# alexlocher/hpmvs

Measured on AMD Instinct MI355X. Metric: refined_patches_per_sec, higher is better.
Workload: dtype f32 textures / f64 optimiser

## Files before the change

hpmvs_amd/api.py:

```python
from __future__ import annotations

import ctypes as C
import os
from dataclasses import dataclass

import numpy as np

try:
    import torch
except Exception:
    torch = None

HERE = os.path.dirname(os.path.abspath(__file__))
LIB_PATH = os.environ.get("HPMVS_LIB") or os.path.join(HERE, "libhpmvs_amd.so")
MAX_IMAGES = 256
FAST_IMAGES = 64
MAX_LEVELS = 8


class HpmvsError(RuntimeError):
    pass


class Options(C.Structure):
    _fields_ = [("MAXLEVEL", C.c_int32), ("MINLEVEL", C.c_int32), ("MAX_ANGLE", C.c_float),
                ("MIN_ANGLE", C.c_float), ("MAX_IMAGES_PER_PATCH", C.c_int32),
                ("MIN_IMAGES_PER_PATCH", C.c_int32), ("NCC_ALPHA_1", C.c_float), ("NCC_ALPHA_2", C.c_float)]


class Camera(C.Structure):
    _fields_ = [("P0", C.c_float * 12), ("center", C.c_float * 4), ("xaxis", C.c_float * 3),
                ("yaxis", C.c_float * 3), ("zaxis", C.c_float * 3), ("fsum", C.c_float), ("n_levels", C.c_int32)]


class PatchBatch(C.Structure):
    _fields_ = [("n", C.c_int32), ("max_images", C.c_int32), ("center", C.c_void_p), ("normal", C.c_void_p),
                ("scale", C.c_void_p), ("n_images", C.c_void_p), ("images", C.c_void_p), ("ok", C.c_void_p),
                ("color", C.c_void_p), ("ncc", C.c_void_p), ("fmin", C.c_void_p), ("x", C.c_void_p),
                ("result", C.c_void_p), ("nevals", C.c_void_p), ("stage", C.c_void_p), ("ngrabs", C.c_void_p)]


class LeafTable(C.Structure):
    _fields_ = [("n", C.c_int32), ("root_center", C.c_float * 3), ("root_width", C.c_float), ("cell_center", C.c_void_p),
                ("cell_width", C.c_void_p), ("patch_center", C.c_void_p), ("born", C.c_void_p), ("died", C.c_void_p)]


class OctreeIndex(C.Structure):
    _fields_ = [("root_center", C.c_float * 3), ("root_width", C.c_float), ("n_branches", C.c_int32), ("n_leaves", C.c_int32),
                ("branch_key", C.c_void_p), ("leaf_key", C.c_void_p)]


class ExtendTreeKeysStruct(C.Structure):
    _fields_ = [("skip", C.c_void_p), ("pre_inside", C.c_void_p), ("pre_key", C.c_void_p), ("border", C.c_void_p),
                ("post_key", C.c_void_p)]


class OctreeForest(C.Structure):
    _fields_ = [("n_trees", C.c_int32), ("root", C.c_void_p), ("branch_first", C.c_void_p), ("leaf_first", C.c_void_p),
                ("branch_key", C.c_void_p), ("leaf_key", C.c_void_p)]


class ProcessForestResultStruct(C.Structure):
    _fields_ = [("support", C.c_void_p), ("removed", C.c_void_p), ("split", C.c_void_p), ("children", C.c_void_p),
                ("child_key", C.c_void_p), ("n_neighbours", C.c_void_p), ("neighbour_key", C.c_void_p)]


class BorderForestResultStruct(C.Structure):
    _fields_ = [("tree", C.c_void_p), ("accepted", C.c_void_p), ("leaf_key", C.c_void_p), ("blocker", C.c_void_p)]


class OctreePartitionInfo(C.Structure):
    _fields_ = [("n_trees", C.c_int32), ("n_orphans", C.c_int32), ("n_splits", C.c_int32), ("stop", C.c_int32),
                ("histogram", C.c_int32 * 22)]


class SeedTreeInfo(C.Structure):
    _fields_ = [("root_center", C.c_float * 3), ("root_width", C.c_float), ("scale_floor", C.c_float), ("n_rows", C.c_int32),
                ("n_leaves", C.c_int32)]


EXPORTS = [
    "hpmvs_last_error", "hpmvs_device_count", "hpmvs_build_id", "hpmvs_default_options", "hpmvs_camera_from_nvm",
    "hpmvs_scene_create", "hpmvs_scene_set_view", "hpmvs_scene_set_covis", "hpmvs_scene_commit",
    "hpmvs_scene_destroy", "hpmvs_scene_get_level", "hpmvs_scene_bytes", "hpmvs_build_pyramid",
    "hpmvs_optimize_batch", "hpmvs_init_patches_batch", "hpmvs_objective_batch", "hpmvs_inccs_batch", "hpmvs_last_kernel_ms",
    "hpmvs_last_wide_patches",
    "hpmvs_expand_batch", "hpmvs_expand_directions", "hpmvs_selftest_bobyqa",
    "hpmvs_pack_records", "hpmvs_unpack_records", "hpmvs_allgather_records", "hpmvs_pack_record_tails", "hpmvs_unpack_record_tails",
    "hpmvs_scene_depth_reset", "hpmvs_scene_depth_set_level", "hpmvs_scene_depth_get_level",
    "hpmvs_set_depths_batch", "hpmvs_depth_gates_batch", "hpmvs_depth_footprints_batch", "hpmvs_depth_ops_batch", "hpmvs_level_support_batch",
    "hpmvs_host_alloc", "hpmvs_host_free", "hpmvs_last_staging",
    "hpmvs_undistort", "hpmvs_undistort_map", "hpmvs_scene_set_view_distorted",
    "hpmvs_regularize_batch", "hpmvs_filter_batch", "hpmvs_seed_tree_batch", "hpmvs_octree_locate_batch",
    "hpmvs_octree_insert_batch", "hpmvs_octree_route_batch", "hpmvs_octree_partition", "hpmvs_extend_tree_batch",
    "hpmvs_extend_forest_batch", "hpmvs_process_forest_batch", "hpmvs_border_forest_batch",
    "hpmvs_level_conflicts_batch", "hpmvs_conflicts_from_footprints", "hpmvs_level_walk_batch", "hpmvs_last_level_walk",
    "hpmvs_scene_center", "hpmvs_init_patches_sphere_batch",
    "hpmvs_jpeg_info", "hpmvs_jpeg_decode", "hpmvs_scene_set_view_jpeg", "hpmvs_jpeg_decode_timed",
    "hpmvs_jpeg_decode_ex", "hpmvs_scene_set_view_jpeg_ex", "hpmvs_jpeg_coefficients", "hpmvs_jpeg_entropy_timed",
    "hpmvs_jpeg_last_decode",
    "hpmvs_jpeg_encode_bound", "hpmvs_jpeg_encode", "hpmvs_jpeg_encode_timed", "hpmvs_scene_get_level_jpeg",
    "hpmvs_depth_colormap", "hpmvs_scene_depth_image", "hpmvs_scene_depth_jpeg",
    "hpmvs_ply_ext_batch", "hpmvs_ply_ext_timed",
]
JPEG_ENTROPY = {"auto": 0, "host": 1, "device": 2}


_lib = None


def lib():
    global _lib
    if _lib is not None:
        return _lib
    if not os.path.exists(LIB_PATH):
        raise HpmvsError(f"{LIB_PATH} is missing: run `python -c 'import __graft_entry__ as g; g.build()'` "
                         "(there is no fallback implementation)")
    L = C.CDLL(LIB_PATH)
    L.hpmvs_last_error.restype = C.c_char_p
    L.hpmvs_build_id.restype = C.c_char_p
    L.hpmvs_default_options.argtypes = [C.POINTER(Options)]
    L.hpmvs_camera_from_nvm.argtypes = [C.c_double, C.POINTER(C.c_double), C.POINTER(C.c_double), C.c_int, C.c_int,
                                        C.c_int, C.POINTER(Camera)]
    L.hpmvs_scene_create.argtypes = [C.c_int, C.c_int, C.POINTER(C.c_void_p)]
    L.hpmvs_scene_set_view.argtypes = [C.c_void_p, C.c_int, C.c_int, C.c_int, C.c_void_p, C.c_int, C.POINTER(Camera)]
    L.hpmvs_scene_set_covis.argtypes = [C.c_void_p, C.c_int, C.POINTER(C.c_int32), C.c_int]
    L.hpmvs_scene_commit.argtypes = [C.c_void_p]
    L.hpmvs_scene_destroy.argtypes = [C.c_void_p]
    L.hpmvs_scene_get_level.argtypes = [C.c_void_p, C.c_int, C.c_int, C.c_void_p, C.c_size_t, C.POINTER(C.c_int),
                                        C.POINTER(C.c_int)]
    L.hpmvs_scene_bytes.restype = C.c_size_t
    L.hpmvs_scene_bytes.argtypes = [C.c_void_p]
    L.hpmvs_build_pyramid.argtypes = [C.c_int, C.c_void_p, C.c_int, C.c_int, C.c_void_p, C.c_int]
    L.hpmvs_undistort.argtypes = [C.c_int, C.c_void_p, C.c_int, C.c_int, C.c_float, C.c_float, C.c_void_p, C.c_int]
    L.hpmvs_undistort_map.argtypes = [C.c_int, C.c_int, C.c_int, C.c_float, C.c_float, C.c_void_p]
    L.hpmvs_scene_set_view_distorted.argtypes = [C.c_void_p, C.c_int, C.c_int, C.c_int, C.c_void_p, C.c_int,
                                                 C.POINTER(Camera), C.c_float, C.c_float]
    L.hpmvs_jpeg_info.argtypes = [C.c_char_p, C.c_size_t] + [C.POINTER(C.c_int)] * 5
    L.hpmvs_jpeg_decode.argtypes = [C.c_int, C.c_char_p, C.c_size_t, C.c_void_p, C.c_size_t, C.c_int]
    L.hpmvs_jpeg_decode_timed.argtypes = [C.c_int, C.c_char_p, C.c_size_t, C.c_void_p, C.c_size_t, C.POINTER(C.c_float)]
    L.hpmvs_scene_set_view_jpeg.argtypes = [C.c_void_p, C.c_int, C.c_char_p, C.c_size_t, C.POINTER(Camera), C.c_float, C.c_float]
    L.hpmvs_jpeg_decode_ex.argtypes = [C.c_int, C.c_char_p, C.c_size_t, C.c_void_p, C.c_size_t, C.c_int, C.c_int, C.POINTER(C.c_int)]
    L.hpmvs_scene_set_view_jpeg_ex.argtypes = [C.c_void_p, C.c_int, C.c_char_p, C.c_size_t, C.POINTER(Camera), C.c_float, C.c_float,
                                               C.c_int, C.POINTER(C.c_int)]
    L.hpmvs_jpeg_coefficients.argtypes = [C.c_int, C.c_char_p, C.c_size_t, C.c_int, C.c_int, C.c_void_p, C.c_size_t,
                                          C.POINTER(C.c_int), C.POINTER(C.c_int)]
    L.hpmvs_jpeg_last_decode.argtypes = [C.POINTER(C.c_int), C.POINTER(C.c_int)]
    L.hpmvs_jpeg_entropy_timed.argtypes = [C.c_int, C.c_char_p, C.c_size_t, C.c_void_p, C.c_size_t, C.POINTER(C.c_float)]
    L.hpmvs_jpeg_encode_bound.restype = C.c_size_t
    L.hpmvs_jpeg_encode_bound.argtypes = [C.c_int, C.c_int]
    L.hpmvs_jpeg_encode.argtypes = [C.c_int, C.c_void_p, C.c_int, C.c_int, C.c_int, C.c_void_p, C.c_size_t, C.POINTER(C.c_size_t), C.c_int]
    L.hpmvs_jpeg_encode_timed.argtypes = [C.c_int, C.c_void_p, C.c_int, C.c_int, C.c_int, C.c_void_p, C.c_size_t, C.POINTER(C.c_size_t),
                                          C.POINTER(C.c_float)]
    L.hpmvs_scene_get_level_jpeg.argtypes = [C.c_void_p, C.c_int, C.c_int, C.c_int, C.c_void_p, C.c_size_t, C.POINTER(C.c_size_t)]
    L.hpmvs_optimize_batch.argtypes = [C.c_void_p, C.POINTER(Options), C.POINTER(PatchBatch), C.c_int, C.c_void_p]
    L.hpmvs_init_patches_batch.argtypes = [C.c_void_p, C.POINTER(Options), C.c_int, C.c_int, C.c_void_p, C.c_void_p,
                                           C.c_void_p, C.POINTER(PatchBatch), C.c_int, C.c_void_p]
    L.hpmvs_init_patches_sphere_batch.argtypes = [C.c_void_p, C.POINTER(Options), C.c_int, C.c_int, C.c_void_p, C.c_void_p,
                                                  C.c_void_p, C.c_void_p, C.POINTER(PatchBatch), C.c_int, C.c_void_p]
    L.hpmvs_scene_center.argtypes = [C.c_void_p, C.c_int, C.POINTER(C.c_double), C.POINTER(C.c_double), C.POINTER(C.c_int)]
    L.hpmvs_objective_batch.argtypes = [C.c_void_p, C.POINTER(Options), C.POINTER(PatchBatch), C.c_void_p,
                                        C.c_void_p, C.c_void_p, C.c_int, C.c_void_p]
    L.hpmvs_inccs_batch.argtypes = [C.c_void_p, C.POINTER(Options), C.POINTER(PatchBatch), C.c_int, C.c_int,
                                    C.c_void_p, C.c_int, C.c_void_p]
    L.hpmvs_last_kernel_ms.argtypes = [C.c_void_p, C.POINTER(C.c_float)]
    L.hpmvs_host_alloc.argtypes = [C.c_size_t]
    L.hpmvs_host_alloc.restype = C.c_void_p
    L.hpmvs_host_free.argtypes = [C.c_void_p]
    L.hpmvs_host_free.restype = None
    L.hpmvs_last_staging.argtypes = [C.c_void_p, C.POINTER(C.c_ulonglong), C.POINTER(C.c_ulonglong)]
    L.hpmvs_expand_batch.argtypes = [C.c_void_p, C.POINTER(Options), C.c_int, C.POINTER(PatchBatch), C.c_void_p,
                                     C.c_void_p, C.c_void_p, C.POINTER(PatchBatch), C.c_int, C.c_void_p]
    L.hpmvs_expand_directions.argtypes = [C.c_int, C.c_void_p]
    L.hpmvs_scene_depth_reset.argtypes = [C.c_void_p]
    L.hpmvs_scene_depth_set_level.argtypes = [C.c_void_p, C.c_int, C.c_int, C.c_void_p, C.c_int, C.c_int]
    L.hpmvs_scene_depth_get_level.argtypes = [C.c_void_p, C.c_int, C.c_int, C.c_void_p, C.c_size_t, C.POINTER(C.c_int),
                                              C.POINTER(C.c_int)]
    L.hpmvs_depth_colormap.argtypes = [C.c_void_p]
    L.hpmvs_scene_depth_image.argtypes = [C.c_void_p, C.c_int, C.c_int, C.c_void_p, C.c_size_t, C.c_int, C.POINTER(C.c_int),
                                          C.POINTER(C.c_int), C.POINTER(C.c_float)]
    L.hpmvs_scene_depth_jpeg.argtypes = [C.c_void_p, C.c_int, C.c_int, C.c_int, C.c_void_p, C.c_size_t, C.POINTER(C.c_size_t)]
    L.hpmvs_set_depths_batch.argtypes = [C.c_void_p, C.POINTER(PatchBatch), C.c_int, C.c_void_p]
    L.hpmvs_depth_footprints_batch.argtypes = [C.c_void_p, C.POINTER(PatchBatch), C.c_void_p, C.c_void_p, C.c_void_p, C.c_void_p,
                                               C.c_int, C.c_void_p]
    L.hpmvs_level_conflicts_batch.argtypes = [C.c_void_p, C.POINTER(PatchBatch), C.c_void_p, C.c_void_p, C.c_void_p, C.c_size_t,
                                              C.c_void_p, C.c_void_p, C.c_size_t, C.POINTER(C.c_uint32), C.POINTER(C.c_uint32),
                                              C.c_int, C.c_void_p]
    L.hpmvs_conflicts_from_footprints.argtypes = [C.c_int] * 5 + [C.c_void_p] * 6 + [C.c_void_p, C.c_void_p, C.c_size_t,
                                                  C.c_void_p, C.c_void_p, C.c_size_t, C.POINTER(C.c_uint32), C.POINTER(C.c_uint32),
                                                  C.c_int, C.c_void_p]
    L.hpmvs_level_walk_batch.argtypes = [C.c_void_p, C.POINTER(Options), C.POINTER(PatchBatch)] + [C.c_void_p] * 4 + [C.c_float, C.c_int] + \
        [C.c_void_p] * 4 + [C.POINTER(C.c_int32), C.c_int, C.c_void_p]
    L.hpmvs_last_level_walk.argtypes = [C.c_void_p] + [C.POINTER(C.c_int32)] * 3
    L.hpmvs_depth_gates_batch.argtypes = [C.c_void_p, C.POINTER(PatchBatch), C.c_float, C.c_int, C.c_void_p, C.c_void_p,
                                          C.c_void_p, C.c_int, C.c_void_p]
    L.hpmvs_depth_ops_batch.argtypes = [C.c_void_p, C.POINTER(PatchBatch), C.c_void_p, C.c_int, C.c_void_p]
    L.hpmvs_regularize_batch.argtypes = [C.c_void_p, C.POINTER(PatchBatch), C.c_void_p, C.c_void_p, C.c_void_p, C.POINTER(LeafTable),
                                         C.c_void_p, C.c_void_p, C.c_void_p, C.c_int, C.c_void_p]
    L.hpmvs_level_support_batch.argtypes = [C.c_void_p, C.POINTER(PatchBatch), C.c_int, C.c_void_p, C.c_int, C.c_void_p]
    L.hpmvs_filter_batch.argtypes = [C.c_void_p, C.POINTER(PatchBatch), C.c_void_p, C.c_int, C.c_void_p, C.c_void_p, C.c_int, C.c_void_p]
    L.hpmvs_seed_tree_batch.argtypes = [C.c_void_p, C.POINTER(PatchBatch), C.c_int, C.c_int, C.POINTER(SeedTreeInfo), C.c_void_p,
                                        C.c_void_p, C.c_void_p, C.c_void_p, C.c_void_p, C.c_void_p, C.c_int, C.c_void_p]
    L.hpmvs_octree_locate_batch.argtypes = [C.c_void_p, C.POINTER(OctreeIndex), C.c_int] + [C.c_void_p] * 8 + [C.c_int, C.c_void_p]
    L.hpmvs_octree_insert_batch.argtypes = [C.c_void_p, C.POINTER(OctreeIndex), C.c_int] + [C.c_void_p] * 5 + [C.c_int, C.c_void_p]
    L.hpmvs_extend_tree_batch.argtypes = [C.c_void_p, C.POINTER(Options), C.POINTER(OctreeIndex), C.POINTER(PatchBatch), C.c_float,
                                          C.POINTER(PatchBatch), C.POINTER(ExtendTreeKeysStruct), C.c_int, C.c_void_p]
    L.hpmvs_extend_forest_batch.argtypes = [C.c_void_p, C.POINTER(Options), C.POINTER(OctreeForest), C.POINTER(PatchBatch), C.c_void_p,
                                            C.c_float, C.POINTER(PatchBatch), C.POINTER(ExtendTreeKeysStruct), C.c_int, C.c_void_p]
    L.hpmvs_process_forest_batch.argtypes = [C.c_void_p, C.POINTER(Options), C.POINTER(OctreeForest), C.c_void_p, C.POINTER(PatchBatch),
                                             C.c_void_p, C.c_void_p, C.c_void_p, C.c_void_p, C.POINTER(PatchBatch),
                                             C.POINTER(ProcessForestResultStruct), C.c_int, C.c_void_p]
    L.hpmvs_border_forest_batch.argtypes = [C.c_void_p, C.POINTER(OctreeForest), C.POINTER(PatchBatch), C.c_int,
                                            C.POINTER(BorderForestResultStruct), C.c_int, C.c_void_p]
    L.hpmvs_octree_route_batch.argtypes = [C.c_void_p, C.c_int, C.c_void_p, C.c_int, C.c_void_p, C.c_void_p, C.c_int, C.c_void_p]
    L.hpmvs_octree_partition.argtypes = [C.c_void_p, C.POINTER(OctreeIndex), C.c_int, C.c_int, C.POINTER(OctreePartitionInfo)] + \
        [C.c_void_p] * 9 + [C.c_int, C.c_void_p]
    L.hpmvs_ply_ext_batch.argtypes = [C.c_int, C.POINTER(PatchBatch), C.c_void_p, C.c_int, C.c_int, C.c_void_p, C.c_size_t,
                                      C.POINTER(C.c_size_t), C.c_int, C.c_void_p]
    L.hpmvs_ply_ext_timed.argtypes = [C.c_int, C.POINTER(PatchBatch), C.c_void_p, C.c_int, C.c_int, C.c_void_p, C.c_size_t,
                                      C.POINTER(C.c_size_t), C.POINTER(C.c_float)]
    _lib = L
    return L


def _chk(rc):
    if rc != 0:
        raise HpmvsError(f"hpmvs_amd error {rc}: {lib().hpmvs_last_error().decode()}")


def build_id() -> str:
    return lib().hpmvs_build_id().decode()


def device_count() -> int:
    return lib().hpmvs_device_count()


def default_options() -> Options:
    o = Options()
    lib().hpmvs_default_options(C.byref(o))
    return o


def camera_from_nvm(f, q, c, width, height, max_level=5) -> Camera:
    cam = Camera()
    qq = (C.c_double * 4)(*[float(t) for t in q])
    cc = (C.c_double * 3)(*[float(t) for t in c])
    _chk(lib().hpmvs_camera_from_nvm(float(f), qq, cc, int(width), int(height), int(max_level), C.byref(cam)))
    return cam


def scene_center(cameras):
    cams = (Camera * max(1, len(cameras)))(*cameras)
    center, radius, valid = (C.c_double * 3)(), C.c_double(), C.c_int()
    _chk(lib().hpmvs_scene_center(cams, len(cameras), center, C.byref(radius), C.byref(valid)))
    if not valid.value:
        return None
    return np.array(center[:], dtype=np.float64), radius.value


def _ptr(a):
    if a is None:
        return None
    if isinstance(a, np.ndarray):
        return a.ctypes.data
    if isinstance(a, int):
        return a
    return a.data_ptr()


def undistort(img, f: float, k1: float, device: int = 0):
    if isinstance(img, np.ndarray):
        src = np.ascontiguousarray(img, dtype=np.uint8)
        if src.ndim != 3 or src.shape[2] != 3:
            raise HpmvsError("undistort: img must be uint8 [H, W, 3]")
        out = np.empty_like(src)
        _chk(lib().hpmvs_undistort(device, src.ctypes.data, src.shape[1], src.shape[0], float(f), float(k1),
                                   out.ctypes.data, 0))
        return out
    src = img.contiguous()
    if src.dim() != 3 or src.shape[2] != 3 or str(src.dtype) != "torch.uint8":
        raise HpmvsError("undistort: img must be uint8 [H, W, 3]")
    out = torch.empty_like(src)
    _chk(lib().hpmvs_undistort(device, src.data_ptr(), src.shape[1], src.shape[0], float(f), float(k1), out.data_ptr(), 1))
    return out


def undistort_map(w: int, h: int, f: float, k1: float, device: int = 0) -> np.ndarray:
    xy = np.empty((int(h), int(w), 2), dtype=np.float32)
    _chk(lib().hpmvs_undistort_map(device, int(w), int(h), float(f), float(k1), xy.ctypes.data))
    return xy


def jpeg_info(data):
    data = bytes(data)
    v = [C.c_int() for _ in range(5)]
    _chk(lib().hpmvs_jpeg_info(data, len(data), *[C.byref(x) for x in v]))
    return tuple(x.value for x in v)


def _jpeg_entropy(name):
    if name not in JPEG_ENTROPY:
        raise HpmvsError(f"entropy must be one of {sorted(JPEG_ENTROPY)}, not {name!r}")
    return JPEG_ENTROPY[name]


def jpeg_decode(data, device: int = 0, on_device: bool = False, entropy: str = "auto"):
    data = bytes(data)
    mode = _jpeg_entropy(entropy)
    w, h = jpeg_info(data)[:2]
    if on_device:
        out = torch.empty((h, w, 3), dtype=torch.uint8, device=f"cuda:{device}")
        ptr, nb = out.data_ptr(), out.numel()
    else:
        out = np.empty((h, w, 3), dtype=np.uint8)
        ptr, nb = out.ctypes.data, out.nbytes
    if mode == 0:
        _chk(lib().hpmvs_jpeg_decode(device, data, len(data), ptr, nb, int(on_device)))
    else:
        _chk(lib().hpmvs_jpeg_decode_ex(device, data, len(data), ptr, nb, int(on_device), mode, None))
    return out


def jpeg_coefficients(data, entropy: str = "auto", subseq_bits: int = 0, device: int = 0):
    data = bytes(data)
    w, h, comps, hs, vs = jpeg_info(data)
    mx, my = -(-w // (8 * hs)), -(-h // (8 * vs))
    out = np.empty(64 * mx * my * (hs * vs + (2 if comps == 3 else 0)), dtype=np.int16)
    used, rounds = C.c_int(), C.c_int()
    _chk(lib().hpmvs_jpeg_coefficients(device, data, len(data), _jpeg_entropy(entropy), int(subseq_bits), out.ctypes.data, out.size,
                                       C.byref(used), C.byref(rounds)))
    return out, "device" if used.value == 2 else "host", rounds.value


def jpeg_encode_bound(width: int, height: int) -> int:
    return int(lib().hpmvs_jpeg_encode_bound(int(width), int(height)))


def jpeg_encode(rgb, quality: int = 100, device: int = 0) -> bytes:
    if isinstance(rgb, np.ndarray):
        rgb = np.ascontiguousarray(rgb, dtype=np.uint8)
        ptr, on_device = rgb.ctypes.data, 0
    else:
        rgb = rgb.contiguous()
        ptr, on_device = rgb.data_ptr(), 1
    if rgb.ndim != 3 or rgb.shape[2] != 3 or (on_device and rgb.dtype != torch.uint8):
        raise HpmvsError("jpeg_encode: pixels must be uint8 [H, W, 3]")
    h, w = int(rgb.shape[0]), int(rgb.shape[1])
    out = np.empty(max(1, jpeg_encode_bound(w, h)), dtype=np.uint8)
    n = C.c_size_t(0)
    _chk(lib().hpmvs_jpeg_encode(device, ptr, w, h, int(quality), out.ctypes.data, out.nbytes, C.byref(n), on_device))
    return out[:n.value].tobytes()


class Scene:

    def __init__(self, synth_scene, device: int = 0, jpeg_entropy: str = "auto"):
        L = lib()
        jpeg_mode = _jpeg_entropy(jpeg_entropy)
        self.h = C.c_void_p()
        self.device = device
        self.n_views = synth_scene.n_views
        self.view_levels = []
        self.cameras = []
        _chk(L.hpmvs_scene_create(self.n_views, device, C.byref(self.h)))
        for i, v in enumerate(synth_scene.views):
            rgb = v.rgb
            if isinstance(rgb, (bytes, bytearray)):
                data = bytes(rgb)
                w, h = jpeg_info(data)[:2]
                cam = camera_from_nvm(v.f, v.q, v.c, w, h, synth_scene.max_level)
                self.view_levels.append(int(cam.n_levels))
                self.cameras.append(cam)
                if jpeg_mode == 0:
                    _chk(L.hpmvs_scene_set_view_jpeg(self.h, i, data, len(data), C.byref(cam), float(v.f),
                                                     float(getattr(v, "k1", 0.0))))
                else:
                    _chk(L.hpmvs_scene_set_view_jpeg_ex(self.h, i, data, len(data), C.byref(cam), float(v.f),
                                                        float(getattr(v, "k1", 0.0)), jpeg_mode, None))
                continue
            cam = camera_from_nvm(v.f, v.q, v.c, v.width, v.height, synth_scene.max_level)
            self.view_levels.append(int(cam.n_levels))
            self.cameras.append(cam)
            if isinstance(rgb, np.ndarray):
                rgb = np.ascontiguousarray(rgb, dtype=np.uint8)
                ptr, on_device = rgb.ctypes.data, 0
            else:
                rgb = rgb.contiguous()
                ptr, on_device = rgb.data_ptr(), 1
            k1 = float(getattr(v, "k1", 0.0))
            if k1 != 0.0:
                _chk(L.hpmvs_scene_set_view_distorted(self.h, i, v.width, v.height, ptr, on_device, C.byref(cam),
                                                      float(v.f), k1))
            else:
                _chk(L.hpmvs_scene_set_view(self.h, i, v.width, v.height, ptr, on_device, C.byref(cam)))
        for i, lst in enumerate(synth_scene.covis):
            arr = (C.c_int32 * max(1, len(lst)))(*lst)
            _chk(L.hpmvs_scene_set_covis(self.h, i, arr, len(lst)))
        _chk(L.hpmvs_scene_commit(self.h))

    def close(self):
        if self.h:
            lib().hpmvs_scene_destroy(self.h)
            self.h = C.c_void_p()

    def __del__(self):
        try:
            self.close()
        except Exception:
            pass

    def bytes(self) -> int:
        return lib().hpmvs_scene_bytes(self.h)

    def level(self, view: int, level: int) -> np.ndarray:
        w, h = C.c_int(), C.c_int()
        _chk(lib().hpmvs_scene_get_level(self.h, view, level, None, 0, C.byref(w), C.byref(h)))
        out = np.empty((h.value, w.value, 3), dtype=np.uint8)
        _chk(lib().hpmvs_scene_get_level(self.h, view, level, out.ctypes.data, out.nbytes, C.byref(w), C.byref(h)))
        return out

    def level_jpeg(self, view: int, level: int = 0, quality: int = 100) -> bytes:
        n = C.c_size_t(0)
        _chk(lib().hpmvs_scene_get_level_jpeg(self.h, view, level, int(quality), None, 0, C.byref(n)))
        out = np.empty(n.value, dtype=np.uint8)
        _chk(lib().hpmvs_scene_get_level_jpeg(self.h, view, level, int(quality), out.ctypes.data, out.nbytes, C.byref(n)))
        return out[:n.value].tobytes()

    def depth_image(self, view: int, level=None, with_range: bool = False):
        lv = DEPTH_COMBINED if level is None else int(level)
        w, h = C.c_int(), C.c_int()
        _chk(lib().hpmvs_scene_depth_image(self.h, view, lv, None, 0, 0, C.byref(w), C.byref(h), None))
        out = np.empty((h.value, w.value, 3), dtype=np.uint8)
        rng = (C.c_float * 2)()
        _chk(lib().hpmvs_scene_depth_image(self.h, view, lv, out.ctypes.data if out.size else None, out.nbytes, 0, C.byref(w), C.byref(h), rng))
        return (out, (np.float32(rng[0]), np.float32(rng[1]))) if with_range else out

    def depth_jpeg(self, view: int, level=None, quality: int = 100) -> bytes:
        lv = DEPTH_COMBINED if level is None else int(level)
        n = C.c_size_t(0)
        _chk(lib().hpmvs_scene_depth_jpeg(self.h, view, lv, int(quality), None, 0, C.byref(n)))
        out = np.empty(n.value, dtype=np.uint8)
        _chk(lib().hpmvs_scene_depth_jpeg(self.h, view, lv, int(quality), out.ctypes.data, out.nbytes, C.byref(n)))
        return out[:n.value].tobytes()

    def last_staging(self):
        a, b = C.c_ulonglong(), C.c_ulonglong()
        _chk(lib().hpmvs_last_staging(self.h, C.byref(a), C.byref(b)))
        return a.value, b.value

    def last_wide_patches(self) -> int:
        n = C.c_int32()
        _chk(lib().hpmvs_last_wide_patches(self.h, C.byref(n)))
        return n.value

    def last_kernel_ms(self) -> float:
        ms = C.c_float()
        _chk(lib().hpmvs_last_kernel_ms(self.h, C.byref(ms)))
        return ms.value


class Batch:

    def __init__(self, center, normal, scale, n_images, images):
        self.n = int(len(scale))
        self.max_images = int(images.shape[1])
        self.center = np.ascontiguousarray(center, dtype=np.float32).copy()
        self.normal = np.ascontiguousarray(normal, dtype=np.float32).copy()
        self.scale = np.ascontiguousarray(scale, dtype=np.float32).copy()
        self.n_images = np.ascontiguousarray(n_images, dtype=np.int32).copy()
        self.images = np.ascontiguousarray(images, dtype=np.int32).copy()
        n = self.n
        self.ok = np.zeros(n, dtype=np.uint8)
        self.color = np.zeros((n, 3), dtype=np.float32)
        self.ncc = np.zeros(n, dtype=np.float32)
        self.fmin = np.zeros(n, dtype=np.float64)
        self.x = np.zeros((n, 3), dtype=np.float64)
        self.result = np.zeros(n, dtype=np.int32)
        self.nevals = np.zeros(n, dtype=np.int32)
        self.stage = np.zeros(n, dtype=np.int32)
        self.ngrabs = np.zeros(n, dtype=np.int32)

    @classmethod
    def from_seeds(cls, seeds, idx=None):
        if idx is None:
            idx = np.arange(len(seeds.scale))
        idx = np.asarray(idx)
        return cls(seeds.center[idx], seeds.normal[idx], seeds.scale[idx], seeds.n_images[idx], seeds.images[idx])

    FIELDS = ("center", "normal", "scale", "n_images", "images", "ok", "color", "ncc", "fmin", "x", "result", "nevals",
              "stage", "ngrabs")

    def pin(self):
        import weakref
        L = lib()
        for name in self.FIELDS:
            a = getattr(self, name)
            nbytes = max(int(a.nbytes), 1)
            p = L.hpmvs_host_alloc(nbytes)
            if not p:
                raise MemoryError(f"hpmvs_host_alloc({nbytes})")
            buf = (C.c_char * nbytes).from_address(p)
            weakref.finalize(buf, L.hpmvs_host_free, p)
            na = np.frombuffer(buf, dtype=a.dtype, count=a.size).reshape(a.shape)
            na[...] = a
            setattr(self, name, na)
        return self

    def c_struct(self) -> PatchBatch:
        b = PatchBatch()
        b.n, b.max_images = self.n, self.max_images
        for name in ("center", "normal", "scale", "n_images", "images", "ok", "color", "ncc", "fmin", "x", "result",
                     "nevals", "stage", "ngrabs"):
            setattr(b, name, _ptr(getattr(self, name)))
        return b


def optimize_batch(scene: Scene, batch: Batch, options: Options | None = None) -> Batch:
    o = options or default_options()
    b = batch.c_struct()
    _chk(lib().hpmvs_optimize_batch(scene.h, C.byref(o), C.byref(b), 0, None))
    return batch


def init_patches_batch(scene: Scene, xyz, meas_off, meas_img, start_level=4, max_images=FAST_IMAGES,
                       options: Options | None = None, sphere=None) -> Batch:
    o = options or default_options()
    xyz = np.ascontiguousarray(xyz, dtype=np.float64)
    off = np.ascontiguousarray(meas_off, dtype=np.int32)
    img = np.ascontiguousarray(meas_img, dtype=np.int32)
    n = len(xyz)
    batch = Batch(np.zeros((n, 4), np.float32), np.zeros((n, 4), np.float32), np.zeros(n, np.float32),
                  np.zeros(n, np.int32), np.full((n, max_images), -1, np.int32))
    b = batch.c_struct()
    if sphere is None:
        _chk(lib().hpmvs_init_patches_batch(scene.h, C.byref(o), start_level, n, xyz.ctypes.data, off.ctypes.data,
                                            img.ctypes.data if len(img) else None, C.byref(b), 0, None))
        return batch
    sph = np.ascontiguousarray(sphere, dtype=np.float64).reshape(4)
    _chk(lib().hpmvs_init_patches_sphere_batch(scene.h, C.byref(o), start_level, n, xyz.ctypes.data, off.ctypes.data,
                                               img.ctypes.data if len(img) else None, sph.ctypes.data, C.byref(b), 0, None))
    return batch


EXPAND_EXTEND, EXPAND_BRANCH = 0, 1


def expand_directions(mode: int) -> np.ndarray:
    out = np.zeros(12, dtype=np.float32)
    n = lib().hpmvs_expand_directions(mode, out.ctypes.data)
    if n < 0:
        _chk(n)
    return out[:2 * n].reshape(n, 2)


def expand_batch(scene: Scene, mode: int, parents: Batch, cell_center, cell_width, skip=None,
                 options: Options | None = None) -> Batch:
    o = options or default_options()
    N = 6 if mode == EXPAND_EXTEND else 4
    n = parents.n
    cc = np.ascontiguousarray(cell_center, dtype=np.float32).reshape(n, 3)
    cw = np.ascontiguousarray(cell_width, dtype=np.float32).reshape(n)
    sk = None if skip is None else np.ascontiguousarray(skip, dtype=np.uint8).reshape(n * N)
    out = Batch(np.zeros((n * N, 4), np.float32), np.zeros((n * N, 4), np.float32), np.zeros(n * N, np.float32),
                np.zeros(n * N, np.int32), np.full((n * N, parents.max_images), -1, np.int32))
    pb, ob = parents.c_struct(), out.c_struct()
    _chk(lib().hpmvs_expand_batch(scene.h, C.byref(o), mode, C.byref(pb), cc.ctypes.data, cw.ctypes.data,
                                  None if sk is None else sk.ctypes.data, C.byref(ob), 0, None))
    return out


def objective_batch(scene: Scene, batch: Batch, x: np.ndarray, options: Options | None = None):
    o = options or default_options()
    b = batch.c_struct()
    x = np.ascontiguousarray(x, dtype=np.float64)
    f = np.zeros(batch.n, dtype=np.float64)
    g = np.zeros(batch.n, dtype=np.int32)
    _chk(lib().hpmvs_objective_batch(scene.h, C.byref(o), C.byref(b), x.ctypes.data, f.ctypes.data, g.ctypes.data, 0,
                                     None))
    return f, g


def inccs_batch(scene: Scene, batch: Batch, ref_idx=0, robust=0, options: Options | None = None) -> np.ndarray:
    o = options or default_options()
    b = batch.c_struct()
    out = np.zeros((batch.n, batch.max_images), dtype=np.float32)
    _chk(lib().hpmvs_inccs_batch(scene.h, C.byref(o), C.byref(b), ref_idx, robust, out.ctypes.data, 0, None))
    return out


def depth_reset(scene: Scene):
    _chk(lib().hpmvs_scene_depth_reset(scene.h))


def depth_level(scene: Scene, view: int, level: int) -> np.ndarray:
    r, c = C.c_int(), C.c_int()
    _chk(lib().hpmvs_scene_depth_get_level(scene.h, view, level, None, 0, C.byref(r), C.byref(c)))
    out = np.zeros((c.value, r.value), dtype=np.float32)
    _chk(lib().hpmvs_scene_depth_get_level(scene.h, view, level, out.ctypes.data, out.size, C.byref(r), C.byref(c)))
    return out


depth_get_level = depth_level


def depth_set_level(scene: Scene, view: int, level: int, data):
    m = np.ascontiguousarray(data, dtype=np.float32)
    if m.size:
        _chk(lib().hpmvs_scene_depth_set_level(scene.h, view, level, m.ctypes.data, m.shape[1], m.shape[0]))


DEPTH_COMBINED = -1


def depth_colormap() -> np.ndarray:
    lut = np.zeros((256, 3), dtype=np.uint8)
    _chk(lib().hpmvs_depth_colormap(lut.ctypes.data))
    return lut


def set_depths_batch(scene: Scene, batch: Batch):
    b = batch.c_struct()
    _chk(lib().hpmvs_set_depths_batch(scene.h, C.byref(b), 0, None))


def depth_ops_batch(scene: Scene, batch: Batch, subtract):
    b = batch.c_struct()
    sub = np.ascontiguousarray(subtract, dtype=np.uint8).reshape(batch.n)
    _chk(lib().hpmvs_depth_ops_batch(scene.h, C.byref(b), sub.ctypes.data, 0, None))


def level_support_batch(scene: Scene, batch: Batch, min_level=0):
    b = batch.c_struct()
    out = np.zeros(batch.n, dtype=np.int32)
    _chk(lib().hpmvs_level_support_batch(scene.h, C.byref(b), int(min_level), out.ctypes.data, 0, None))
    return out


def depth_gates_batch(scene: Scene, batch: Batch, margin=1.0, abs_int=0):
    b = batch.c_struct()
    v = np.zeros(batch.n, dtype=np.int32); k = np.zeros(batch.n, dtype=np.int32); f = np.zeros(batch.n, dtype=np.int32)
    _chk(lib().hpmvs_depth_gates_batch(scene.h, C.byref(b), float(margin), int(abs_int), v.ctypes.data, k.ctypes.data,
                                       f.ctypes.data, 0, None))
    return v, k, f


def depth_footprints_batch(scene: Scene, batch: Batch):
    b = batch.c_struct()
    n, M, V = batch.n, batch.max_images, scene.n_views
    wr = np.zeros((n, M, 4), np.int32); fr = np.zeros((n, M, 4), np.int32)
    at = np.zeros((n, M, 3), np.int32); vb = np.zeros((n, V, 3), np.int32)
    _chk(lib().hpmvs_depth_footprints_batch(scene.h, C.byref(b), wr.ctypes.data, fr.ctypes.data, at.ctypes.data, vb.ctypes.data, 0, None))
    return wr, fr, at, vb


def _conflicts(call, n):
    fo = np.zeros(n + 1, np.uint32); ao = np.zeros(n + 1, np.uint32)
    nf, na = C.c_uint32(0), C.c_uint32(0)
    fa = np.zeros(32 * n + 64, np.uint32); aa = np.zeros(32 * n + 64, np.uint32)
    rc = call(fo.ctypes.data, fa.ctypes.data, fa.size, ao.ctypes.data, aa.ctypes.data, aa.size, C.byref(nf), C.byref(na))
    if rc != 0:
        if "capacity" not in lib().hpmvs_last_error().decode():
            _chk(rc)
        fa = np.zeros(nf.value, np.uint32); aa = np.zeros(na.value, np.uint32)
        _chk(call(fo.ctypes.data, fa.ctypes.data, fa.size, ao.ctypes.data, aa.ctypes.data, aa.size, C.byref(nf), C.byref(na)))
    return fo, fa[:nf.value].copy(), ao, aa[:na.value].copy()


def level_conflicts(scene: Scene, batch: Batch, is_event=None):
    b = batch.c_struct()
    ev = None if is_event is None else np.ascontiguousarray(is_event, dtype=np.uint8).reshape(batch.n)
    evp = None if ev is None else ev.ctypes.data
    return _conflicts(lambda fo, fa, cf, ao, aa, ca, nf, na: lib().hpmvs_level_conflicts_batch(
        scene.h, C.byref(b), evp, fo, fa, cf, ao, aa, ca, nf, na, 0, None), batch.n)


def conflicts_from_footprints(n_images, writes, frees, attached, view_block, n_levels, is_event=None, device: int = 0):
    wr = np.ascontiguousarray(writes, dtype=np.int32); fr = np.ascontiguousarray(frees, dtype=np.int32)
    at = np.ascontiguousarray(attached, dtype=np.int32); vb = np.ascontiguousarray(view_block, dtype=np.int32)
    n, M, V = wr.shape[0], wr.shape[1], vb.shape[1]
    if wr.shape != (n, M, 4) or fr.shape != (n, M, 4) or at.shape != (n, M, 3) or vb.shape != (n, V, 3):
        raise ValueError("conflicts_from_footprints: the footprint arrays do not have the layouts of depth_footprints_batch")
    ni = np.ascontiguousarray(n_images, dtype=np.int32).reshape(n)
    ev = None if is_event is None else np.ascontiguousarray(is_event, dtype=np.uint8).reshape(n)
    evp = None if ev is None else ev.ctypes.data
    return _conflicts(lambda fo, fa, cf, ao, aa, ca, nf, na: lib().hpmvs_conflicts_from_footprints(
        int(device), n, M, V, int(n_levels), ni.ctypes.data, wr.ctypes.data, fr.ctypes.data, at.ctypes.data, vb.ctypes.data, evp,
        fo, fa, cf, ao, aa, ca, nf, na, 0, None), n)


WALK_EVENT, WALK_REFINED, WALK_BORDER, WALK_HAS_PRE, WALK_PRE_TAKEN, WALK_POST_TAKEN = 1, 2, 4, 8, 16, 32


def level_walk(scene: Scene, batch: Batch, flags, set, pre_key, post_key, margin=1.0, abs_int=0, options: Options | None = None,
               stage=None):
    o = options or default_options()
    n = batch.n
    b = batch.c_struct()
    fl = np.ascontiguousarray(flags, dtype=np.uint8).reshape(n)
    st = None if set is None else np.ascontiguousarray(set, dtype=np.int32).reshape(n)
    pre = np.ascontiguousarray(pre_key, dtype=np.uint64).reshape(n)
    post = np.ascontiguousarray(post_key, dtype=np.uint64).reshape(n)
    stage = np.array(batch.stage if stage is None else stage, dtype=np.int32).reshape(n)
    counts = np.full((n, 3), -1, np.int32); accepted = np.zeros(n, np.uint8); wave = np.zeros(n, np.int32)
    n_waves = C.c_int32(0)
    _chk(lib().hpmvs_level_walk_batch(scene.h, C.byref(o), C.byref(b), fl.ctypes.data, None if st is None else st.ctypes.data,
                                      pre.ctypes.data, post.ctypes.data, float(margin), int(abs_int), stage.ctypes.data,
                                      counts.ctypes.data, accepted.ctypes.data, wave.ctypes.data, C.byref(n_waves), 0, None))
    return stage, counts, accepted, wave, int(n_waves.value)


def last_level_walk(scene: Scene):
    r, m, f = C.c_int32(0), C.c_int32(0), C.c_int32(0)
    _chk(lib().hpmvs_last_level_walk(scene.h, C.byref(r), C.byref(m), C.byref(f)))
    return int(r.value), int(m.value), int(f.value)


def build_pyramid(img: np.ndarray, device: int = 0) -> np.ndarray:
    h, w, _ = img.shape
    img = np.ascontiguousarray(img, dtype=np.uint8)
    out = np.zeros((h // 2, w // 2, 3), dtype=np.uint8)
    _chk(lib().hpmvs_build_pyramid(device, img.ctypes.data, w, h, out.ctypes.data, 0))
    return out


INT32_MAX = 2**31 - 1
REGULARIZE_PROBES = 24


def regularize_batch(scene: Scene, cells: Batch, cell_width, position, expanded, root_center, root_width, leaf_center,
                     leaf_width, leaf_patch, born=None, died=None, flatness=None, neighbours: bool = True):
    n = cells.n
    L = int(len(leaf_width))
    cw = np.ascontiguousarray(cell_width, dtype=np.float32).reshape(n)
    pos = np.ascontiguousarray(position, dtype=np.int32).reshape(n)
    exp = np.ascontiguousarray(expanded).astype(np.uint8).reshape(n)
    lc = np.ascontiguousarray(leaf_center, dtype=np.float32).reshape(L, 3)
    lw = np.ascontiguousarray(leaf_width, dtype=np.float32).reshape(L)
    lp = np.ascontiguousarray(np.asarray(leaf_patch, dtype=np.float32)[:, :3]).reshape(L, 3)
    lb = np.full(L, -1, np.int32) if born is None else np.ascontiguousarray(born, dtype=np.int32).reshape(L)
    ld = np.full(L, INT32_MAX, np.int32) if died is None else np.ascontiguousarray(died, dtype=np.int32).reshape(L)
    t = LeafTable()
    t.n = L
    for k in range(3):
        t.root_center[k] = float(np.float32(root_center[k]))
    t.root_width = float(np.float32(root_width))
    t.cell_center, t.cell_width, t.patch_center = lc.ctypes.data, lw.ctypes.data, lp.ctypes.data
    t.born, t.died = lb.ctypes.data, ld.ctypes.data
    fl = np.full(n, -1.0, np.float32) if flatness is None else np.ascontiguousarray(flatness, dtype=np.float32).reshape(n).copy()
    nn = np.zeros(n, np.int32)
    nb = np.zeros((n, REGULARIZE_PROBES), np.int32) if neighbours else None
    b = cells.c_struct()
    _chk(lib().hpmvs_regularize_batch(scene.h, C.byref(b), cw.ctypes.data, pos.ctypes.data, exp.ctypes.data, C.byref(t),
                                      fl.ctypes.data, nn.ctypes.data, None if nb is None else nb.ctypes.data, 0, None))
    return fl, nn, nb


def filter_batch(scene: Scene, patches: Batch, cell_start):
# ... 315 lines not shown
```

hpmvs_amd/csrc/capi.hip:

```cpp
#include <hip/hip_runtime.h>

#include <dlfcn.h>

#include <algorithm>
#include <atomic>
#include <chrono>
#include <cmath>
#include <cstdio>
#include <cstdlib>
#include <cstring>
#include <mutex>
#include <optional>
#include <string>
#include <thread>
#include <time.h>
#include <vector>

#include "../../include/hpmvs_amd.h"
#include "capi_common.hpp"
#include "dev_types.h"
#include "launch.h"
#include "octree.hpp"
#include "ply_text.hpp"

// ... 2489 lines not shown
        if (!on_device) {
            df = nf ? (uint32_t*)c.scratch(4 * (size_t)nf) : nullptr; da = na ? (uint32_t*)c.scratch(4 * (size_t)na) : nullptr;
            if ((nf && !df) || (na && !da)) return c.error();
        }
        launch_conflicts_adjacency(pairs, nf, na, df, da, st);
        HIPCHK(hipGetLastError());
        if (!on_device) {
            HIPCHK(hipStreamSynchronize(st));
            if (nf) HIPCHK(hipMemcpy(flow_adj, df, 4 * (size_t)nf, hipMemcpyDeviceToHost));
            if (na) HIPCHK(hipMemcpy(anti_adj, da, 4 * (size_t)na, hipMemcpyDeviceToHost));
        }
    }
    const int done = c.finish();
    if (done) return done;
    if (!fits) return fail(HPMVS_ERR_ARG, who + ": capacity: the graph has " + std::to_string(nf) + " flow and " + std::to_string(na) +
                                              " anti entries (n_flow / n_anti are set; allocate and call again)");
    return HPMVS_OK;
}
static int conflicts_empty(int on_device, uint32_t* flow_off, uint32_t* anti_off, uint32_t* n_flow, uint32_t* n_anti, hipStream_t st) {
    if (on_device) {
        HIPCHK(hipMemsetAsync(flow_off, 0, 4, st));
        HIPCHK(hipMemsetAsync(anti_off, 0, 4, st));
    } else { flow_off[0] = 0; anti_off[0] = 0; }
    *n_flow = 0; *n_anti = 0;
    return HPMVS_OK;
}

int hpmvs_conflicts_from_footprints(int device, int n, int max_images, int n_views, int n_levels, const int32_t* n_images, const int32_t* writes,
                                    const int32_t* frees, const int32_t* attached, const int32_t* view_block, const uint8_t* is_event,
                                    uint32_t* flow_off, uint32_t* flow_adj, size_t cap_flow, uint32_t* anti_off, uint32_t* anti_adj,
                                    size_t cap_anti, uint32_t* n_flow, uint32_t* n_anti, int on_device, void* stream) {
    const std::string who = "conflicts_from_footprints";
    int rc = conflicts_check(who, n, max_images, n_views, n_levels, flow_off, flow_adj, cap_flow, anti_off, anti_adj, cap_anti, n_flow, n_anti);
    if (rc) return rc;
    if (n > 0 && (!n_images || !writes || !frees || !attached || !view_block)) return fail(HPMVS_ERR_ARG, who + ": a footprint array is null");
    const int count = hpmvs_device_count();
    if (count <= 0) return fail(HPMVS_ERR_NODEVICE, who + ": no HIP device visible");
    if (device < 0 || device >= count) return fail(HPMVS_ERR_ARG, who + ": no such device");
    HIPCHK(hipSetDevice(device));
    hipStream_t st = (hipStream_t)stream;
    if (n == 0) return conflicts_empty(on_device, flow_off, anti_off, n_flow, n_anti, st);
    Call c(nullptr, on_device, st);
    const size_t N = (size_t)n, M = (size_t)max_images, V = (size_t)n_views;
    conflicts::Footprints F;
    F.n = n; F.M = max_images; F.V = n_views; F.n_levels = n_levels;
    F.n_images = c.in(n_images, N);
    F.wr = c.in(writes, N * M * 4); F.fr = c.in(frees, N * M * 4); F.at = c.in(attached, N * M * 3); F.vb = c.in(view_block, N * V * 3);
    F.is_event = c.in(is_event, N);
    uint32_t* dfo = c.arr(flow_off, N + 1, Call::kCopyBack);
    uint32_t* dao = c.arr(anti_off, N + 1, Call::kCopyBack);
    if ((rc = c.begin())) return rc;
    return conflicts_call(c, who, F, on_device, dfo, flow_adj, cap_flow, dao, anti_adj, cap_anti, n_flow, n_anti, st);
}

int hpmvs_level_conflicts_batch(const hpmvs_scene* s, const hpmvs_patch_batch* b, const uint8_t* is_event, uint32_t* flow_off, uint32_t* flow_adj,
                                size_t cap_flow, uint32_t* anti_off, uint32_t* anti_adj, size_t cap_anti, uint32_t* n_flow, uint32_t* n_anti,
                                int on_device, void* stream) {
    const std::string who = "level_conflicts_batch";
    int rc = check_depth_batch(s, b, who.c_str());
    if (rc) return rc;
    int n_levels = 1;
    for (int v = 0; v < s->n_views; v++) n_levels = std::max(n_levels, (int)s->hviews[v].n_levels);
    if ((rc = conflicts_check(who, b->n, b->max_images, s->n_views, n_levels, flow_off, flow_adj, cap_flow, anti_off, anti_adj, cap_anti, n_flow, n_anti)))
        return rc;
    HIPCHK(hipSetDevice(s->device));
    hipStream_t st = (hipStream_t)stream;
    if (b->n == 0) return conflicts_empty(on_device, flow_off, anti_off, n_flow, n_anti, st);
    Call c(s, on_device, st);
    const size_t N = (size_t)b->n, M = (size_t)b->max_images, V = (size_t)s->n_views;
    const DevBatch D = c.batch(b, Call::kRead);
    const uint8_t* dev = c.in(is_event, N);
    uint32_t* dfo = c.arr(flow_off, N + 1, Call::kCopyBack);
    uint32_t* dao = c.arr(anti_off, N + 1, Call::kCopyBack);
    int32_t* fp = (int32_t*)c.scratch(4 * N * (11 * M + 3 * V));
    if (!fp) return c.error();
    if ((rc = c.begin())) return rc;
    conflicts::Footprints F;
    F.n = b->n; F.M = b->max_images; F.V = s->n_views; F.n_levels = n_levels;
    F.n_images = D.n_images; F.is_event = dev;
    int32_t *wr = fp, *fr = wr + N * M * 4, *at = fr + N * M * 4, *vb = at + N * M * 3;
    F.wr = wr; F.fr = fr; F.at = at; F.vb = vb;
    launch_depth_footprints(dev_scene(s), s->ddepth, D, wr, fr, at, vb, st);
    HIPCHK(hipGetLastError());
    return conflicts_call(c, who, F, on_device, dfo, flow_adj, cap_flow, dao, anti_adj, cap_anti, n_flow, n_anti, st);
}

static constexpr int kWalkFewDecided = 8;
static constexpr int kWalkFinishBudget = 128;
int hpmvs_level_walk_batch(hpmvs_scene* s, const hpmvs_options* o, const hpmvs_patch_batch* items, const uint8_t* flags, const int32_t* set,
                           const uint64_t* pre_key, const uint64_t* post_key, float margin, int abs_int, int32_t* stage, int32_t* counts,
                           uint8_t* accepted, int32_t* wave, int32_t* n_waves, int on_device, void* stream) {
    const std::string who = "level_walk_batch";
    if (!s || !o || !items || !n_waves) return fail(HPMVS_ERR_ARG, who + ": null scene / options / batch / n_waves");
    if (items->n < 0 || items->max_images < 1 || items->max_images > HPMVS_MAX_IMAGES) return fail(HPMVS_ERR_ARG, who + ": bad n/max_images");
    if (items->n > 0 && (!items->center || !items->normal || !items->scale || !items->n_images || !items->images))
        return fail(HPMVS_ERR_ARG, who + ": batch input arrays missing");
    if (items->n > 0 && (!flags || !pre_key || !post_key || !stage || !counts || !accepted || !wave))
        return fail(HPMVS_ERR_ARG, who + ": flags / pre_key / post_key / stage / counts / accepted / wave missing");
    if (o->MIN_IMAGES_PER_PATCH < 1) return fail(HPMVS_ERR_ARG, who + ": MIN_IMAGES_PER_PATCH must be >= 1");
    int n_levels = 1;
    for (int v = 0; v < s->n_views; v++) n_levels = std::max(n_levels, (int)s->hviews[v].n_levels);
    {
        uint32_t off = 0, total = 0;
        const int rc = conflicts_check(who, items->n, items->max_images, s->n_views, n_levels, &off, nullptr, 0, &off, nullptr, 0, &total, &total);
        if (rc) return rc;
    }
    if (!s->committed || !s->depth_pool || !s->ddepth) return fail(HPMVS_ERR_STATE, who + ": call hpmvs_scene_depth_reset first");
    if (s->depth_floats >= ((size_t)1 << 32)) return fail(HPMVS_ERR_STATE, who + ": the scene's depth maps hold 2^32 cells or more");
    *n_waves = 0;
    for (auto& w : s->last_walk) w = 0;
    if (items->n == 0) return HPMVS_OK;
    HIPCHK(hipSetDevice(s->device));
    hipStream_t st = (hipStream_t)stream;
    int rc;
    Call c(s, on_device, st);
    const int n = items->n, M = items->max_images, V = s->n_views;
    const size_t N = (size_t)n;
    const DevBatch D = c.batch(items, Call::kRead);
    const uint8_t* dflags = c.in(flags, N);
    const int32_t* dset = c.in(set, N);
    const unsigned long long *dpre = c.in((const unsigned long long*)pre_key, N), *dpost = c.in((const unsigned long long*)post_key, N);
    int32_t* dstage = c.arr(stage, N, Call::kCopyIn | Call::kCopyBack);
    int32_t* dcounts = c.arr(counts, 3 * N, Call::kCopyBack);
    uint8_t* daccepted = c.arr(accepted, N, Call::kCopyBack);
    int32_t* dwave = c.arr(wave, N, Call::kCopyBack);
    size_t need = 0;
    auto room = [&need](size_t bytes) { const size_t at = need; need += reg_align(bytes); return at; };
    const size_t a_ctl = room(64), a_state = room(N), a_ok = room(N), a_sub = room(N), a_nev = room(N), a_mark = room(4 * N), a_scan = room(4 * N),
                 a_node = room(4 * N), a_item = room(4 * N), a_slot = room(4 * N), a_rows = room(4 * N), a_gv = room(4 * N), a_gb = room(4 * N),
                 a_gf = room(4 * N), a_fpre = room(4 * N), a_fpost = room(4 * N), a_foff = room(4 * (N + 1)), a_aoff = room(4 * (N + 1)),
                 a_k0 = room(16 * N), a_k1 = room(16 * N), a_key = room(16 * N), a_v0 = room(8 * N), a_v1 = room(8 * N), a_val = room(8 * N),
                 a_s0 = room(8 * N), a_set = room(8 * N), a_p0 = room(8 * N), a_perm = room(8 * N), a_bc = room(16 * N), a_bn = room(16 * N),
                 a_bs = room(4 * N), a_bi = room(4 * N), a_bm = room(4 * N * (size_t)M);
    char* block = (char*)c.scratch(need);
    if ((rc = c.begin())) return rc;
    if (!block) return c.error() ? c.error() : fail(HPMVS_ERR_HIP, who + ": out of device memory");
    unsigned int* ctl = (unsigned int*)(block + a_ctl);
    uint8_t *state = (uint8_t*)(block + a_state), *ok = (uint8_t*)(block + a_ok), *sub = (uint8_t*)(block + a_sub), *node_event = (uint8_t*)(block + a_nev);
    uint32_t *mark = (uint32_t*)(block + a_mark), *scan = (uint32_t*)(block + a_scan);
    int32_t *node_of = (int32_t*)(block + a_node), *item_of = (int32_t*)(block + a_item), *slot_of = (int32_t*)(block + a_slot), *rows = (int32_t*)(block + a_rows);
    uint32_t *flow_off = (uint32_t*)(block + a_foff), *anti_off = (uint32_t*)(block + a_aoff);
    DevBatch B;
    memset(&B, 0, sizeof(B));
    B.max_images = M;
    B.center = (float*)(block + a_bc); B.normal = (float*)(block + a_bn); B.scale = (float*)(block + a_bs);
    B.n_images = (int32_t*)(block + a_bi); B.images = (int32_t*)(block + a_bm);
    auto temp_of = [&c](size_t bytes) { return c.scratch(bytes ? bytes : 16); };
#define WALK_PRIM(call_with_temp)                                                                        \
    do {                                                                                                 \
        void* temp = nullptr; size_t temp_bytes = 0;                                                     \
        if ((call_with_temp) != 0) return fail(HPMVS_ERR_HIP, who + ": rocPRIM size query failed");      \
        if (!(temp = temp_of(temp_bytes))) return c.error();                                             \
        if ((call_with_temp) != 0) return fail(HPMVS_ERR_HIP, who + ": rocPRIM call failed");            \
    } while (0)

    HIPCHK(hipMemsetAsync(ctl, 0, 64, st));
    launch_walk_check(n, dflags, dset, ctl + 8, st);
    unsigned int bad = 0;
    HIPCHK(hipMemcpyAsync(&bad, ctl + 8, 4, hipMemcpyDeviceToHost, st));
    HIPCHK(hipStreamSynchronize(st));
    if (bad) return fail(HPMVS_ERR_ARG, who + ": " + std::to_string(bad) + " items with a flag byte that cannot occur (an event that is refined or border, an unknown bit) or a negative set");
    launch_walk_mark(n, dflags, mark, st);
    WALK_PRIM(walk_scan(temp, &temp_bytes, mark, scan, n, st));
    launch_walk_nodes(n, dflags, mark, scan, node_of, item_of, node_event, sub, ctl + 9, st);
    unsigned int n_nodes = 0;
    HIPCHK(hipMemcpyAsync(&n_nodes, ctl + 9, 4, hipMemcpyDeviceToHost, st));
    HIPCHK(hipStreamSynchronize(st));
    if (n_nodes > (unsigned int)n) return fail(HPMVS_ERR_HIP, who + ": node count");
    uint32_t *flow_adj = nullptr, *anti_adj = nullptr;
    if (n_nodes) {
        B.n = (int)n_nodes;
        launch_walk_gather(D, item_of, (int)n_nodes, B, st);
        int32_t* fp = (int32_t*)c.scratch(4 * (size_t)n_nodes * (11 * (size_t)M + 3 * (size_t)V));
        if (!fp) return c.error();
        conflicts::Footprints F;
        F.n = (int)n_nodes; F.M = M; F.V = V; F.n_levels = n_levels; F.n_images = B.n_images; F.is_event = node_event;
        int32_t *wr = fp, *fr = wr + (size_t)n_nodes * M * 4, *at = fr + (size_t)n_nodes * M * 4, *vb = at + (size_t)n_nodes * M * 3;
        F.wr = wr; F.fr = fr; F.at = at; F.vb = vb;
        launch_depth_footprints(dev_scene(s), s->ddepth, B, wr, fr, at, vb, st);
        HIPCHK(hipGetLastError());
        const unsigned long long* pairs = nullptr;
        uint32_t nf = 0, na = 0;
        const int grc = launch_conflicts(F, [&c](size_t bytes) { return c.scratch(bytes); }, flow_off, anti_off, &pairs, &nf, &na, st);
        if (grc == kConflictsMemory) return c.error() ? c.error() : fail(HPMVS_ERR_HIP, who + ": out of device memory");
        if (grc == kConflictsTooMany)
            return fail(HPMVS_ERR_STATE, who + ": more than 2^30 conflicting (reader, writer) pairs before duplicates are dropped");
        if (grc != kConflictsOk) return fail(HPMVS_ERR_HIP, who + ": " + hipGetErrorString(hipGetLastError()));
        flow_adj = (uint32_t*)c.scratch(4 * ((size_t)nf + 1)); anti_adj = (uint32_t*)c.scratch(4 * ((size_t)na + 1));
        if (!flow_adj || !anti_adj) return c.error();
        launch_conflicts_adjacency(pairs, nf, na, flow_adj, anti_adj, st);
        HIPCHK(hipGetLastError());
    }
    unsigned long long *k0 = (unsigned long long*)(block + a_k0), *k1 = (unsigned long long*)(block + a_k1), *rec_key = (unsigned long long*)(block + a_key);
    uint32_t *v0 = (uint32_t*)(block + a_v0), *v1 = (uint32_t*)(block + a_v1), *rec_val = (uint32_t*)(block + a_val);
    uint32_t *s0 = (uint32_t*)(block + a_s0), *rec_set = (uint32_t*)(block + a_set), *p0 = (uint32_t*)(block + a_p0), *perm = (uint32_t*)(block + a_perm);
    launch_walk_records(n, dflags, dpre, dpost, k0, v0, st);
    WALK_PRIM(walk_sort_keys64(temp, &temp_bytes, k0, k1, v0, v1, 2 * n, st));
    launch_walk_record_sets(n, dflags, dset, v1, s0, p0, st);
    WALK_PRIM(walk_sort_keys32(temp, &temp_bytes, s0, rec_set, p0, perm, 2 * n, st));
    launch_walk_permute(n, perm, k1, v1, rec_key, rec_val, st);
    level_walk::Level L;
    L.n = n; L.min_images = o->MIN_IMAGES_PER_PATCH; L.flags = dflags; L.set = dset; L.pre = dpre; L.post = dpost;
    L.node_of = node_of; L.item_of = item_of; L.flow_off = flow_off; L.flow_adj = flow_adj; L.anti_off = anti_off; L.anti_adj = anti_adj;
    L.n_rec = 2u * (unsigned int)n; L.rec_set = rec_set; L.rec_key = rec_key; L.rec_val = rec_val;
    L.first_pre = (uint32_t*)(block + a_fpre); L.first_post = (uint32_t*)(block + a_fpost);
    launch_walk_first(L, (uint32_t*)(block + a_fpre), (uint32_t*)(block + a_fpost), st);
    launch_walk_init(n, state, ok, dcounts, daccepted, dwave, st);
    HIPCHK(hipGetLastError());
    WalkArrays A;
    A.state = state; A.ok = ok; A.slot_of = slot_of; A.gv = (int32_t*)(block + a_gv); A.gb = (int32_t*)(block + a_gb); A.gf = (int32_t*)(block + a_gf);
    A.n_images = D.n_images; A.stage = dstage; A.counts = dcounts; A.wave = dwave; A.accepted = daccepted;
    DevBatch Dok = D;
    Dok.ok = ok;
    const DevScene sc = dev_scene(s);
    unsigned long long *op_keys = nullptr, *op_sorted = nullptr;
    void* op_temp = nullptr;
    size_t op_temp_bytes = 0;
    int waves = 0, rounds_all = 0, rounds_most = 0, finishes = 0;
    for (int w = 1;; w++) {
        HIPCHK(hipMemsetAsync(ctl, 0, 32, st));
        launch_walk_begin(n, dflags, state, ok, rows, slot_of, ctl, st);
        unsigned int head[2] = {0, 0};
        HIPCHK(hipMemcpyAsync(head, ctl, 8, hipMemcpyDeviceToHost, st));
        HIPCHK(hipStreamSynchronize(st));
        const unsigned int pending = head[0], gated = head[1];
        if (!pending) break;
        if (w > n || pending > (unsigned int)n || gated > pending) return fail(HPMVS_ERR_STATE, who + ": the waves do not end (a bug: the first pending item of a wave always decides)");
        waves = w;
        if (gated) {
            B.n = (int)gated;
            launch_walk_gather(D, rows, (int)gated, B, st);
            launch_depth_gates(sc, s->ddepth, B, margin, abs_int, A.gv, A.gb, A.gf, st);
        }
        unsigned int tail[3] = {0, 0, 0};
        int rounds = 0;
        for (unsigned int decided = 0; decided < pending;) {
            launch_walk_round(L, A, w, ctl, st);
            HIPCHK(hipMemcpyAsync(tail, ctl + 2, 12, hipMemcpyDeviceToHost, st));
            HIPCHK(hipStreamSynchronize(st));
            rounds++;
            if (tail[0] <= decided || tail[0] > pending) return fail(HPMVS_ERR_STATE, who + ": a round decided nothing (a bug: the first undecided item always decides)");
            const bool few = tail[0] - decided < (unsigned int)kWalkFewDecided;
            decided = tail[0];
            if (few && decided < pending && pending - decided <= (unsigned int)kWalkFinishBudget) {
                launch_walk_finish(L, A, w, kWalkFinishBudget, ctl, st);
                HIPCHK(hipMemcpyAsync(tail, ctl + 2, 12, hipMemcpyDeviceToHost, st));
                HIPCHK(hipStreamSynchronize(st));
                finishes++;
                if (tail[0] <= decided || tail[0] > pending) return fail(HPMVS_ERR_STATE, who + ": the in-order pass decided nothing (a bug)");
                decided = tail[0];
            }
        }
        HIPCHK(hipGetLastError());
        rounds_all += rounds; rounds_most = std::max(rounds_most, rounds);
        if (tail[1] && !tail[2]) launch_set_depths(sc, s->ddepth, Dok, st);
        else if (tail[1]) {
            const size_t cap = N * (size_t)M;
            if (!op_keys) {
                op_keys = (unsigned long long*)c.scratch(8 * cap); op_sorted = (unsigned long long*)c.scratch(8 * cap);
                if (!op_keys || !op_sorted) return c.error();
            }
            HIPCHK(hipMemsetAsync(ctl + 10, 0, 4, st));
            launch_depth_ops_keys(sc, s->ddepth, s->depth_pool, Dok, op_keys, ctl + 10, st);
            unsigned int count = 0;
            HIPCHK(hipMemcpyAsync(&count, ctl + 10, 4, hipMemcpyDeviceToHost, st));
            HIPCHK(hipStreamSynchronize(st));
            if (count > cap) return fail(HPMVS_ERR_HIP, who + ": depth-op key count");
            if (count) {
                size_t bytes = 0;
                if (depth_ops_sort(nullptr, &bytes, op_keys, op_sorted, count, st) != 0) return fail(HPMVS_ERR_HIP, who + ": rocPRIM size query failed");
                if (bytes > op_temp_bytes || !op_temp) {
                    if (!(op_temp = temp_of(bytes))) return c.error();
                    op_temp_bytes = bytes;
                }
                if (depth_ops_sort(op_temp, &bytes, op_keys, op_sorted, count, st) != 0) return fail(HPMVS_ERR_HIP, who + ": rocPRIM sort failed");
                launch_depth_ops_apply(sc, s->ddepth, s->depth_pool, Dok, sub, op_sorted, count, st);
            }
        }
        HIPCHK(hipGetLastError());
    }
#undef WALK_PRIM
    *n_waves = waves;
    s->last_walk[0] = rounds_all; s->last_walk[1] = rounds_most; s->last_walk[2] = finishes;
    return c.finish();
}
int hpmvs_last_level_walk(const hpmvs_scene* s, int32_t* rounds, int32_t* most_rounds, int32_t* in_order_passes) {
    if (!s) return fail(HPMVS_ERR_ARG, "last_level_walk: null scene");
    if (rounds) *rounds = s->last_walk[0];
    if (most_rounds) *most_rounds = s->last_walk[1];
    if (in_order_passes) *in_order_passes = s->last_walk[2];
    return HPMVS_OK;
}

int hpmvs_last_wide_patches(const hpmvs_scene* s, int32_t* n) {
    if (!s || !n) return fail(HPMVS_ERR_ARG, "last_wide_patches: null argument");
    *n = 0;
    if (!s->last_ws) return HPMVS_OK;
    HIPCHK(hipSetDevice(s->device));
    HIPCHK(hipDeviceSynchronize());
    HIPCHK(hipMemcpy(n, s->last_ws + 241, sizeof(int32_t), hipMemcpyDeviceToHost));
    return HPMVS_OK;
}

int hpmvs_debug_counters(const hpmvs_scene* s, unsigned long long* out4) {
    if (!s || !out4) return fail(HPMVS_ERR_ARG, "debug_counters: null argument");
    HIPCHK(hipSetDevice(s->device));
    { const int rcq = service_quiesce(s); if (rcq) return rcq; }
    HIPCHK(hipDeviceSynchronize());
    if (!s->last_queue) return fail(HPMVS_ERR_STATE, "debug_counters: no launch yet");
    HIPCHK(hipMemcpy(out4, (char*)s->last_queue + 16, 544, hipMemcpyDeviceToHost));
    return HPMVS_OK;
}

int hpmvs_last_staging(const hpmvs_scene* s, unsigned long long* staged_bytes, unsigned long long* in_place_bytes) {
    if (!s || !staged_bytes || !in_place_bytes) return fail(HPMVS_ERR_ARG, "last_staging: null argument");
    *staged_bytes = s->last_staged_bytes; *in_place_bytes = s->last_mapped_bytes;
    return HPMVS_OK;
}

void* hpmvs_host_alloc(size_t bytes) {
    void* p = nullptr;
    if (bytes == 0 || hipHostMalloc(&p, bytes, hipHostMallocDefault) != hipSuccess) { (void)hipGetLastError(); return nullptr; }
    return p;
}
void hpmvs_host_free(void* p) {
    if (p && hipHostFree(p) != hipSuccess) (void)hipGetLastError();
}

int hpmvs_last_kernel_ms(const hpmvs_scene* s, float* ms) {
    if (!s || !ms) return fail(HPMVS_ERR_ARG, "last_kernel_ms: null argument");
    if (!s->timed) return fail(HPMVS_ERR_STATE, "last_kernel_ms: no optimize launch yet");
    HIPCHK(hipSetDevice(s->device));
    HIPCHK(hipEventSynchronize(s->ev1));
    HIPCHK(hipEventElapsedTime(ms, s->ev0, s->ev1));
    return HPMVS_OK;
}

}
```

hpmvs_amd/csrc/kernel_optimize.hip:

```cpp
#include <hip/hip_runtime.h>
#include <atomic>

#include "prof.h"
#define BQ_STATE_LDS 1
#define BQ_STATE_LDS_EXTERN 1
#ifndef BQ_P
#define BQ_P 29
#endif
#define BQ_SLOTS BQ_P
#ifndef HPMVS_STATIC_SLOTS
#define HPMVS_STATIC_SLOTS (!HPMVS_COLD_GLOBAL)
#endif
#ifndef HPMVS_STATIC_MAX_PER_WG
#define HPMVS_STATIC_MAX_PER_WG(W_, kS_) ((W_) * (kS_))
#endif
#ifndef HPMVS_SPREAD_SOLO
#define HPMVS_SPREAD_SOLO 1
#endif
#ifndef HPMVS_COLD_GLOBAL
#define HPMVS_COLD_GLOBAL 0
#endif
#if HPMVS_COLD_GLOBAL
#define BQ_COLD_GLOBAL 1
#ifndef BQ_COLD_LO
#define BQ_COLD_LO 77
#endif
#ifndef BQ_COLD_HI
#define BQ_COLD_HI 138
#endif
#define HPMVS_STATE_ND (164 - (BQ_COLD_HI - BQ_COLD_LO))
#else
#define HPMVS_STATE_ND 164
#endif
#define HPMVS_STATE_NI 13
#define HPMVS_REGION_BYTES (HPMVS_STATE_ND * 8 * BQ_P + HPMVS_STATE_NI * 4 * BQ_P)
#define HPMVS_REGION_KIB ((HPMVS_REGION_BYTES + 1023) / 1024)
#define HPMVS_REGION_16 (HPMVS_REGION_KIB * 64)
#ifndef HPMVS_WG_WAVES
#define HPMVS_WG_WAVES 8
#endif
#ifndef HPMVS_WG_REGIONS
#if HPMVS_COLD_GLOBAL
#define HPMVS_WG_REGIONS 6
#else
#define HPMVS_WG_REGIONS 4
#endif
#endif
#ifdef HPMVS_VARIANT_SUFFIX
#define HPMVS_CAT2(a, b) a##b
#define HPMVS_CAT(a, b) HPMVS_CAT2(a, b)
#define HPMVS_V(name) HPMVS_CAT(name, HPMVS_VARIANT_SUFFIX)
#define HPMVS_VK(name) HPMVS_CAT(name, HPMVS_VARIANT_SUFFIX)
#else
#define HPMVS_VK(name) name
#define HPMVS_V(name) name##_std
#endif
extern __shared__ uint4 hpmvs_dyn[];
#define bq_lds_d ((double*)hpmvs_dyn)
#define bq_lds_i ((int*)((char*)hpmvs_dyn + HPMVS_STATE_ND * 8 * BQ_P))
#include "bobyqa3.hpp"
#include "launch.h"
#include "photometric.hpp"
#include "pipeline.hpp"

namespace hpmvs {

static_assert(BQ_ND_LDS == HPMVS_STATE_ND && BQ_NI == HPMVS_STATE_NI, "state region sized for another layout");

namespace {

constexpr int kP = BQ_P;
constexpr int kRow = 64;
constexpr size_t kCounterBytes = 1024;
constexpr int kPark16 = HPMVS_REGION_16;

#ifndef HPMVS_PARK_AUX
#define HPMVS_PARK_AUX 0
#endif
#ifndef HPMVS_PROXY
#define HPMVS_PROXY 0
#endif
constexpr int kAuxDoubles = 64;
constexpr int kAuxVal = 18;
constexpr int kAuxGrabs = 25;
constexpr int kAuxCtx = 64;
constexpr int kMaxExtra = 7;
typedef __attribute__((address_space(1))) double gdouble;
typedef __attribute__((address_space(1))) float gfloat;
__device__ __forceinline__ void page_in(const uint4* __restrict__ park, uint4* hpmvs_region) {
    const char* g = (const char*)(park + lane_id());
#pragma unroll
    for (int c4 = 0; c4 < HPMVS_REGION_KIB; c4 += 4) {
        asm volatile("" : "+v"(g));
        auto lds = (__attribute__((address_space(3))) void*)(hpmvs_region + c4 * 64);
        auto src = (const __attribute__((address_space(1))) void*)g;
        __builtin_amdgcn_global_load_lds(src, lds, 16, 0, HPMVS_PARK_AUX);
        if (c4 + 1 < HPMVS_REGION_KIB) __builtin_amdgcn_global_load_lds(src, lds, 16, 1024, HPMVS_PARK_AUX);
        if (c4 + 2 < HPMVS_REGION_KIB) __builtin_amdgcn_global_load_lds(src, lds, 16, 2048, HPMVS_PARK_AUX);
        if (c4 + 3 < HPMVS_REGION_KIB) __builtin_amdgcn_global_load_lds(src, lds, 16, 3072, HPMVS_PARK_AUX);
        g += 4096;
    }
    asm volatile("s_waitcnt vmcnt(0)" ::: "memory");
}
#ifndef HPMVS_PARK_NT_STORE
#define HPMVS_PARK_NT_STORE 0
#endif
#if HPMVS_PARK_NT_STORE
#define HPMVS_PARK_ST(dst, v) __builtin_nontemporal_store((v), &(dst))
#else
#define HPMVS_PARK_ST(dst, v) (dst) = (v)
#endif
__device__ __attribute__((noinline)) void page_out(uint4* __restrict__ park, int region_index) {
    typedef unsigned int u4 __attribute__((ext_vector_type(4)));
    typedef __attribute__((address_space(1))) u4 gu4;
    const int lane = lane_id();
    const u4* region = (const u4*)(hpmvs_dyn + region_index * HPMVS_REGION_16);
    gu4* out = (gu4*)(unsigned long long)park;
    int c = 0;
#pragma unroll
    for (; c + 8 <= HPMVS_REGION_KIB; c += 8) {
        const u4 v0 = region[(c + 0) * 64 + lane], v1 = region[(c + 1) * 64 + lane], v2 = region[(c + 2) * 64 + lane],
                    v3 = region[(c + 3) * 64 + lane], v4 = region[(c + 4) * 64 + lane], v5 = region[(c + 5) * 64 + lane],
                    v6 = region[(c + 6) * 64 + lane], v7 = region[(c + 7) * 64 + lane];
        __builtin_amdgcn_sched_barrier(0);
        HPMVS_PARK_ST(out[(c + 0) * 64 + lane], v0); HPMVS_PARK_ST(out[(c + 1) * 64 + lane], v1); HPMVS_PARK_ST(out[(c + 2) * 64 + lane], v2); HPMVS_PARK_ST(out[(c + 3) * 64 + lane], v3);
        HPMVS_PARK_ST(out[(c + 4) * 64 + lane], v4); HPMVS_PARK_ST(out[(c + 5) * 64 + lane], v5); HPMVS_PARK_ST(out[(c + 6) * 64 + lane], v6); HPMVS_PARK_ST(out[(c + 7) * 64 + lane], v7);
        __builtin_amdgcn_sched_barrier(0);
    }
#pragma unroll
    for (; c < HPMVS_REGION_KIB; c++) { const u4 v = region[c * 64 + lane]; HPMVS_PARK_ST(out[c * 64 + lane], v); }
}

}

__device__ __forceinline__ unsigned long long ld_host64(const unsigned long long* p) {
    return __hip_atomic_load(p, __ATOMIC_RELAXED, __HIP_MEMORY_SCOPE_SYSTEM);
}

#ifndef HPMVS_WAVES_PER_EU
#define HPMVS_WAVES_PER_EU 2
#endif
#ifndef HPMVS_BQ_PRIO
#define HPMVS_BQ_PRIO 3
#endif
#ifndef HPMVS_LOCK_SLEEP
#define HPMVS_LOCK_SLEEP 8
#endif
#ifndef HPMVS_A_PRIO
#define HPMVS_A_PRIO 2
#endif
template <bool SERVICE, int W, int R>
__device__ __forceinline__ void optimize_body(DevScene sc, DevOptions o, DevBatch b, int32_t* queue) {
    const int lane = lane_id();
    const int wv = (int)(threadIdx.x >> 6);
    int* const hpmvs_lock = (int*)(hpmvs_dyn + R * HPMVS_REGION_16);
    const int n_wgs = (int)gridDim.x;
    const int gw = wv * n_wgs + (int)blockIdx.x;
    uint16_t* lists = (uint16_t*)((char*)queue + kCounterBytes) + (size_t)gw * kP * kRow;
    uint16_t* row = &lists[(lane < kP ? lane : 0) * kRow];
    uint4* park = (uint4*)((char*)queue + kCounterBytes + (size_t)W * n_wgs * kP * kRow * sizeof(uint16_t)) + (size_t)gw * kPark16;
#if HPMVS_COLD_GLOBAL
    char* cold = (char*)queue + kCounterBytes + (size_t)W * n_wgs * kP * kRow * sizeof(uint16_t) + (size_t)W * n_wgs * kPark16 * 16 +
                 (size_t)W * n_wgs * kP * kRow * sizeof(float) + (size_t)gw * BQ_NCOLD * kP * sizeof(double);
    {
        const unsigned long long a = (unsigned long long)cold;
        const unsigned lo = (unsigned)__builtin_amdgcn_readfirstlane((int)(a & 0xffffffffull)), hi = (unsigned)__builtin_amdgcn_readfirstlane((int)(a >> 32));
        cold = (char*)(((unsigned long long)hi << 32) | lo);
    }
#endif
    const GlobalRows erows{(float*)((char*)queue + kCounterBytes + (size_t)W * n_wgs * kP * kRow * sizeof(uint16_t) +
                                    (size_t)W * n_wgs * kPark16 * 16) + (size_t)gw * kP * kRow, kRow};
    constexpr bool kProxy = HPMVS_PROXY == 2 || (HPMVS_PROXY == 1 && SERVICE);
    gdouble* const auxw = (gdouble*)(unsigned long long)((char*)queue + kCounterBytes + (size_t)W * n_wgs * kP * kRow * sizeof(uint16_t) +
                          (size_t)W * n_wgs * kPark16 * 16 + (size_t)W * n_wgs * kP * kRow * sizeof(float) +
                          (size_t)W * n_wgs * (size_t)(HPMVS_COLD_GLOBAL ? (164 - HPMVS_STATE_ND) : 0) * kP * sizeof(double)) +
                          (size_t)gw * kP * kAuxDoubles;
    gdouble* const aux = auxw + (lane < kP ? lane : 0) * kAuxDoubles;
    int pre_nf = 0;
    bool pre_ctx = false;
    int extra = 0;
    int px_owner = -1;
    int px_k = 0;

    constexpr bool service = SERVICE;
    const int per_wg = (b.n + n_wgs - 1) / n_wgs;
    int quota = per_wg - wv * kP;
    quota = quota < 0 ? 0 : (quota < kP ? quota : kP);
#if HPMVS_SPREAD_SOLO
    if (4 * per_wg <= 3 * R * kP) {
        const int a = per_wg < R ? per_wg : R;
        quota = wv < a ? per_wg / a + (wv < per_wg % a ? 1 : 0) : 0;
    }
#endif
#if HPMVS_STATIC_SLOTS
    constexpr bool can_static = !SERVICE && (W % R == 0) && (W / R > 1);
    constexpr int kS = kP / (W / R > 0 ? W / R : 1);
    bool stat = false;
    if (can_static && per_wg <= HPMVS_STATIC_MAX_PER_WG(W, kS)) {
        stat = true;
        const int a = per_wg < W ? per_wg : W;
        quota = wv < a ? per_wg / a + (wv < per_wg % a ? 1 : 0) : 0;
    }
#endif
    if (service) quota = wv == 0 ? (b.svc_lanes < kP ? b.svc_lanes : kP) : 0;
    if (threadIdx.x <= R) hpmvs_lock[threadIdx.x] = 0;
    __syncthreads();
    if (quota == 0) {
        if (lane == 0) atomicOr(&hpmvs_lock[R], 1 << wv);
        return;
    }
    __builtin_amdgcn_s_setprio(HPMVS_A_PRIO);
    bool held = false, solo = false;
    int reg = 0;
    bool parked = false;
    int stage = (lane < quota) ? S_FETCH : S_IDLE;
    int idx = -1, nimg = 0, ii = 0, refindex = -1, ngrabs = 0, fail_stage = 0, nl_result = 0;
    float c0[3] = {0, 0, 0}, n0[3] = {0, 0, 0};
    float c[3] = {0, 0, 0}, n[3] = {0, 0, 1};
    float scale = 1.0f, refbest = 0.0f;
    OptFields F;
    Bobyqa3 B;
    B.slot = lane < kP ? lane : 0;
    B.slot_i = B.slot;
#if HPMVS_STATIC_SLOTS
    if (stat) {
        reg = wv / (W / R);
        const int sl = (lane < kS ? lane : 0) + (wv % (W / R)) * kS;
        B.slot = sl + reg * (HPMVS_REGION_16 * 2);
        B.slot_i = sl + reg * (HPMVS_REGION_16 * 4);
        held = true; solo = true;
    }
#endif
#if HPMVS_COLD_GLOBAL
    B.coff = (unsigned)B.slot * 8u;
    B.coldp = cold;
    B.cold = __builtin_amdgcn_make_buffer_rsrc(cold, 0, BQ_NCOLD * BQ_CSTRIDE * 8, 0x00020000);
#endif
    float ax[3] = {0, 0, 0}, ay[3] = {0, 0, 0}, az[3] = {0, 0, 1};
    int op = OP_NONE, req_ref = 0, req_robust = 0;
    float req_thr = 0.0f;
    double res_f = 0.0;
    unsigned long long res_mask = 0ull;
    float res_sum = 0.0f;
    const double lbv[3] = {-HUGE_VAL, -23.99999, -23.99999};
    const double ubv[3] = {HUGE_VAL, 23.99999, 23.99999};

#ifdef HPMVS_PROFILE_PHASES
    long long tA = 0, tB = 0, nrounds = 0, nreq = 0, t0 = clock64();
    s_prof[lane] = 0ull;
    __syncthreads();
#endif
    int res_n = 0, res_fail = 0;
    float res_rgb[3] = {0, 0, 0};
    int svc_n = 0, svc_closed = 0;
    uint32_t* srec = service ? b.svc_stage + ((size_t)gw * kP + (lane < kP ? lane : 0)) * kSvcOutDwords : nullptr;
    int fin_idx = 0;
    bool fin_pending = false;
    for (;;) {
        bool yield = false;
        if (service) {
            if (gw == 0 && lane == 0) {
                const int closed = __hip_atomic_load(&b.svc_ctrl[1], __ATOMIC_RELAXED, __HIP_MEMORY_SCOPE_SYSTEM);
                asm volatile("s_waitcnt vmcnt(0)" ::: "memory");
                const int n_pub = __hip_atomic_load(&b.svc_ctrl[0], __ATOMIC_RELAXED, __HIP_MEMORY_SCOPE_SYSTEM);
                __hip_atomic_store(&queue[200], n_pub, __ATOMIC_RELAXED, __HIP_MEMORY_SCOPE_AGENT);
                asm volatile("s_waitcnt vmcnt(0)" ::: "memory");
                __hip_atomic_store(&queue[201], closed, __ATOMIC_RELAXED, __HIP_MEMORY_SCOPE_AGENT);
            }
            int cl = 0, np = 0;
            if (lane == 0) {
                cl = __hip_atomic_load(&queue[201], __ATOMIC_RELAXED, __HIP_MEMORY_SCOPE_AGENT);
                asm volatile("s_waitcnt vmcnt(0)" ::: "memory");
                np = __hip_atomic_load(&queue[200], __ATOMIC_RELAXED, __HIP_MEMORY_SCOPE_AGENT);
            }
            svc_closed = bcast_i(cl, 0);
            svc_n = bcast_i(np, 0);
        }
        while (op == OP_NONE && stage != S_IDLE && !yield) {
            bool finish_fail = false, finish_ok = false;
            switch (stage) {
            case S_FETCH:
                idx = atomicAdd(queue, 1);
                if (idx >= b.n) { stage = S_IDLE; break; }
                if (service) { stage = S_WAIT; break; }
                [[fallthrough]];
            case S_WAIT: {
                if (service && stage == S_WAIT) {
                    if (idx >= svc_n) {
                        if (svc_closed) stage = S_IDLE; else yield = true;
                        break;
                    }
                }
                bool bad_id = false;
                if (service) {
                    const unsigned long long* in = b.svc_in + (size_t)idx * (kSvcInDwords / 2);
                    const unsigned long long w0 = ld_host64(in), w1 = ld_host64(in + 1), w2 = ld_host64(in + 2), w3 = ld_host64(in + 3);
                    c0[0] = __uint_as_float((unsigned)w0); c0[1] = __uint_as_float((unsigned)(w0 >> 32));
                    c0[2] = __uint_as_float((unsigned)w1); scale = __uint_as_float((unsigned)(w1 >> 32));
                    n0[0] = __uint_as_float((unsigned)w2); n0[1] = __uint_as_float((unsigned)(w2 >> 32));
                    n0[2] = __uint_as_float((unsigned)w3); nimg = (int)(unsigned)(w3 >> 32);
                    for (int k = 0; k < 3; k++) { c[k] = c0[k]; n[k] = n0[k]; }
                    ngrabs = 0; nl_result = 0;
                    srec[3] = 0;
                    for (int k = 20; k < 28; k++) srec[k] = 0;
                    if (nimg < 0) { fail_stage = -nimg; nimg = 0; finish_fail = true; break; }
                    if (nimg > kMaxImages || nimg > b.max_images) { fail_stage = 100; finish_fail = true; break; }
                    for (int k = 0; k < nimg; k += 2) {
                        const unsigned long long w = ld_host64(in + 4 + k / 2);
                        const int id0 = (int)(unsigned)w, id1 = (int)(unsigned)(w >> 32);
                        bad_id |= (id0 < 0 || id0 >= sc.n_views);
                        row[k] = (uint16_t)id0;
                        if (k + 1 < nimg) { bad_id |= (id1 < 0 || id1 >= sc.n_views); row[k + 1] = (uint16_t)id1; }
                    }
                } else {
                    for (int k = 0; k < 3; k++) { c0[k] = b.center[4 * idx + k]; n0[k] = b.normal[4 * idx + k]; c[k] = c0[k]; n[k] = n0[k]; }
                    scale = b.scale[idx];
                    nimg = b.n_images[idx];
                    ngrabs = 0; nl_result = 0;
                    if (b.fmin) b.fmin[idx] = 0.0;
                    if (b.x) for (int k = 0; k < 3; k++) b.x[3 * idx + k] = 0.0;
                    if (b.nevals) b.nevals[idx] = 0;
                    if (nimg < 0) { fail_stage = -nimg; nimg = 0; finish_fail = true; break; }
                    if (nimg > kMaxImages || nimg > b.max_images) { fail_stage = 100; finish_fail = true; break; }
                    for (int k = 0; k < nimg; k++) {
                        const int id = b.images[(size_t)idx * b.max_images + k];
                        bad_id |= (id < 0 || id >= sc.n_views);
                        row[k] = (uint16_t)id;
                    }
                }
                if (bad_id) { fail_stage = 101; finish_fail = true; break; }
                op = OPL_ADD;
                stage = S_ADD1;
                break;
            }
            case S_ADD1: {
                nimg = res_n;
                if (nimg < 0) { fail_stage = 100; finish_fail = true; break; }
                if (nimg < o.MIN_IMAGES_PER_PATCH) { fail_stage = 1; finish_fail = true; break; }
                op = OP_INCC; req_ref = 0; req_robust = 0; req_thr = o.NCC_ALPHA_1;
                stage = S_F1;
                break;
            }
            case S_F1:
                op = OPL_F1;
                stage = S_F1B;
                break;
            case S_F1B: {
                nimg = res_n;
                if (res_fail) { fail_stage = res_fail; finish_fail = true; break; }
                set_optimization_fields(sc.views[row[0]], c, F);
                op = OPQ_START;
                stage = S_BQ;
                break;
            }
            case S_BQ:
                op = OPQ_STEP;
                break;
            case S_BQFAIL:
                fail_stage = 4; finish_fail = true;
                break;
            case S_ADD2: {
                nimg = res_n;
                if (nimg < 0) { fail_stage = 100; finish_fail = true; break; }
                if (nimg < o.MIN_IMAGES_PER_PATCH) { fail_stage = 5; finish_fail = true; break; }
                op = OP_INCC; req_ref = 0; req_robust = 0; req_thr = o.NCC_ALPHA_2;
                stage = S_F2;
                break;
            }
            case S_F2:
                op = OPL_F2;
                stage = S_F2B;
                break;
            case S_F2B: {
                nimg = res_n;
                if (res_fail) { fail_stage = res_fail; finish_fail = true; break; }
                ii = 0; refindex = -1; refbest = 3.402823466e+38f;
                op = OP_REFSUM; req_ref = 0; req_robust = 1;
                stage = S_RS;
                if (kProxy) {
                    gfloat* ctx = (gfloat*)aux + kAuxCtx;
                    ctx[0] = scale; ctx[1] = __int_as_float(nimg);
                    for (int k = 0; k < 3; k++) { ctx[2 + k] = c[k]; ctx[5 + k] = n[k]; }
                }
                break;
            }
            case S_RS: {
                if (res_sum < refbest) { refbest = res_sum; refindex = ii; }
                ii++;
                if (kProxy) {
                    for (int k = 0; k < extra; k++) {
                        const float sx = (float)aux[kAuxVal + k];
                        ngrabs += (int)aux[kAuxGrabs + k];
                        if (sx < refbest) { refbest = sx; refindex = ii; }
                        ii++;
                    }
                    extra = 0;
                }
                if (ii < nimg) { op = OP_REFSUM; req_ref = ii; req_robust = 1; break; }
                if (refindex > 0) {
                    const uint16_t t = row[0];
                    row[0] = row[refindex];
                    row[refindex] = t;
                }
                op = OP_INCC; req_ref = 0; req_robust = 0; req_thr = o.NCC_ALPHA_2;
                stage = S_F3;
                break;
            }
            case S_F3:
                op = OPL_F3;
                stage = S_F3B;
                break;
            case S_F3B: {
                nimg = res_n;
                if (res_fail) { fail_stage = res_fail; finish_fail = true; break; }
                finish_ok = true;
                break;
            }
            default: stage = S_IDLE; break;
            }
            if (finish_ok || finish_fail) {
                if (service) {
                    srec[0] = finish_ok ? 1u : 0u; srec[1] = (unsigned)(finish_ok ? 0 : fail_stage); srec[2] = (unsigned)nl_result;
                    srec[4] = (unsigned)ngrabs; srec[5] = (unsigned)(finish_ok ? nimg : 0);
                    if (finish_ok) {
                        for (int k = 0; k < 3; k++) { srec[8 + k] = __float_as_uint(c[k]); srec[12 + k] = __float_as_uint(n[k]); srec[16 + k] = __float_as_uint(res_rgb[k]); }
                        srec[11] = __float_as_uint(1.0f); srec[15] = __float_as_uint(0.0f);
                        srec[19] = __float_as_uint(1.4f);
                        for (int k = 0; k < nimg && k < b.max_images; k++) srec[32 + k] = row[k];
                    }
                    fin_idx = idx; fin_pending = true; yield = true;
                } else {
                    b.ok[idx] = finish_ok ? 1 : (fail_stage == 100 ? 2 : 0);
                    if (finish_ok) {
                        for (int k = 0; k < 3; k++) { b.center[4 * idx + k] = c[k]; b.normal[4 * idx + k] = n[k]; }
                        b.center[4 * idx + 3] = 1.0f;
                        b.normal[4 * idx + 3] = 0.0f;
                        b.n_images[idx] = nimg;
                        for (int k = 0; k < nimg && k < b.max_images; k++) b.images[(size_t)idx * b.max_images + k] = row[k];
                        if (b.color) { b.color[3 * idx] = res_rgb[0]; b.color[3 * idx + 1] = res_rgb[1]; b.color[3 * idx + 2] = res_rgb[2]; }
                        if (b.ncc) b.ncc[idx] = 1.4f;
                    }
                    if (b.stage) b.stage[idx] = finish_ok ? 0 : fail_stage;
                    if (b.result) b.result[idx] = nl_result;
                    if (b.ngrabs) b.ngrabs[idx] = ngrabs;
                }
                stage = S_FETCH;
            }
        }
        if (service) {
            const unsigned long long fm = __ballot(fin_pending);
            if (fm) {
                asm volatile("s_waitcnt vmcnt(0)" ::: "memory");
                for (unsigned long long t = fm; t; t &= t - 1ull) {
                    const int p = __ffsll((long long)t) - 1;
                    const int pidx = bcast_i(fin_idx, p);
                    const uint32_t* src = b.svc_stage + ((size_t)gw * kP + p) * kSvcOutDwords;
                    uint32_t* dst = b.svc_out + (size_t)pidx * kSvcOutDwords;
                    const uint32_t v0 = __hip_atomic_load(src + lane, __ATOMIC_RELAXED, __HIP_MEMORY_SCOPE_AGENT);
                    const uint32_t v1 = lane < kSvcOutDwords - 64 ? __hip_atomic_load(src + 64 + lane, __ATOMIC_RELAXED, __HIP_MEMORY_SCOPE_AGENT) : 0u;
                    __hip_atomic_store(dst + lane, v0, __ATOMIC_RELAXED, __HIP_MEMORY_SCOPE_SYSTEM);
                    if (lane < kSvcOutDwords - 64) __hip_atomic_store(dst + 64 + lane, v1, __ATOMIC_RELAXED, __HIP_MEMORY_SCOPE_SYSTEM);
                }
                asm volatile("s_waitcnt vmcnt(0)" ::: "memory");
                if (fin_pending) __hip_atomic_store(&b.svc_done[fin_idx], 1, __ATOMIC_RELAXED, __HIP_MEMORY_SCOPE_SYSTEM);
                fin_pending = false;
            }
        }
        {
            wave_lds_sync();
            const unsigned long long lm = __ballot(op >= OPL_ADD && op <= OPL_F3);
            if (lm) {
                BQ_PROF_BEGIN(tls_);
                for (unsigned long long t = lm; t; t &= t - 1ull) {
                    const int p = __ffsll((long long)t) - 1;
                    const int kind = bcast_i(op, p);
                    uint16_t* prow = lists + p * kRow;
                    const int pn = bcast_i(nimg, p);
                    const U3 pc{bcast_f(c[0], p), bcast_f(c[1], p), bcast_f(c[2], p)};
                    const U3 pnrm{bcast_f(n[0], p), bcast_f(n[1], p), bcast_f(n[2], p)};
                    const float pscale = bcast_f(scale, p);
                    const unsigned long long pmask = bcast_u64(res_mask, p);
                    ListResult r;
                    r.nimg = 0; r.fail = 0; r.rgb = U3{0.0f, 0.0f, 0.0f};
                    const ListEnv le = list_env(sc, o);
                    if (kind == OPL_ADD) r.nimg = coop_add_images(le, prow, pn, pc, pnrm, pscale);
                    else if (kind == OPL_F1) r = coop_list_f1(le, prow, pn, pmask, pc, pnrm, pscale);
                    else if (kind == OPL_F2) r = coop_list_f2(le, prow, pn, pmask, pc, pnrm);
                    else { LevelThr lt; for (int k = 0; k < kMaxLevels; k++) lt.t[k] = sc.lvl_thr[k]; r = coop_list_f3(sc.views, lt, o.MIN_IMAGES_PER_PATCH, prow, pn, pmask, pc, pscale, b.max_images, service || b.color != nullptr); }
                    if (lane == p) {
                        res_n = r.nimg; res_fail = r.fail;
                        res_rgb[0] = r.rgb.x; res_rgb[1] = r.rgb.y; res_rgb[2] = r.rgb.z;
                        op = OP_NONE;
                    }
                }
                wave_lds_sync();
                BQ_PROF_END(tls_, 24);
                continue;
            }
        }
        if (__any(op >= OPQ_START)) {
            const bool mine = op >= OPQ_START;
            double x0[3] = {0, 0, 0}, dx[3] = {1, 1, 1};
            if (op == OPQ_START) {
                parameters_from_center_norm(F, o, n, lbv, ubv, x0);
                bq_default_step(x0, lbv, ubv, dx);
            }
            if (!held) {
                BQ_PROF_BEGIN(tpg_);
                int got = 0;
                if (lane == 0) {
                    int r = R > 1 ? wv % R : 0;
                    for (;;) {
                        if (atomicCAS(&hpmvs_lock[r], 0, 1 + wv) == 0) break;
                        r = r + 1 == R ? 0 : r + 1;
                        if (r == (R > 1 ? wv % R : 0)) __builtin_amdgcn_s_sleep(HPMVS_LOCK_SLEEP);
                    }
                    got = r;
                }
                reg = __builtin_amdgcn_readfirstlane(got);
                __builtin_amdgcn_fence(__ATOMIC_ACQUIRE, "workgroup");
                __builtin_amdgcn_wave_barrier();
                BQ_PROF_END(tpg_, 25);
                B.slot = (lane < kP ? lane : 0) + reg * (HPMVS_REGION_16 * 2);
                B.slot_i = (lane < kP ? lane : 0) + reg * (HPMVS_REGION_16 * 4);
                BQ_PROF_BEGIN(tpi_);
                if (parked) page_in(park, hpmvs_dyn + reg * HPMVS_REGION_16);
                BQ_PROF_END(tpi_, 27);
                held = true;
                solo = W - __popc((unsigned)hpmvs_lock[R] & ((1u << W) - 1u)) <= R;
            }
#if HPMVS_BQ_PRIO
            __builtin_amdgcn_s_setprio(HPMVS_BQ_PRIO);
#endif
            int ret = BQ_DONE;
#ifdef HPMVS_HOLD_DELAY
            for (int dly = 0; dly < HPMVS_HOLD_DELAY; dly++) __builtin_amdgcn_s_sleep(127);
#endif
            if (kProxy) {
                if (op == OPQ_START) {
                    ret = bq_start(B, x0, lbv, ubv, dx, 1.e-7, 1000, (double*)(unsigned long long)aux);
                    pre_nf = ret == BQ_CONTINUE ? 1 : 0; pre_ctx = false;
                }
                const bool pre = op == OPQ_STEP && pre_nf > 0;
                bool stepping = op == OPQ_STEP;
                double fcur = res_f;
                int kx = 0;
                for (;;) {
                    if (stepping) { ret = bq_step(B, fcur); pre_nf += pre ? 1 : 0; }
                    stepping = pre && kx < extra && ret == BQ_CONTINUE;
                    if (!__any(stepping)) break;
                    if (stepping) { fcur = (double)aux[kAuxVal + kx]; ngrabs += (int)aux[kAuxGrabs + kx]; kx++; }
                }
                if (pre) { if (pre_nf > 7 || ret != BQ_CONTINUE) pre_nf = 0; extra = 0; }
            } else {
                if (op == OPQ_START) ret = bq_start(B, x0, lbv, ubv, dx, 1.e-7, 1000);
                if (op == OPQ_STEP) ret = bq_step(B, res_f);
            }
            double xe[3] = {0, 0, 0};
            if (mine) {
                for (int k = 0; k < 3; k++) xe[k] = BQA(xeval, k);
                if (ret != BQ_CONTINUE) {
                    nl_result = BQN(rc);
                    if (service) {
                        const unsigned long long mf = (unsigned long long)__double_as_longlong((double)BQS(minf));
                        srec[3] = (unsigned)BQN(nevals);
                        srec[20] = (unsigned)mf; srec[21] = (unsigned)(mf >> 32);
                        for (int k = 0; k < 3; k++) {
                            const unsigned long long xv = (unsigned long long)__double_as_longlong(xe[k]);
                            srec[22 + 2 * k] = (unsigned)xv; srec[23 + 2 * k] = (unsigned)(xv >> 32);
                        }
                    } else {
                        if (b.fmin) b.fmin[idx] = BQS(minf);
                        if (b.x) for (int k = 0; k < 3; k++) b.x[3 * idx + k] = xe[k];
                        if (b.nevals) b.nevals[idx] = BQN(nevals);
                    }
                }
            }
            if (!solo) {
                BQ_PROF_BEGIN(tpo_);
                page_out(park, reg);
                parked = true;
                __builtin_amdgcn_fence(__ATOMIC_RELEASE, "workgroup");
                __builtin_amdgcn_wave_barrier();
                if (lane == 0) atomicExch(&hpmvs_lock[reg], 0);
                held = false;
                BQ_PROF_END(tpo_, 26);
            }
#if HPMVS_BQ_PRIO
            __builtin_amdgcn_s_setprio(HPMVS_A_PRIO);
#endif
            {
                const bool cont = mine && ret == BQ_CONTINUE;
                const bool failed = mine && !cont && (op == OPQ_START || !(nl_result >= 1 && nl_result <= 4));
                const bool done = mine && !cont && !failed;
                int nset = (cont || done) ? 1 : 0;
                const int pfirst = pre_nf;
                if (kProxy) {
                    const bool anyfree = __any(!mine && op == OP_NONE && lane < kP && (stage == S_IDLE || (service && stage == S_WAIT)));
                    if (anyfree && cont && pre_nf >= 1 && pre_nf <= 6 && !pre_ctx) { nset = 8 - pre_nf; pre_ctx = true; }
                }
                for (int k = 0; __any(k < nset); k++) {
                    if (k < nset) {
                        double xk[3] = {xe[0], xe[1], xe[2]};
                        float ck[3], nk[3];
                        if (kProxy && k > 0) for (int i3 = 0; i3 < 3; i3++) xk[i3] = aux[3 * (pfirst + k - 2) + i3];
                        set_center_norm(F, o, xk, ck, nk);
                        if (k == 0) { for (int i3 = 0; i3 < 3; i3++) { c[i3] = ck[i3]; n[i3] = nk[i3]; } }
                        else if (kProxy) {
                            gfloat* ctx = (gfloat*)aux + kAuxCtx + 8 + 6 * (pfirst + k - 2);
                            for (int i3 = 0; i3 < 3; i3++) { ctx[i3] = ck[i3]; ctx[3 + i3] = nk[i3]; }
                            gfloat* c0 = (gfloat*)aux + kAuxCtx;
                            c0[0] = scale; c0[1] = __int_as_float(nimg);
                        }
                    }
                }
                if (cont) op = OP_OBJ;
                else if (failed) { op = OP_NONE; stage = S_BQFAIL; }
                else if (done) { op = OPL_ADD; stage = S_ADD2; }
            }
            if (__any((op == OP_NONE && stage != S_IDLE) || (op >= OPL_ADD && op <= OPL_F3))) continue;
        }
        const uint16_t* brow = row;
        if (kProxy) {
            unsigned long long freem = __ballot(op == OP_NONE && lane < kP && (stage == S_IDLE || (service && stage == S_WAIT)) && !fin_pending);
            int want = 0;
            if (op == OP_OBJ && pre_ctx && pre_nf >= 1 && pre_nf <= 6) want = 7 - pre_nf;
            else if (op == OP_REFSUM && stage == S_RS) want = nimg - 1 - req_ref;
            want = want > kMaxExtra ? kMaxExtra : want;
            unsigned long long own = freem ? __ballot(want > 0) : 0ull;
            if (own) {
                for (; own && freem; own &= own - 1ull) {
                    const int p = __ffsll((long long)own) - 1;
                    const int w = bcast_i(want, p);
                    int cnt = 0;
                    for (; cnt < w && freem; cnt++, freem &= freem - 1ull)
                        if (lane == __ffsll((long long)freem) - 1) { px_owner = p; px_k = cnt; }
                    if (lane == p) extra = cnt;
                }
                const int src = px_owner >= 0 ? px_owner : lane;
                const int o_op = shfl_i(op, src), o_ref = shfl_i(req_ref, src), o_pre = shfl_i(pre_nf, src);
                if (px_owner >= 0) {
                    brow = lists + px_owner * kRow;
                    const gfloat* ctx = (const gfloat*)(auxw + px_owner * kAuxDoubles) + kAuxCtx;
                    scale = ctx[0]; nimg = __float_as_int(ctx[1]);
                    const gfloat* cn = (o_op == OP_OBJ) ? ctx + 8 + 6 * (o_pre - 1 + px_k) : ctx + 2;
                    for (int k = 0; k < 3; k++) { c[k] = cn[k]; n[k] = cn[3 + k]; }
                    if (o_op == OP_OBJ) op = OP_OBJ;
                    else { op = OP_REFSUM; req_ref = o_ref + 1 + px_k; req_robust = 1; }
                }
            }
        }
        BQ_PROF_BEGIN(tax_);
        if (op != OP_NONE) {
            const DevView& RV = sc.views[brow[op == OP_OBJ ? 0 : req_ref]];
            calc_patch_axes(RV.xaxis, RV.yaxis, n, scale, ax, ay, az);
        }
        BQ_PROF_END(tax_, 17);
        wave_lds_sync();
        unsigned long long pending = __ballot(op != OP_NONE);
#ifdef HPMVS_PROFILE_PHASES
        { const long long t1 = clock64(); tA += t1 - t0; t0 = t1; nrounds++; nreq += __popcll(pending); }
#endif
        if (pending == 0ull) {
            if (service && (__any(stage != S_IDLE) || (gw == 0 && !svc_closed))) {
                if (gw == 0) __builtin_amdgcn_s_sleep(32);
                else { __builtin_amdgcn_s_sleep(127); __builtin_amdgcn_s_sleep(127); __builtin_amdgcn_s_sleep(127); }
                continue;
            }
            if (lane == 0) atomicOr(&hpmvs_lock[R], 1 << wv);
            break;
        }
        {
            PackedReq q;
            q.obj_mode = (op == OP_OBJ) ? 1 : 0;
            q.ref = req_ref; q.robust = req_robust; q.nimg = nimg; q.thr = req_thr;
            q.scale = scale;
            for (int k = 0; k < 3; k++) { q.c[k] = c[k]; q.zax[k] = (op == OP_OBJ) ? az[k] : n[k]; q.px[k] = ax[k]; q.py[k] = ay[k]; }
            PackedRes r;
            r.obj = 2.0; r.keep = 0ull; r.incc_sum = 0.0f; r.ngrabs = 0;
            __builtin_amdgcn_s_setprio(0);
            wave_eval_rows<false>(sc, o, brow, pending, q, r, erows);
            __builtin_amdgcn_s_setprio(HPMVS_A_PRIO);
            if (op != OP_NONE) {
                res_f = r.obj;
                res_mask = r.keep;
                res_sum = r.incc_sum;
                ngrabs += r.ngrabs;
                op = OP_NONE;
            }
            if (kProxy) {
                const unsigned long long pm = __ballot(px_owner >= 0);
                if (pm) {
                    for (unsigned long long t = pm; t; t &= t - 1ull) {
                        const int fl = __ffsll((long long)t) - 1;
                        const int p = bcast_i(px_owner, fl), k = bcast_i(px_k, fl), g = bcast_i(r.ngrabs, fl), kind = bcast_i(q.obj_mode, fl);
                        const double vf = bcast_d(res_f, fl);
                        const float vs = bcast_f(res_sum, fl);
                        if (lane == p) { aux[kAuxVal + k] = kind ? vf : (double)vs; aux[kAuxGrabs + k] = (double)g; }
                    }
                    asm volatile("s_waitcnt vmcnt(0)" ::: "memory");
                    px_owner = -1;
                }
            }
        }
        wave_lds_sync();
#ifdef HPMVS_PROFILE_PHASES
        { const long long t1 = clock64(); tB += t1 - t0; t0 = t1; }
#endif
    }
#ifdef HPMVS_PROFILE_PHASES
    unsigned long long* dbg = (unsigned long long*)(queue + 4);
    if (lane == 0) {
        atomicAdd(&dbg[0], (unsigned long long)tA);
        atomicAdd(&dbg[1], (unsigned long long)tB);
        atomicAdd(&dbg[2], (unsigned long long)nrounds);
        atomicAdd(&dbg[3], (unsigned long long)nreq);
    }
    __syncthreads();
    if (threadIdx.x == 0)
        for (int k = 0; k < 64; k++) atomicAdd(&dbg[4 + k], s_prof[k]);
#endif
}

__global__ void __launch_bounds__(64 * HPMVS_WG_WAVES, HPMVS_WAVES_PER_EU) HPMVS_VK(optimize_kernel)(DevScene sc, DevOptions o, DevBatch b, int32_t* queue) {
    optimize_body<false, HPMVS_WG_WAVES, HPMVS_WG_REGIONS>(sc, o, b, queue);
}
#ifndef HPMVS_VARIANT_SUFFIX
__global__ void __launch_bounds__(128, HPMVS_WAVES_PER_EU) optimize_service_kernel(DevScene sc, DevOptions o, DevBatch b, int32_t* queue) {
    optimize_body<true, 2, 1>(sc, o, b, queue);
}
#endif

static size_t lds_bytes(int regions) { return (size_t)regions * HPMVS_REGION_16 * 16 + (size_t)(regions + 1) * sizeof(int); }

static int max_workgroups(int n_cus, int waves, int regions) {
    int lds_per_wg = (int)lds_bytes(regions);
#ifdef HPMVS_PROFILE_PHASES
    lds_per_wg += 64 * 8;
#endif
    lds_per_wg = (lds_per_wg + 511) & ~511;
    int per_cu = (160 * 1024) / lds_per_wg;
    if (per_cu > 4 * HPMVS_WAVES_PER_EU / waves) per_cu = 4 * HPMVS_WAVES_PER_EU / waves;
    return n_cus * per_cu;
}

size_t HPMVS_V(optimize_workspace_bytes)(int n_cus) {
    const size_t waves = (size_t)HPMVS_WG_WAVES * max_workgroups(n_cus, HPMVS_WG_WAVES, HPMVS_WG_REGIONS);
    return kCounterBytes + waves * kP * kRow * sizeof(uint16_t) + waves * (size_t)kPark16 * 16 + waves * kP * kRow * sizeof(float) +
           waves * (size_t)(HPMVS_COLD_GLOBAL ? (164 - HPMVS_STATE_ND) : 0) * kP * sizeof(double) +
           (HPMVS_PROXY == 2 ? waves * kP * kAuxDoubles * sizeof(double) : 0);
}

#ifndef HPMVS_VARIANT_SUFFIX
size_t optimize_workspace_bytes_for(int wgs) {
    return kCounterBytes + (size_t)2 * wgs * kP * kRow * sizeof(uint16_t) + (size_t)2 * wgs * (size_t)kPark16 * 16 +
           (size_t)2 * wgs * kP * kRow * sizeof(float) + (size_t)2 * wgs * (size_t)(HPMVS_COLD_GLOBAL ? (164 - HPMVS_STATE_ND) : 0) * kP * sizeof(double) +
           (HPMVS_PROXY ? (size_t)2 * wgs * kP * kAuxDoubles * sizeof(double) : 0);
}
size_t optimize_stage_bytes_for(int wgs) { return (size_t)2 * wgs * kP * kSvcOutDwords * sizeof(uint32_t); }
void launch_optimize_service(const DevScene& sc, const DevOptions& o, const DevBatch& b, int32_t* workspace, int wgs,
                             hipStream_t st) {
    hipLaunchKernelGGL(optimize_service_kernel, dim3(wgs), dim3(128), lds_bytes(1), st, sc, o, b, workspace);
}
#endif

void HPMVS_V(launch_optimize)(const DevScene& sc, const DevOptions& o, const DevBatch& b, int32_t* workspace, int n_cus,
                     hipStream_t st) {
    if (b.n <= 0) return;
    int wgs = b.n;
    const int cap = max_workgroups(n_cus, HPMVS_WG_WAVES, HPMVS_WG_REGIONS);
    if (wgs > cap) wgs = cap;
    static std::atomic<unsigned long long> attr_done{0ull};
    int dev = 0;
    if (hipGetDevice(&dev) == hipSuccess && dev >= 0 && dev < 64 && !((attr_done.load(std::memory_order_relaxed) >> dev) & 1ull)) {
        (void)hipFuncSetAttribute((const void*)HPMVS_VK(optimize_kernel), hipFuncAttributeMaxDynamicSharedMemorySize, (int)lds_bytes(HPMVS_WG_REGIONS));
        attr_done.fetch_or(1ull << dev, std::memory_order_relaxed);
    }
    hipLaunchKernelGGL(HPMVS_VK(optimize_kernel), dim3(wgs), dim3(64 * HPMVS_WG_WAVES), lds_bytes(HPMVS_WG_REGIONS), st, sc, o, b, workspace);
}

}
```

hpmvs_amd/csrc/photometric.hpp:

```cpp
#pragma once
#include <hip/hip_runtime.h>

#include "cr_acos.hpp"
#include "dev_types.h"

#include "prof.h"
#if defined(HPMVS_PROFILE_PHASES) && defined(__HIP_DEVICE_COMPILE__)
#define PH_T(v) const long long v = clock64()
#define PH_ADD(v0, v1, i) do { if (__lane_id() == 0) { atomicAdd(&s_prof[2 * (i)], (unsigned long long)((v1) - (v0))); atomicAdd(&s_prof[2 * (i) + 1], 1ull); } } while (0)
#else
#define PH_T(v) do { } while (0)
#define PH_ADD(v0, v1, i) do { } while (0)
#endif

namespace hpmvs {


__device__ __forceinline__ int lane_id() { return (int)__lane_id(); }

__device__ __forceinline__ float bcast_f(float v, int src_lane) {
    return __int_as_float(__builtin_amdgcn_readlane(__float_as_int(v), src_lane));
}
__device__ __forceinline__ int bcast_i(int v, int src_lane) { return __builtin_amdgcn_readlane(v, src_lane); }
__device__ __forceinline__ double bcast_d(double v, int src_lane) {
    const long long b = __double_as_longlong(v);
    const int lo = __builtin_amdgcn_readlane((int)(b & 0xffffffffll), src_lane);
    const int hi = __builtin_amdgcn_readlane((int)(b >> 32), src_lane);
    return __longlong_as_double(((long long)hi << 32) | (unsigned int)lo);
}
__device__ __forceinline__ const uint8_t* bcast_p(const uint8_t* p, int src_lane) {
    const unsigned long long b = (unsigned long long)p;
    const unsigned int lo = (unsigned int)__builtin_amdgcn_readlane((int)(b & 0xffffffffull), src_lane);
    const unsigned int hi = (unsigned int)__builtin_amdgcn_readlane((int)(b >> 32), src_lane);
    return (const uint8_t*)(((unsigned long long)hi << 32) | lo);
}

__device__ __forceinline__ int cvt_i32_x86(float v) { return (v >= -2147483648.0f && v < 2147483648.0f) ? (int)v : (int)0x80000000; }
__device__ __forceinline__ int cvt_i32_x86(double v) { return (v > -2147483649.0 && v < 2147483648.0) ? (int)v : (int)0x80000000; }


__device__ __forceinline__ float dot3f(const float* a, const float* b) { return (a[0] * b[0] + a[1] * b[1]) + a[2] * b[2]; }
__device__ __forceinline__ void cross3f(const float* a, const float* b, float* r) {
    const float r0 = a[1] * b[2] - a[2] * b[1];
    const float r1 = a[2] * b[0] - a[0] * b[2];
    const float r2 = a[0] * b[1] - a[1] * b[0];
    r[0] = r0; r[1] = r1; r[2] = r2;
}
__device__ __forceinline__ void normalized3f(const float* a, float* r) {
    const float n2 = dot3f(a, a);
    if (n2 > 0.0f) { const float n = sqrtf(n2); r[0] = a[0] / n; r[1] = a[1] / n; r[2] = a[2] / n; }
    else { r[0] = a[0]; r[1] = a[1]; r[2] = a[2]; }
}

__device__ __forceinline__ void calc_patch_axes(const float* cam_xaxis, const float* cam_yaxis, const float* n,
                                                float scale, float* px, float* py, float* pz) {
    float t[3], x[3], y[3];
    normalized3f(n, pz);
    cross3f(pz, cam_xaxis, t); normalized3f(t, y);
    cross3f(y, pz, t); normalized3f(t, x);
    for (int k = 0; k < 3; k++) { x[k] *= scale; y[k] *= scale; }
    float yn[3], yan[3];
    normalized3f(y, yn); normalized3f(cam_yaxis, yan);
    const float fs = dot3f(yn, yan);
    for (int k = 0; k < 3; k++) { px[k] = x[k]; py[k] = y[k] * fs; }
}

__device__ __forceinline__ void project0(const float* P, float X0, float X1, float X2, float& u, float& v) {
    const float r0 = ((P[0] * X0 + P[1] * X1) + P[2] * X2) + P[3];
    const float r1 = ((P[4] * X0 + P[5] * X1) + P[6] * X2) + P[7];
    const float r2 = ((P[8] * X0 + P[9] * X1) + P[10] * X2) + P[11];
    const float lo = -2147483648.0f, hi = 2147483648.0f;
    const float uu = fmaxf(lo, fminf(hi, r0 / r2)), vv = fmaxf(lo, fminf(hi, r1 / r2));
    const bool behind = r2 <= 0.0f;
    u = behind ? -65535.0f : uu;
    v = behind ? -65535.0f : vv;
}

__device__ __forceinline__ int level_clamped(const DevScene& sc, float scale, float fsum, float fz, int max_level) {
    const double r = (double)(scale * fsum) / (2.0 * (double)fz);
    int lvl = 0;
#pragma unroll
    for (int k = 0; k < kMaxLevels - 1; k++)
        if (k < max_level && r >= sc.lvl_thr[k]) lvl++;
    return lvl;
}

struct Prep {
    int ok;
    float tlx, tly;
    float dxx, dxy;
    float dyx, dyy;
    const uint8_t* pix;
    int W;
};

constexpr int kGrabLevels = 5;
struct ViewRegs { float P[12]; float cx, cy, cz, fsum; int w0, h0; const uint8_t* pix0; const DevView* vp; };
__device__ __forceinline__ ViewRegs load_view(const DevView& V) {
    ViewRegs r;
#pragma unroll
    for (int k = 0; k < 12; k++) r.P[k] = V.P0[k];
    r.cx = V.center[0]; r.cy = V.center[1]; r.cz = V.center[2];
    r.fsum = V.fsum; r.w0 = V.w[0]; r.h0 = V.h[0];
    r.pix0 = V.pix[0];
    r.vp = &V;
    return r;
}
__device__ __forceinline__ Prep prep_from_view(const DevScene& sc, const ViewRegs& V, const DevOptions& o, const float* c, float scale,
                                               const float* pxa, const float* pya, const float* zax) {
    Prep r;
    const float d0 = V.cx - c[0], d1 = V.cy - c[1], d2 = V.cz - c[2];
    const float n2 = (d0 * d0 + d1 * d1) + d2 * d2;
    const float nn = sqrtf(n2);
    const float g_unit = ((d0 / nn) * zax[0] + (d1 / nn) * zax[1]) + (d2 / nn) * zax[2];
    const float g_raw = (d0 * zax[0] + d1 * zax[1]) + d2 * zax[2];
    const float g = (n2 > 0.0f) ? g_unit : g_raw;
    const bool angle_ok = !((double)g < o.cos_max_d);
    const int lvl = level_clamped(sc, scale, V.fsum, nn, o.MAXLEVEL - 1);
    {
        unsigned ofs = 0u;
#pragma unroll
        for (int k = 0; k < kGrabLevels - 1; k++) {
            const unsigned nb = (3u * (unsigned)(V.w0 >> k) * (unsigned)(V.h0 >> k) + 16u + 255u) & ~255u;
            ofs += (k < lvl) ? nb : 0u;
        }
        r.pix = (lvl < kGrabLevels) ? V.pix0 + ofs : V.vp->pix[lvl];
    }
    float cu, cv, xu, xv, yu, yv;
    project0(V.P, c[0], c[1], c[2], cu, cv);
    project0(V.P, c[0] + pxa[0], c[1] + pxa[1], c[2] + pxa[2], xu, xv);
    project0(V.P, c[0] + pya[0], c[1] + pya[1], c[2] + pya[2], yu, yv);
    const float s = __int_as_float((127 - lvl) << 23);
    cu *= s; cv *= s;
    const float dxx = xu * s - cu, dxy = xv * s - cv;
    const float dyx = yu * s - cu, dyy = yv * s - cv;
    const float hs = 3.5f;
    const float tlx = (cu - hs * dxx) - hs * dyx, tly = (cv - hs * dxy) - hs * dyy;
    const float trx = (cu + hs * dxx) - hs * dyx, try_ = (cv + hs * dxy) - hs * dyy;
    const float blx = (cu - hs * dxx) + hs * dyx, bly = (cv - hs * dxy) + hs * dyy;
    const float brx = (cu + hs * dxx) + hs * dyx, bry = (cv + hs * dxy) + hs * dyy;
    const float mnx = fminf(fminf(fminf(tlx, trx), blx), brx), mny = fminf(fminf(fminf(tly, try_), bly), bry);
    const float mxx = fmaxf(fmaxf(fmaxf(tlx, trx), blx), brx), mxy = fmaxf(fmaxf(fmaxf(tly, try_), bly), bry);
    const int W = V.w0 >> lvl, H = V.h0 >> lvl;
    const float m = 3.0f;
    const bool box_ok = !(mnx < m || mny < m || mxx >= (float)(W - 3) || mxy >= (float)(H - 3));
    r.ok = (angle_ok && box_ok) ? 1 : 0;
    r.tlx = tlx; r.tly = tly; r.dxx = dxx; r.dxy = dxy; r.dyx = dyx; r.dyy = dyy;
    r.W = W;
    return r;
}

__device__ __forceinline__ uint2 load8(const uint8_t* p) {
    typedef __attribute__((address_space(1))) const uint8_t gbyte;
    gbyte* g = (gbyte*)(unsigned long long)p;
    uint2 v;
    __builtin_memcpy(&v, g, 8);
    return v;
}

__device__ __forceinline__ double recip64(float w) { return 1.0 / (double)w; }
__device__ __forceinline__ float div_by(float a, double inv_w) { return (float)((double)a * inv_w); }

__device__ __forceinline__ float robustincc(float rhs) { return rhs / (1 + 3 * rhs); }

struct PackedReq {
    int obj_mode;
    int ref, robust, nimg;
    float thr;
    float c[3], zax[3], scale, px[3], py[3];
};
struct PackedRes {
    double obj;
    unsigned long long keep;
    float incc_sum;
    int ngrabs;
};

__device__ __forceinline__ void wave_lds_sync() {
    __builtin_amdgcn_fence(__ATOMIC_RELEASE, "wavefront");
    __builtin_amdgcn_wave_barrier();
    __builtin_amdgcn_fence(__ATOMIC_ACQUIRE, "wavefront");
}

__device__ __forceinline__ float shfl_f(float v, int src_lane) {
    return __int_as_float(__builtin_amdgcn_ds_bpermute(src_lane << 2, __float_as_int(v)));
}
__device__ __forceinline__ int shfl_i(int v, int src_lane) { return __builtin_amdgcn_ds_bpermute(src_lane << 2, v); }
__device__ __forceinline__ unsigned long long bcast_u64(unsigned long long v, int src_lane) {
    const unsigned int lo = (unsigned int)__builtin_amdgcn_readlane((int)(v & 0xffffffffull), src_lane);
    const unsigned int hi = (unsigned int)__builtin_amdgcn_readlane((int)(v >> 32), src_lane);
    return ((unsigned long long)hi << 32) | lo;
}

struct Taps { uint2 a, b; float f00, f01, f10, f11; };

__device__ __forceinline__ void texel(const Taps& t, float& r, float& g, float& b) {
    r = (float)(t.a.x & 0xff) * t.f00 + (float)(t.b.x & 0xff) * t.f01;
    g = (float)((t.a.x >> 8) & 0xff) * t.f00 + (float)((t.b.x >> 8) & 0xff) * t.f01;
    b = (float)((t.a.x >> 16) & 0xff) * t.f00 + (float)((t.b.x >> 16) & 0xff) * t.f01;
    r += (float)(t.a.x >> 24) * t.f10 + (float)(t.b.x >> 24) * t.f11;
    g += (float)(t.a.y & 0xff) * t.f10 + (float)(t.b.y & 0xff) * t.f11;
    b += (float)((t.a.y >> 8) & 0xff) * t.f10 + (float)((t.b.y >> 8) & 0xff) * t.f11;
}

typedef float v2f __attribute__((ext_vector_type(2)));
__device__ __forceinline__ void texel_pair(uint2 aA, uint2 bA, float wxA, float wyA, uint2 aB, uint2 bB, float wxB, float wyB,
                                           float* outA, float* outB) {
    const v2f dx1 = {wxA, wxB}, dy1 = {wyA, wyB};
    const v2f one = {1.0f, 1.0f};
    const v2f dx0 = one - dx1, dy0 = one - dy1;
    const v2f f00 = dx0 * dy0, f01 = dx0 * dy1, f10 = dx1 * dy0, f11 = dx1 * dy1;
#define HPMVS_B(v, sh) (float)(((v) >> (sh)) & 0xffu)
    const v2f r00 = {HPMVS_B(aA.x, 0), HPMVS_B(aB.x, 0)}, r01 = {HPMVS_B(bA.x, 0), HPMVS_B(bB.x, 0)};
    const v2f g00 = {HPMVS_B(aA.x, 8), HPMVS_B(aB.x, 8)}, g01 = {HPMVS_B(bA.x, 8), HPMVS_B(bB.x, 8)};
    const v2f b00 = {HPMVS_B(aA.x, 16), HPMVS_B(aB.x, 16)}, b01 = {HPMVS_B(bA.x, 16), HPMVS_B(bB.x, 16)};
    const v2f r10 = {(float)(aA.x >> 24), (float)(aB.x >> 24)}, r11 = {(float)(bA.x >> 24), (float)(bB.x >> 24)};
    const v2f g10 = {HPMVS_B(aA.y, 0), HPMVS_B(aB.y, 0)}, g11 = {HPMVS_B(bA.y, 0), HPMVS_B(bB.y, 0)};
    const v2f b10 = {HPMVS_B(aA.y, 8), HPMVS_B(aB.y, 8)}, b11 = {HPMVS_B(bA.y, 8), HPMVS_B(bB.y, 8)};
#undef HPMVS_B
    const v2f r = (r00 * f00 + r01 * f01) + (r10 * f10 + r11 * f11);
    const v2f g = (g00 * f00 + g01 * f01) + (g10 * f10 + g11 * f11);
    const v2f b = (b00 * f00 + b01 * f01) + (b10 * f10 + b11 * f11);
    outA[0] = r.x; outA[1] = g.x; outA[2] = b.x;
    outB[0] = r.y; outB[1] = g.y; outB[2] = b.y;
}

constexpr int kGroups = 9;
#ifndef HPMVS_JOB_SETS
#define HPMVS_JOB_SETS 2
#endif
constexpr int kJobSets = HPMVS_JOB_SETS;
constexpr int kRowVals = 3 * kTex;
constexpr int kFinChunk = 8;

__device__ __forceinline__ float lane_prev(float v) {
    return __int_as_float(__builtin_amdgcn_update_dpp(0, __float_as_int(v), 0x138, 0xf, 0xf, true));
}

template <int N>
__device__ __forceinline__ float row_chain(const float (&v)[N]) {
    float out = 0.0f;
#pragma unroll
    for (int s = 0; s < kTex; s++) {
        float a = (s == 0) ? 0.0f : lane_prev(out);
#pragma unroll
        for (int i = 0; i < N; i++) a += v[i];
        out = a;
    }
    return out;
}

template <int N>
__device__ __forceinline__ void row_chain_pair(const float (&va)[N], const float (&vb)[N], float& outa, float& outb) {
    v2f out = {0.0f, 0.0f};
#pragma unroll
    for (int s = 0; s < kTex; s++) {
        v2f a;
        if (s == 0) { a.x = 0.0f; a.y = 0.0f; }
        else { a.x = lane_prev(out.x); a.y = lane_prev(out.y); }
#pragma unroll
        for (int i = 0; i < N; i++) { const v2f t = {va[i], vb[i]}; a = a + t; }
        out = a;
    }
    outa = out.x; outb = out.y;
}

#ifndef HPMVS_FAST_SUMS
#define HPMVS_FAST_SUMS 0
#endif
#ifndef HPMVS_SPLIT_PREP
#define HPMVS_SPLIT_PREP 1
#endif
#ifndef HPMVS_SINGLE_FAST
#define HPMVS_SINGLE_FAST 1
#endif
#ifndef HPMVS_TAKE_OVER
#define HPMVS_TAKE_OVER 1
#endif
template <int N>
__device__ __forceinline__ float window_sum(const float (&v)[N]) {
#if HPMVS_FAST_SUMS
    float a = v[0];
#pragma unroll
    for (int i = 1; i < N; i++) a += v[i];
    float out = a;
#pragma unroll
    for (int s = 1; s < kTex; s++) out = lane_prev(out) + a;
    return out;
#else
    return row_chain<N>(v);
#endif
}
__device__ __forceinline__ void mean_chains(const float (&vr)[kTex], const float (&vg)[kTex], const float (&vb)[kTex],
                                            float& s0, float& s1, float& s2) {
#if HPMVS_FAST_SUMS
    s0 = window_sum<kTex>(vr); s1 = window_sum<kTex>(vg); s2 = window_sum<kTex>(vb);
#else
    row_chain_pair<kTex>(vr, vg, s0, s1);
    s2 = row_chain<kTex>(vb);
#endif
}

#ifndef HPMVS_SCAN_BATCHES
#define HPMVS_SCAN_BATCHES 1
#endif
__device__ __forceinline__ int wave_scan_add(int v) {
    v += __builtin_amdgcn_update_dpp(0, v, 0x111, 0xf, 0xf, true);
    v += __builtin_amdgcn_update_dpp(0, v, 0x112, 0xf, 0xf, true);
    v += __builtin_amdgcn_update_dpp(0, v, 0x114, 0xf, 0xf, true);
    v += __builtin_amdgcn_update_dpp(0, v, 0x118, 0xf, 0xf, true);
    v += __builtin_amdgcn_update_dpp(0, v, 0x142, 0xa, 0xf, false);
    v += __builtin_amdgcn_update_dpp(0, v, 0x143, 0xc, 0xf, false);
    return v;
}

__device__ __forceinline__ int wave_max_i32(int v) {
#pragma unroll
    for (int d = 1; d < 64; d <<= 1) { const int o = __shfl_xor(v, d, 64); v = o > v ? o : v; }
    return v;
}

struct GlobalRows {
    float* base; int stride;
    typedef __attribute__((address_space(1))) float gfloat;
    __device__ __forceinline__ void store(int p, int k, float v) const { ((gfloat*)(unsigned long long)(base + (size_t)p * stride))[k] = v; }
    __device__ __forceinline__ float load(int p, int k) const { return ((const gfloat*)(unsigned long long)(base + (size_t)p * stride))[k]; }
};
struct LdsRows {
    float* base; int stride;
    typedef __attribute__((address_space(3))) float lfloat;
    __device__ __forceinline__ void store(int p, int k, float v) const { ((lfloat*)base)[p * stride + k] = v; }
    __device__ __forceinline__ float load(int p, int k) const { return ((const lfloat*)base)[p * stride + k]; }
};

template <bool WRITE_INCCS, typename ListT, typename Rows>
__device__ __forceinline__ void wave_eval_rows(const DevScene& sc, const DevOptions& o, const ListT* list,
                                               unsigned long long pending, const PackedReq& q, PackedRes& out,
                                               const Rows rows) {
    const int lane = lane_id();
    const int grp = lane / kTex;
    const int yy = lane - grp * kTex;
    const bool glane = grp < kGroups;
    const int last = glane ? grp * kTex + (kTex - 1) : lane;
    const int gl0 = lane - yy;
    const int q_refsel = q.obj_mode ? 0 : q.ref;
    const int q_userob = (q.obj_mode || q.robust) ? 1 : 0;
    const unsigned long long listbits = (unsigned long long)list;
    const int list_lo = (int)(listbits & 0xffffffffull), list_hi = (int)(listbits >> 32);

    unsigned long long rem = pending;
    while (rem) {
#if HPMVS_SCAN_BATCHES
        const bool inrem = (rem >> lane) & 1ull;
        const int mynp = inrem ? q.nimg : 0;
        const int incl = wave_scan_add(mynp);
        const int excl = incl - mynp;
        const int j_rem = bcast_i(incl, 63);
        const int n_batches = (j_rem + 64 * kJobSets - 1) / (64 * kJobSets);
        const int j_target = n_batches > 1 ? (j_rem + n_batches - 1) / n_batches : 64 * kJobSets;
        const int first = __ffsll((long long)rem) - 1;
        const unsigned long long stop = __ballot(inrem && lane != first && (incl > 64 * kJobSets || excl >= j_target));
        const unsigned long long batch = stop ? (rem & ((1ull << (__ffsll((long long)stop) - 1)) - 1ull)) : rem;
        const int lastb = 63 - __clzll(batch);
        const int J = bcast_i(incl, lastb);
        rem &= ~batch;
        PH_T(t1);
        const int myoff = excl;
        int jp[kJobSets], ji[kJobSets];
        {
            int lo[kJobSets];
#pragma unroll
            for (int k = 0; k < kJobSets; k++) lo[k] = 0;
#pragma unroll
            for (int step = 32; step >= 1; step >>= 1) {
                int v[kJobSets];
#pragma unroll
                for (int k = 0; k < kJobSets; k++) v[k] = shfl_i(incl, lo[k] + step - 1);
#pragma unroll
                for (int k = 0; k < kJobSets; k++) lo[k] += (v[k] <= lane + 64 * k) ? step : 0;
            }
#pragma unroll
            for (int k = 0; k < kJobSets; k++) {
                const int j = lane + 64 * k;
                const int e = shfl_i(excl, lo[k] & 63);
                const bool has = j < J;
                jp[k] = has ? lo[k] : -1;
                ji[k] = has ? j - e : 0;
            }
        }
#else
        int j_rem = 0;
        for (unsigned long long t = rem; t; t &= t - 1ull) j_rem += bcast_i(q.nimg, __ffsll((long long)t) - 1);
        const int n_batches = (j_rem + 64 * kJobSets - 1) / (64 * kJobSets);
        const int j_target = n_batches > 1 ? (j_rem + n_batches - 1) / n_batches : 64 * kJobSets;
        unsigned long long batch = 0ull;
        int J = 0;
        for (unsigned long long t = rem; t; t &= t - 1ull) {
            const int p = __ffsll((long long)t) - 1;
            const int np = bcast_i(q.nimg, p);
            if (batch && (J + np > 64 * kJobSets || J >= j_target)) break;
            batch |= 1ull << p;
            J += np;
        }
        rem &= ~batch;
        PH_T(t1);
        int myoff = 0;
        int jp[kJobSets], ji[kJobSets];
#pragma unroll
        for (int k = 0; k < kJobSets; k++) { jp[k] = -1; ji[k] = 0; }
        {
            int off = 0;
            for (unsigned long long t = batch; t; t &= t - 1ull) {
                const int p = __ffsll((long long)t) - 1;
                const int np = bcast_i(q.nimg, p);
                if (lane == p) myoff = off;
#pragma unroll
                for (int k = 0; k < kJobSets; k++) {
                    const int j = lane + 64 * k;
                    if (j >= off && j < off + np) { jp[k] = p; ji[k] = j - off; }
                }
                off += np;
            }
        }
#endif
        Prep PS[kJobSets];
        unsigned long long okS[kJobSets];
        int pix_lo[kJobSets], pix_hi[kJobSets];
        {
            float jc[kJobSets][3], jz[kJobSets][3], jx[kJobSets][3], jy[kJobSets][3], jscale[kJobSets];
            int jid[kJobSets];
#pragma unroll
            for (int k = 0; k < kJobSets; k++) {
                jid[k] = 0; jscale[k] = 1.0f;
                for (int a3 = 0; a3 < 3; a3++) { jc[k][a3] = 0.0f; jz[k][a3] = 0.0f; jx[k][a3] = 0.0f; jy[k][a3] = 0.0f; }
                if (J > 64 * k) {
                    const int src = jp[k] >= 0 ? jp[k] : 0;
#pragma unroll
                    for (int a3 = 0; a3 < 3; a3++) {
                        jc[k][a3] = shfl_f(q.c[a3], src); jz[k][a3] = shfl_f(q.zax[a3], src);
                        jx[k][a3] = shfl_f(q.px[a3], src); jy[k][a3] = shfl_f(q.py[a3], src);
                    }
                    jscale[k] = shfl_f(q.scale, src);
                    const unsigned long long lb = ((unsigned long long)(unsigned int)shfl_i(list_hi, src) << 32) |
                                                  (unsigned long long)(unsigned int)shfl_i(list_lo, src);
                    if (jp[k] >= 0) jid[k] = (int)((const ListT*)lb)[ji[k]];
                }
            }
            ViewRegs VR[kJobSets];
#pragma unroll
            for (int k = 0; k < kJobSets; k++) {
                VR[k] = ViewRegs{};
                if (k == 0 || J > 64) VR[k] = load_view(sc.views[jid[k]]);
            }
#if HPMVS_SPLIT_PREP == 2
#pragma unroll
            for (int k = 0; k < kJobSets; k++) {
                PS[k] = Prep{};
                if (k == 0 || J > 64) PS[k] = prep_from_view(sc, VR[k], o, jc[k], jscale[k], jx[k], jy[k], jz[k]);
            }
#else
            if (kJobSets == 1 || !HPMVS_SPLIT_PREP || J > 64) {
#pragma unroll
                for (int k = 0; k < kJobSets; k++) PS[k] = prep_from_view(sc, VR[k], o, jc[k], jscale[k], jx[k], jy[k], jz[k]);
            } else {
                PS[0] = prep_from_view(sc, VR[0], o, jc[0], jscale[0], jx[0], jy[0], jz[0]);
#pragma unroll
                for (int k = 1; k < kJobSets; k++) PS[k] = Prep{};
            }
#endif
#pragma unroll
            for (int k = 0; k < kJobSets; k++) {
                PS[k].ok = (J > 64 * k && jp[k] >= 0) ? PS[k].ok : 0;
                okS[k] = __ballot(PS[k].ok != 0);
                const unsigned long long pb = (unsigned long long)PS[k].pix;
                pix_lo[k] = (int)(pb & 0xffffffffull); pix_hi[k] = (int)(pb >> 32);
            }
        }

        const bool inbatch = (batch >> lane) & 1ull;
        unsigned long long myok = 0ull;
        if (inbatch) {
            unsigned long long lo = 0ull;
            const int w = myoff >> 6, sh = myoff & 63;
#pragma unroll
            for (int k = 0; k < kJobSets; k++) {
                if (k == w) lo |= okS[k] >> sh;
                if (k == w + 1 && sh > 0) lo |= okS[k] << (64 - sh);
            }
            myok = (q.nimg >= 64) ? lo : (lo & ((1ull << q.nimg) - 1ull));
        }
        const bool refok = inbatch && q.nimg > 0 && ((myok >> q_refsel) & 1ull);
        unsigned long long todo = __ballot(refok);
        const int mylen = __popcll(myok);
        const unsigned long long len6 = __ballot(mylen >= 6), len4 = __ballot(mylen >= 4);
#if defined(HPMVS_PROFILE_PHASES) && defined(__HIP_DEVICE_COMPILE__)
        {
            int mx = 0, tot = 0, longreq = 0;
            for (unsigned long long t = todo; t; t &= t - 1ull) {
                const int pp = __ffsll((long long)t) - 1;
                const int l = bcast_i(mylen, pp);
                mx = l > mx ? l : mx; tot += l;
                longreq += (l > 8 && !bcast_i(q.obj_mode, pp)) ? 1 : 0;
            }
            if (lane == 0) {
                atomicAdd(&s_prof[60], (unsigned long long)mx); atomicAdd(&s_prof[61], (unsigned long long)((tot + kGroups - 1) / kGroups));
                atomicAdd(&s_prof[62], 1ull); atomicAdd(&s_prof[63], (unsigned long long)longreq);
            }
        }
#endif
        PH_T(t2);
        PH_ADD(t1, t2, 13);

        int g_req = -1, g_off = 0, g_ref = 0, g_userob = 0, g_cur = 0;
        bool g_isref = false;
        unsigned long long g_ok = 0ull;
        float refn[kRowVals];
#pragma unroll
        for (int i = 0; i < kRowVals; i++) refn[i] = 0.0f;

        bool single = HPMVS_SINGLE_FAST && __popcll(todo) == 1;
        for (;;) {
            PH_T(t3);
            int rsrc = lane;
            bool moved = false;
            {
                unsigned long long idle = __ballot(glane && yy == 0 && g_req < 0);
                while (todo && idle) {
                    const unsigned long long c6 = todo & len6, c4 = todo & len4;
                    const int p = __ffsll((long long)(c6 ? c6 : (c4 ? c4 : todo))) - 1;
                    todo &= ~(1ull << p);
                    const int gl = __ffsll((long long)idle) - 1;
                    idle &= idle - 1ull;
                    const int r_off = bcast_i(myoff, p), r_ref = bcast_i(q_refsel, p), r_rob = bcast_i(q_userob, p);
                    const unsigned long long r_ok = bcast_u64(myok, p);
                    if (gl0 == gl) {
                        g_req = p; g_off = r_off; g_ref = r_ref; g_userob = r_rob;
                        g_ok = r_ok & ~(1ull << r_ref);
                        g_cur = r_ref; g_isref = true;
                    }
                }
                if (single) {
                    single = false;
                    const unsigned long long nonref = bcast_u64(g_ok, 0);
                    const int n_other = __popcll(nonref);
                    const int nh = n_other < kGroups - 1 ? n_other : kGroups - 1;
                    if (nh > 0) {
                        const int r_req = bcast_i(g_req, 0), r_off = bcast_i(g_off, 0), r_ref = bcast_i(g_ref, 0), r_rob = bcast_i(g_userob, 0);
                        unsigned long long mine = nonref, rest = nonref;
#pragma unroll
                        for (int i = 1; i < kGroups; i++) {
                            if (i < grp) mine &= mine - 1ull;
                            if (i <= nh) rest &= rest - 1ull;
                        }
                        if (grp == 0) g_ok = rest;
                        else if (glane && grp <= nh) {
                            g_req = r_req; g_off = r_off; g_ref = r_ref; g_userob = r_rob;
                            g_cur = __ffsll((long long)mine) - 1; g_ok = 0ull; g_isref = false; rsrc = yy;
                        }
                        moved = true;
                        idle = 0ull;
                    }
                }
                while (HPMVS_TAKE_OVER && idle) {
                    const int left = (glane && g_req >= 0) ? __popcll(g_ok) : 0;
                    int best = 0, n_best = 0;
                    unsigned long long vmask = 0ull;
#pragma unroll
                    for (int g = 0; g < kGroups; g++) {
                        const int l = bcast_i(left, g * kTex);
                        if (l > best) { best = l; n_best = 0; vmask = 0ull; }
                        if (l == best && l > 0) { n_best++; vmask |= 1ull << (g * kTex); }
                    }
                    if (best < 1 || __popcll(idle) < n_best) break;
                    for (unsigned long long t = vmask; t; t &= t - 1ull) {
                        const int vl = __ffsll((long long)t) - 1;
                        const int tl = __ffsll((long long)idle) - 1;
                        idle &= idle - 1ull;
                        const int take = (best + 1) / 2;
                        unsigned long long hi = bcast_u64(g_ok, vl);
                        for (int i = 0; i < best - take; i++) hi &= hi - 1ull;
                        const int r_req = bcast_i(g_req, vl), r_off = bcast_i(g_off, vl), r_ref = bcast_i(g_ref, vl), r_rob = bcast_i(g_userob, vl);
                        const int r_src = bcast_i(rsrc, vl);
                        if (gl0 == vl) g_ok &= ~hi;
                        if (gl0 == tl && glane) {
                            g_req = r_req; g_off = r_off; g_ref = r_ref; g_userob = r_rob;
                            g_cur = __ffsll((long long)hi) - 1; g_ok = hi & (hi - 1ull); g_isref = false; rsrc = r_src + yy;
                        }
                    }
                    moved = true;
                }
            }
            const bool act = glane && g_req >= 0;
            if (!__any(act)) break;

            float tlx, tly, dxx, dxy, dyx, dyy;
            const uint8_t* pix;
            int W;
            {
                const int j = g_off + g_cur;
                const int src = j & 63, set = j >> 6;
                tlx = shfl_f(PS[0].tlx, src); tly = shfl_f(PS[0].tly, src);
                dxx = shfl_f(PS[0].dxx, src); dxy = shfl_f(PS[0].dxy, src);
                dyx = shfl_f(PS[0].dyx, src); dyy = shfl_f(PS[0].dyy, src);
                W = shfl_i(PS[0].W, src);
                int plo = shfl_i(pix_lo[0], src), phi = shfl_i(pix_hi[0], src);
#pragma unroll
                for (int k = 1; k < kJobSets; k++) {
                    if (J > 64 * k) {
                        const bool sb = set == k;
                        const float b0 = shfl_f(PS[k].tlx, src), b1 = shfl_f(PS[k].tly, src), b2 = shfl_f(PS[k].dxx, src),
                                    b3 = shfl_f(PS[k].dxy, src), b4 = shfl_f(PS[k].dyx, src), b5 = shfl_f(PS[k].dyy, src);
                        const int b6 = shfl_i(PS[k].W, src), b7 = shfl_i(pix_lo[k], src), b8 = shfl_i(pix_hi[k], src);
                        tlx = sb ? b0 : tlx; tly = sb ? b1 : tly; dxx = sb ? b2 : dxx; dxy = sb ? b3 : dxy;
                        dyx = sb ? b4 : dyx; dyy = sb ? b5 : dyy; W = sb ? b6 : W; plo = sb ? b7 : plo; phi = sb ? b8 : phi;
                    }
                }
                pix = (const uint8_t*)(((unsigned long long)(unsigned int)phi << 32) | (unsigned long long)(unsigned int)plo);
            }

            float t[kRowVals];
            {
                float x = tlx, y = tly;
#pragma unroll
                for (int k = 0; k < kTex - 1; k++) { const float m = (k < yy) ? 1.0f : 0.0f; x = __builtin_fmaf(m, dyx, x); y = __builtin_fmaf(m, dyy, y); }
                uint2 ta[kTex], tb[kTex];
                float wx[kTex], wy[kTex];
                int toff[kTex];
#pragma unroll
                for (int xx = 0; xx < kTex; xx++) {
                    const int lx = (int)x, ly = (int)y;
                    wx[xx] = x - (float)lx; wy[xx] = y - (float)ly;
                    toff[xx] = 3 * (ly * W + lx);
                    ta[xx] = make_uint2(0u, 0u); tb[xx] = make_uint2(0u, 0u);
                    x += dxx; y += dxy;
                }
                if (act) {
#pragma unroll
                    for (int xx = 0; xx < kTex; xx++) {
                        const uint8_t* p0 = pix + toff[xx];
                        ta[xx] = load8(p0);
                        tb[xx] = load8(p0 + 3 * W);
                    }
                }
#pragma unroll
                for (int xx = 0; xx + 1 < kTex; xx += 2)
                    texel_pair(ta[xx], tb[xx], wx[xx], wy[xx], ta[xx + 1], tb[xx + 1], wx[xx + 1], wy[xx + 1], &t[3 * xx], &t[3 * xx + 3]);
                {
                    const int xx = kTex - 1;
                    Taps tp;
                    tp.a = ta[xx]; tp.b = tb[xx];
                    const float dx1 = wx[xx], dx0 = 1.0f - dx1;
                    const float dy1 = wy[xx], dy0 = 1.0f - dy1;
                    tp.f00 = dx0 * dy0; tp.f01 = dx0 * dy1; tp.f10 = dx1 * dy0; tp.f11 = dx1 * dy1;
                    texel(tp, t[3 * xx], t[3 * xx + 1], t[3 * xx + 2]);
                }
            }
            PH_T(t4);
            PH_ADD(t3, t4, 14);

            float a0, a1, a2;
            {
                float vr[kTex], vg[kTex], vb[kTex];
#pragma unroll
                for (int xx = 0; xx < kTex; xx++) { vr[xx] = t[3 * xx]; vg[xx] = t[3 * xx + 1]; vb[xx] = t[3 * xx + 2]; }
                float s0, s1, s2;
                mean_chains(vr, vg, vb, s0, s1, s2);
                a0 = div_by(shfl_f(s0, last), 1.0 / 49.0);
                a1 = div_by(shfl_f(s1, last), 1.0 / 49.0);
                a2 = div_by(shfl_f(s2, last), 1.0 / 49.0);
            }
            double iv;
            {
                float sq[kTex];
#pragma unroll
                for (int xx = 0; xx < kTex; xx++) {
                    const float f0 = a0 - t[3 * xx], f1 = a1 - t[3 * xx + 1], f2 = a2 - t[3 * xx + 2];
                    sq[xx] = f0 * f0 + f1 * f1 + f2 * f2;
                }
                float v2 = sqrtf(div_by(shfl_f(window_sum<kTex>(sq), last), 1.0 / 147.0));
                if (v2 == 0.0f) v2 = 1.0f;
                iv = recip64(v2);
            }
            PH_T(t5);
            PH_ADD(t4, t5, 15);
#pragma unroll
            for (int xx = 0; xx < kTex; xx++) {
                t[3 * xx] = div_by(t[3 * xx] - a0, iv);
                t[3 * xx + 1] = div_by(t[3 * xx + 1] - a1, iv);
                t[3 * xx + 2] = div_by(t[3 * xx + 2] - a2, iv);
            }
            float raw = 0.0f, rob = 0.0f;
#pragma unroll
            for (int i = 0; i < kRowVals; i++) refn[i] = g_isref ? t[i] : refn[i];
            if (moved) {
#pragma unroll
                for (int i = 0; i < kRowVals; i++) refn[i] = shfl_f(refn[i], rsrc);
            }
            PH_T(t6);
            PH_ADD(t5, t6, 20);
            if (__any(act && !g_isref)) {
                float pr[kRowVals];
#pragma unroll
                for (int i = 0; i < kRowVals; i++) pr[i] = refn[i] * t[i];
                raw = 1.0f - div_by(shfl_f(window_sum<kRowVals>(pr), last), 1.0 / 147.0);
                rob = robustincc(raw);
            }
            PH_T(t7);
            PH_ADD(t6, t7, 21);

            if (act) {
                if (!g_isref && yy == 0) rows.store(g_req, g_cur, g_userob ? rob : raw);
                if (g_ok) { g_cur = __ffsll((long long)g_ok) - 1; g_ok &= g_ok - 1ull; g_isref = false; }
                else g_req = -1;
            }
            PH_T(t8);
            PH_ADD(t7, t8, 22);
        }

        PH_T(t9);
        asm volatile("s_waitcnt vmcnt(0) lgkmcnt(0)" ::: "memory");
        __builtin_amdgcn_wave_barrier();
        if (inbatch && !refok) {
            if (q.obj_mode) out.obj = 2.0;
            else {
                float s = 0.0f;
                for (int k = 0; k < q.nimg; k++) s += 2.0f;
                out.keep = 0ull;
                out.incc_sum = s;
            }
        }
        {
            const bool fin = inbatch && refok;
            const float thr1 = 1.0f - q.thr;
            double val = 0.0;
            int nok = 0;
            float s = 0.0f;
            unsigned long long keep = 0ull;
            const int kmax = rows.stride - 1;
            for (int k0 = 0; __any(fin && k0 < q.nimg); k0 += kFinChunk) {
                float e[kFinChunk];
#pragma unroll
                for (int j = 0; j < kFinChunk; j++) e[j] = 2.0f;
                if (fin && k0 < q.nimg) {
#pragma unroll
                    for (int j = 0; j < kFinChunk; j++) { const int kk = k0 + j < kmax ? k0 + j : kmax; e[j] = rows.load(lane, kk); }
                }
#pragma unroll
                for (int j = 0; j < kFinChunk; j++) {
                    const int k = k0 + j;
                    const bool in = fin && k < q.nimg;
                    const bool okk = (myok >> (k & 63)) & 1ull;
                    const bool isref = k == q_refsel;
                    const unsigned long long bit = 1ull << (k & 63);
                    const bool add_o = in && okk && !isref;
                    val += add_o ? (double)e[j] : 0.0;
                    nok += add_o ? 1 : 0;
                    const float v = okk ? e[j] : 2.0f;
                    s += (in && !isref) ? v : 0.0f;
                    const bool kp = in && (isref ? (0.0f < thr1) : (v < thr1));
                    keep |= kp ? bit : 0ull;
                }
            }
            if (fin) {
                out.ngrabs += mylen;
                if (q.obj_mode) out.obj = (nok < o.MIN_IMAGES_PER_PATCH - 1) ? 2.0 : val / (double)nok;
                else {
                    out.keep = WRITE_INCCS ? myok : keep;
                    out.incc_sum = s;
                    if (WRITE_INCCS) rows.store(lane, q_refsel, 0.0f);
                }
            }
        }
        PH_T(t10);
        PH_ADD(t9, t10, 16);
    }
}



struct OptFields {
    float refCenter[3];
    float refRay[3];
    float imgX[3], imgY[3], imgZ[3];
};

__device__ __forceinline__ void set_optimization_fields(const DevView& V0, const float* c, OptFields& F) {
    normalized3f(V0.xaxis, F.imgX);
    normalized3f(V0.yaxis, F.imgY);
    normalized3f(V0.zaxis, F.imgZ);
    F.refCenter[0] = c[0]; F.refCenter[1] = c[1]; F.refCenter[2] = c[2];
    const float d[3] = {c[0] - V0.center[0], c[1] - V0.center[1], c[2] - V0.center[2]};
    normalized3f(d, F.refRay);
}

__device__ __forceinline__ void sincos_halfpi(double a, double& s, double& c) {
    const double z = a * a;
    double ps = -1.0 / 51090942171709440000.0;
    ps = ps * z + 1.0 / 121645100408832000.0;
    ps = ps * z - 1.0 / 355687428096000.0;
    ps = ps * z + 1.0 / 1307674368000.0;
    ps = ps * z - 1.0 / 6227020800.0;
    ps = ps * z + 1.0 / 39916800.0;
    ps = ps * z - 1.0 / 362880.0;
    ps = ps * z + 1.0 / 5040.0;
    ps = ps * z - 1.0 / 120.0;
    ps = ps * z + 1.0 / 6.0;
    s = a - a * z * ps;
    double pc = 1.0 / 1124000727777607680000.0;
    pc = pc * z - 1.0 / 2432902008176640000.0;
    pc = pc * z + 1.0 / 6402373705728000.0;
    pc = pc * z - 1.0 / 20922789888000.0;
    pc = pc * z + 1.0 / 87178291200.0;
    pc = pc * z - 1.0 / 479001600.0;
    pc = pc * z + 1.0 / 3628800.0;
    pc = pc * z - 1.0 / 40320.0;
    pc = pc * z + 1.0 / 720.0;
    pc = pc * z - 1.0 / 24.0;
    pc = pc * z + 0.5;
    c = 1.0 - z * pc;
}

__device__ __forceinline__ void set_center_norm(const OptFields& F, const DevOptions& o, const double* x, float* c,
                                                float* n) {
    const float x0 = (float)x[0];
    for (int k = 0; k < 3; k++) c[k] = F.refCenter[k] + (x0 * F.refRay[k]) * 1.0f;
    const float angle1 = (float)(x[1] * (double)o.angle_scale);
    const float angle2 = (float)(x[2] * (double)o.angle_scale);
    double s1, c1, s2, c2;
    sincos_halfpi((double)angle1, s1, c1);
    sincos_halfpi((double)angle2, s2, c2);
    const float fx = (float)(s1 * c2);
    const float fy = (float)s2;
    const float fz = (float)(-c1 * c2);
    for (int k = 0; k < 3; k++) n[k] = (F.imgX[k] * fx + F.imgY[k] * fy) + F.imgZ[k] * fz;
}

__device__ __forceinline__ float asinf_glibc(float x) {
    const float one = 1.0f, pio2_hi = 1.57079637050628662109375f, pio2_lo = -4.37113900018624283e-8f,
                pio4_hi = 0.785398185253143310546875f;
    const float p0 = 1.666675248e-1f, p1 = 7.495297643e-2f, p2 = 4.547037598e-2f, p3 = 2.417951451e-2f,
                p4 = 4.216630880e-2f;
    const int hx = __float_as_int(x);
    const int ix = hx & 0x7fffffff;
    if (ix == 0x3f800000) return x * pio2_hi + x * pio2_lo;
    if (ix > 0x3f800000) return (x - x) / (x - x);
    if (ix < 0x3f000000) {
        if (ix < 0x32000000) return x;
        const float t = x * x;
        const float w = t * (p0 + t * (p1 + t * (p2 + t * (p3 + t * p4))));
        return x + x * w;
    }
    float w = one - fabsf(x);
    float t = w * 0.5f;
    float p = t * (p0 + t * (p1 + t * (p2 + t * (p3 + t * p4))));
    const float s = sqrtf(t);
    if (ix >= 0x3F79999A) {
        t = pio2_hi - (2.0f * (s + s * p) - pio2_lo);
    } else {
        w = __int_as_float(__float_as_int(s) & 0xfffff000);
        const float c = (t - w * w) / (s + w);
        const float r = p;
        p = 2.0f * s * r - (pio2_lo - 2.0f * c);
        const float q = pio4_hi - 2.0f * w;
        t = pio4_hi - (p - q);
    }
    return hx > 0 ? t : -t;
}

__device__ __forceinline__ void parameters_from_center_norm(const OptFields& F, const DevOptions& o, const float* n,
                                                            const double* lb, const double* ub, double* x) {
    x[0] = 0.0;
    const float fx = dot3f(F.imgX, n), fy = dot3f(F.imgY, n), fz = dot3f(F.imgZ, n);
    x[2] = (double)asinf_glibc(fy);
    double t = (x[2] < 1.0) ? x[2] : 1.0;
    t = (-1.0 < t) ? t : -1.0;
    const float cosb = (float)cos(t);
    if (cosb == 0.0f) x[1] = 0.0;
    else {
        const double sina = (double)(fx / cosb);
        const double cosa = (double)(-fz / cosb);
        double u = (-1.0 < cosa) ? cosa : -1.0;
        u = (u < 1.0) ? u : 1.0;
        x[1] = cra::acos_cr(u, acos(u));
        if (sina < 0.0) x[1] = -x[1];
    }
    x[1] /= (double)o.angle_scale;
    x[2] /= (double)o.angle_scale;
    for (int k = 0; k < 3; k++) {
        const double v = (lb[k] < x[k]) ? x[k] : lb[k];
        x[k] = (v < ub[k]) ? v : ub[k];
    }
}


}
```

hpmvs_amd/csrc/pipeline.hpp:

```cpp
#pragma once
#include <hip/hip_runtime.h>

#include "dev_types.h"
#include "photometric.hpp"

namespace hpmvs {

namespace {

enum Op { OP_NONE = 0, OP_OBJ = 1, OP_INCC = 2, OP_REFSUM = 3,
          OPL_ADD = 4, OPL_F1 = 5, OPL_F2 = 6, OPL_F3 = 7,
          OPQ_START = 8, OPQ_STEP = 9 };
enum Stage {
    S_FETCH = 0, S_WAIT, S_ADD1, S_F1, S_F1B, S_BQ, S_BQFAIL, S_ADD2, S_F2, S_F2B, S_RS, S_F3, S_F3B, S_IDLE
};

struct U3 { float x, y, z; };

struct LevelThr { double t[kMaxLevels]; };
struct ListEnv {
    const DevView* views; const int32_t* covis_off; const int32_t* covis;
    float cos_max_f, sort_thr, MAX_ANGLE, MIN_ANGLE;
    int32_t MAXLEVEL, MINLEVEL, MIN_IMAGES_PER_PATCH;
};
__device__ __forceinline__ ListEnv list_env(const DevScene& sc, const DevOptions& o) {
    return ListEnv{sc.views, sc.covis_off, sc.covis, o.cos_max_f, o.sort_thr, o.MAX_ANGLE, o.MIN_ANGLE, o.MAXLEVEL, o.MINLEVEL, o.MIN_IMAGES_PER_PATCH};
}

__device__ __forceinline__ void ray_to_cam(const DevView& V, const float* c, float* ray) {
    const float d[3] = {V.center[0] - c[0], V.center[1] - c[1], V.center[2] - c[2]};
    normalized3f(d, ray);
}

__device__ __forceinline__ unsigned long long lanes_below(int lane) { return (1ull << lane) - 1ull; }

__device__ __forceinline__ int compact_list(int& id, unsigned long long keep) {
    const int lane = lane_id();
    int nid = -1, m = 0;
    for (unsigned long long t = keep; t; t &= t - 1ull, m++) {
        const int v = bcast_i(id, __ffsll((long long)t) - 1);
        if (lane == m) nid = v;
    }
    id = nid;
    return m;
}

__device__ __forceinline__ float wave_min_f32(float v) {
#define HPMVS_MIN_DPP(ctrl, rows) v = fminf(v, __int_as_float(__builtin_amdgcn_update_dpp(__float_as_int(v), __float_as_int(v), ctrl, rows, 0xf, false)))
    HPMVS_MIN_DPP(0x111, 0xf);
    HPMVS_MIN_DPP(0x112, 0xf);
    HPMVS_MIN_DPP(0x114, 0xf);
    HPMVS_MIN_DPP(0x118, 0xf);
    HPMVS_MIN_DPP(0x142, 0xa);
    HPMVS_MIN_DPP(0x143, 0xc);
#undef HPMVS_MIN_DPP
    return bcast_f(v, 63);
}

template <class OP>
__device__ __forceinline__ bool add_images_test(const DevView& V, const OP& o, const float* c, const float* n, float scale) {
    float ray[3];
    ray_to_cam(V, c, ray);
    if (dot3f(ray, n) < o.cos_max_f) return false;
    const float dd[3] = {c[0] - V.center[0], c[1] - V.center[1], c[2] - V.center[2]};
    const float fz = sqrtf(dot3f(dd, dd));
    const float lv = (float)log2((double)(scale * V.fsum) / (2.0 * (double)fz));
    const int il = cvt_i32_x86(roundf(lv));
    if (il < o.MINLEVEL || il >= o.MAXLEVEL - 2) return false;
    float P[12];
    for (int k = 0; k < 12; k++) P[k] = V.P0[k];
    float u, v;
    project0(P, c[0], c[1], c[2], u, v);
    const float s = __int_as_float((127 - il) << 23);
    u *= s; v *= s;
    if (u < 0.0f || (float)(V.w[il] - 1) <= u || v < 0.0f || (float)(V.h[il] - 1) <= v) return false;
    return true;
}

__device__ __noinline__ int coop_add_images(ListEnv sc, uint16_t* row, int nimg, U3 c_, U3 n_, float scale) {
    if (nimg <= 0) return 0;
    const int lane = lane_id();
    const float c[3] = {c_.x, c_.y, c_.z}, n[3] = {n_.x, n_.y, n_.z};
    const int id = (lane < nimg) ? (int)row[lane] : -1;
    const int ref = bcast_i(id, 0);
    const int existing = nimg;
    const int beg = sc.covis_off[ref], end = sc.covis_off[ref + 1];
    for (int base = beg; base < end; base += 64) {
        const int ci = base + lane;
        const bool valid = ci < end;
        const int cv = valid ? sc.covis[ci] : -2;
        bool found = false;
        for (int k = 0; k < existing; k++) found |= (bcast_i(id, k) == cv);
        bool pass = false;
        if (valid && !found) pass = add_images_test(sc.views[cv], sc, c, n, scale);
        const unsigned long long m = __ballot(pass);
        const int cnt = __popcll(m);
        if (nimg + cnt > kMaxImages) return -1;
        if (pass) row[nimg + __popcll(m & lanes_below(lane))] = (uint16_t)cv;
        nimg += cnt;
    }
    return nimg;
}

template <class SC, class OP>
__device__ __forceinline__ int coop_sort_images(const SC& sc, const OP& o, int& id, int nimg, const float* c,
                                                const float* n, float scale) {
    const int lane = lane_id();
    bool cand = false;
    float w = 0.0f, ray[3] = {0.0f, 0.0f, 0.0f};
    if (nimg > 0) {
        const DevView& V0 = sc.views[bcast_i(id, 0)];
        const float dd[3] = {c[0] - V0.center[0], c[1] - V0.center[1], c[2] - V0.center[2]};
        const float fz0 = sqrtf(dot3f(dd, dd));
        int refLevel = cvt_i32_x86(roundf((float)log2((double)(scale * V0.fsum) / (2.0 * (double)fz0))));
        refLevel = refLevel < o.MAXLEVEL - 1 ? refLevel : o.MAXLEVEL - 1;
        refLevel = refLevel > 0 ? refLevel : 0;
        float nn[3];
        normalized3f(n, nn);
        if (lane < nimg) {
            const DevView& V = sc.views[id];
            ray_to_cam(V, c, ray);
            const float cosa = dot3f(ray, nn);
            if (cosa > 0.0f) {
                cand = true;
                const float e[3] = {c[0] - V.center[0], c[1] - V.center[1], c[2] - V.center[2]};
                const float fz = sqrtf(dot3f(e, e));
                const float sc_ = (V.fsum == 0.0f) ? 1.0f : (float)(2.0 * (double)fz * (double)(1 << refLevel) / (double)V.fsum);
                w = sc_ / cosa;
            }
        }
    }
    unsigned long long alive = __ballot(cand);
    if (__popcll(alive) < 2) { id = -1; return 0; }
    if (lane == __ffsll((long long)alive) - 1) w = 0.0f;
    const float thr = o.sort_thr;
    int out = 0, nid = -1;
    while (alive) {
        const bool mine = (alive >> lane) & 1ull;
        const float mn = wave_min_f32(mine ? w : __int_as_float(0x7f800000));
        const unsigned long long eq = __ballot(mine && w == mn);
        const int best = __ffsll((long long)(eq ? eq : alive)) - 1;
        const int bid = bcast_i(id, best);
        if (lane == out) nid = bid;
        out++;
        const float rb[3] = {bcast_f(ray[0], best), bcast_f(ray[1], best), bcast_f(ray[2], best)};
        alive &= ~(1ull << best);
        if ((alive >> lane) & 1ull) {
            const float ftmp = fminf(thr, fmaxf(thr / 2.0f, 1.0f - dot3f(rb, ray)));
            w = w * (thr / ftmp);
        }
    }
    id = nid;
    return out;
}

template <class SC, class OP>
__device__ __forceinline__ bool coop_assure_image_angles(const SC& sc, const OP& o, int id, int nimg, const float* c) {
    const int lane = lane_id();
    float rj[3] = {0.0f, 0.0f, 0.0f};
    if (lane < nimg) ray_to_cam(sc.views[id], c, rj);
    for (int ii = 0; ii < nimg - 1; ii++) {
        const float ri[3] = {bcast_f(rj[0], ii), bcast_f(rj[1], ii), bcast_f(rj[2], ii)};
        bool hit = false;
        if (lane > ii && lane < nimg) {
            const float a = acosf(dot3f(ri, rj));
            hit = a < o.MAX_ANGLE && a > o.MIN_ANGLE;
        }
        if (__any(hit)) return true;
    }
    return false;
}

template <class SC, class OP>
__device__ __forceinline__ int coop_filter_images_by_angle(const SC& sc, const OP& o, int& id, int nimg,
                                                           const float* c, const float* n) {
    bool keep = false;
    if (lane_id() < nimg) {
        float ray[3];
        ray_to_cam(sc.views[id], c, ray);
        keep = dot3f(ray, n) > o.cos_max_f;
    }
    return compact_list(id, __ballot(keep));
}

__device__ __forceinline__ void colour_at(const DevScene& sc, const DevView& V, const float* c, float scale, float* rgb) {
    const float dd[3] = {c[0] - V.center[0], c[1] - V.center[1], c[2] - V.center[2]};
    const float fz = sqrtf(dot3f(dd, dd));
    const int lvl = level_clamped(sc, scale, V.fsum, fz, V.n_levels - 1);
    float P[12];
    for (int k = 0; k < 12; k++) P[k] = V.P0[k];
    float x, y;
    project0(P, c[0], c[1], c[2], x, y);
    const float s = __int_as_float((127 - lvl) << 23);
    x *= s; y *= s;
    const int W = V.w[lvl];
    const int lx = (int)x, ly = (int)y;
    const uint8_t* p0 = V.pix[lvl] + 3 * (ly * W + lx);
    const uint8_t* p1 = p0 + 3 * W;
    const float dx1 = x - (float)lx, dx0 = 1.0f - dx1;
    const float dy1 = y - (float)ly, dy0 = 1.0f - dy1;
    const float f00 = dx0 * dy0, f01 = dx0 * dy1, f10 = dx1 * dy0, f11 = dx1 * dy1;
    for (int ch = 0; ch < 3; ch++) {
        float v = (float)p0[ch] * f00 + (float)p1[ch] * f01;
        v += (float)p0[3 + ch] * f10 + (float)p1[3 + ch] * f11;
        rgb[ch] = v;
    }
}

__device__ __forceinline__ U3 coop_patch_colour(const DevScene& sc, int id, int nimg, const float* c, float scale) {
    const int lane = lane_id();
    float rgb[3] = {0.0f, 0.0f, 0.0f}, norm = 0.0f;
    if (lane < nimg) {
        colour_at(sc, sc.views[id], c, scale, rgb);
        norm = sqrtf(dot3f(rgb, rgb));
    }
    int rank = 0;
    for (int j = 0; j < nimg; j++) {
        const float nj = bcast_f(norm, j);
        rank += (nj < norm) || (nj == norm && j < lane);
    }
    const int want = nimg / 2;
    const unsigned long long mm = __ballot(lane < nimg && rank == want), m0 = __ballot(lane < nimg && rank == 0);
    const int med = mm ? __ffsll((long long)mm) - 1 : 0, mn = m0 ? __ffsll((long long)m0) - 1 : 0;
    const int pick = (bcast_f(norm, med) > 250.0f) ? mn : med;
    return U3{bcast_f(rgb[0], pick), bcast_f(rgb[1], pick), bcast_f(rgb[2], pick)};
}

struct ListResult { int nimg; int fail; U3 rgb; };

__device__ __forceinline__ void store_list(uint16_t* row, int id, int nimg) {
    if (lane_id() < nimg) row[lane_id()] = (uint16_t)id;
}

__device__ __noinline__ ListResult coop_list_f1(ListEnv sc, uint16_t* row, int nimg, unsigned long long keep,
                                               U3 c_, U3 n_, float scale) {
    const ListEnv& o = sc;
    const int lane = lane_id();
    const float c[3] = {c_.x, c_.y, c_.z}, n[3] = {n_.x, n_.y, n_.z};
    ListResult r;
    r.fail = 0; r.rgb = U3{0.0f, 0.0f, 0.0f};
    int id = (lane < nimg) ? (int)row[lane] : -1;
    const unsigned long long all = nimg >= 64 ? ~0ull : ((1ull << nimg) - 1ull);
    nimg = compact_list(id, (keep | 1ull) & all);
    r.nimg = nimg;
    if (nimg < o.MIN_IMAGES_PER_PATCH) { r.fail = 2; return r; }
    nimg = coop_sort_images(sc, o, id, nimg, c, n, scale);
    r.nimg = nimg;
    if (!coop_assure_image_angles(sc, o, id, nimg, c)) { r.fail = 3; return r; }
    if (nimg < o.MIN_IMAGES_PER_PATCH) { r.fail = 4; return r; }
    store_list(row, id, nimg);
    return r;
}

__device__ __noinline__ ListResult coop_list_f2(ListEnv sc, uint16_t* row, int nimg, unsigned long long keep,
                                               U3 c_, U3 n_) {
    const ListEnv& o = sc;
    const int lane = lane_id();
    const float c[3] = {c_.x, c_.y, c_.z}, n[3] = {n_.x, n_.y, n_.z};
    ListResult r;
    r.fail = 0; r.rgb = U3{0.0f, 0.0f, 0.0f};
    int id = (lane < nimg) ? (int)row[lane] : -1;
    const unsigned long long all = nimg >= 64 ? ~0ull : ((1ull << nimg) - 1ull);
    nimg = compact_list(id, (keep | 1ull) & all);
    r.nimg = nimg;
    if (nimg < o.MIN_IMAGES_PER_PATCH) { r.fail = 6; return r; }
    nimg = coop_filter_images_by_angle(sc, o, id, nimg, c, n);
    r.nimg = nimg;
    if (nimg < o.MIN_IMAGES_PER_PATCH) { r.fail = 7; return r; }
    if (!coop_assure_image_angles(sc, o, id, nimg, c)) { r.fail = 8; return r; }
    store_list(row, id, nimg);
    return r;
}

__device__ __noinline__ ListResult coop_list_f3(const DevView* views, LevelThr lt, int min_images, uint16_t* row, int nimg, unsigned long long keep,
                                               U3 c_, float scale, int max_images, int want_colour) {
    DevScene sc;
    sc.views = views; sc.covis_off = nullptr; sc.covis = nullptr; sc.n_views = 0;
    for (int k = 0; k < kMaxLevels; k++) sc.lvl_thr[k] = lt.t[k];
    const int lane = lane_id();
    const float c[3] = {c_.x, c_.y, c_.z};
    ListResult r;
    r.fail = 0; r.rgb = U3{0.0f, 0.0f, 0.0f};
    int id = (lane < nimg) ? (int)row[lane] : -1;
    const unsigned long long all = nimg >= 64 ? ~0ull : ((1ull << nimg) - 1ull);
    nimg = compact_list(id, (keep | 1ull) & all);
    r.nimg = nimg;
    if (nimg < min_images) { r.fail = 9; return r; }
    if (nimg > max_images) { r.fail = 100; return r; }
    store_list(row, id, nimg);
    if (want_colour) r.rgb = coop_patch_colour(sc, id, nimg, c, scale);
    return r;
}

}

}
```

include/hpmvs_amd.h:

```cpp
#ifndef HPMVS_AMD_H
#define HPMVS_AMD_H

#include <stddef.h>
#include <stdint.h>

#ifdef __cplusplus
extern "C" {
#endif

#define HPMVS_OK 0
#define HPMVS_ERR_HIP (-1)
#define HPMVS_ERR_ARG (-2)
#define HPMVS_ERR_STATE (-3)
#define HPMVS_ERR_NODEVICE (-4)
#define HPMVS_ERR_UNSUPPORTED (-5)

#define HPMVS_MAX_LEVELS 8
#define HPMVS_MAX_IMAGES 256
#define HPMVS_FAST_IMAGES 64
#define HPMVS_RECORD_IMAGES 64

typedef struct hpmvs_scene hpmvs_scene;

typedef struct {
    int32_t MAXLEVEL;
    int32_t MINLEVEL;
    float MAX_ANGLE;
    float MIN_ANGLE;
    int32_t MAX_IMAGES_PER_PATCH;
    int32_t MIN_IMAGES_PER_PATCH;
    float NCC_ALPHA_1;
    float NCC_ALPHA_2;
} hpmvs_options;

typedef struct {
    float P0[12];
    float center[4];
    float xaxis[3];
    float yaxis[3];
    float zaxis[3];
    float fsum;
    int32_t n_levels;
} hpmvs_camera;

typedef struct {
    int32_t n;
    int32_t max_images;
    float *center;
    float *normal;
    float *scale;
    int32_t *n_images;
    int32_t *images;
    uint8_t *ok;
    float *color;
    float *ncc;
    double *fmin;
    double *x;
    int32_t *result;
    int32_t *nevals;
    int32_t *stage;
    int32_t *ngrabs;
} hpmvs_patch_batch;

const char *hpmvs_last_error(void);
int hpmvs_device_count(void);
const char *hpmvs_build_id(void);
void hpmvs_default_options(hpmvs_options *o);

int hpmvs_camera_from_nvm(double f, const double q_wxyz[4], const double c[3], int width, int height,
                          int max_level, hpmvs_camera *out);

int hpmvs_scene_center(const hpmvs_camera *cams, int n, double center[3], double *radius, int *valid);

int hpmvs_scene_create(int n_views, int device, hpmvs_scene **out);
int hpmvs_scene_set_view(hpmvs_scene *s, int view, int width, int height, const uint8_t *rgb_l0,
                         int rgb_on_device, const hpmvs_camera *cam);
int hpmvs_scene_set_covis(hpmvs_scene *s, int view, const int32_t *ids, int n);
int hpmvs_scene_commit(hpmvs_scene *s);
int hpmvs_scene_destroy(hpmvs_scene *s);
int hpmvs_scene_get_level(const hpmvs_scene *s, int view, int level, uint8_t *host_out, size_t cap,
                          int *w, int *h);
size_t hpmvs_scene_bytes(const hpmvs_scene *s);

int hpmvs_build_pyramid(int device, const uint8_t *src, int w, int h, uint8_t *dst, int on_device);

int hpmvs_undistort(int device, const uint8_t *src, int w, int h, float f, float k1, uint8_t *dst, int on_device);
int hpmvs_undistort_map(int device, int w, int h, float f, float k1, float *xy);
int hpmvs_scene_set_view_distorted(hpmvs_scene *s, int view, int width, int height, const uint8_t *rgb_raw,
                                   int rgb_on_device, const hpmvs_camera *cam, float f, float k1);

int hpmvs_jpeg_info(const uint8_t *bytes, size_t n, int *width, int *height, int *components, int *h_samp, int *v_samp);
int hpmvs_jpeg_decode(int device, const uint8_t *bytes, size_t n, uint8_t *rgb, size_t cap, int rgb_on_device);
int hpmvs_jpeg_decode_timed(int device, const uint8_t *bytes, size_t n, uint8_t *rgb_device, size_t cap, float *ms);
int hpmvs_jpeg_last_decode(int *used, int *rounds);
int hpmvs_jpeg_entropy_timed(int device, const uint8_t *bytes, size_t n, uint8_t *rgb_device, size_t cap, float *ms);
int hpmvs_scene_set_view_jpeg(hpmvs_scene *s, int view, const uint8_t *bytes, size_t n, const hpmvs_camera *cam, float f,
                              float k1);
enum { HPMVS_JPEG_ENTROPY_AUTO = 0, HPMVS_JPEG_ENTROPY_HOST = 1, HPMVS_JPEG_ENTROPY_DEVICE = 2 };
#define HPMVS_JPEG_AUTO_MIN_SCAN_BYTES 445155
int hpmvs_jpeg_decode_ex(int device, const uint8_t *bytes, size_t n, uint8_t *rgb, size_t cap, int rgb_on_device, int entropy,
                         int *used);
int hpmvs_scene_set_view_jpeg_ex(hpmvs_scene *s, int view, const uint8_t *bytes, size_t n, const hpmvs_camera *cam, float f,
                                 float k1, int entropy, int *used);
int hpmvs_jpeg_coefficients(int device, const uint8_t *bytes, size_t n, int entropy, int subseq_bits, int16_t *coef, size_t cap,
                            int *used, int *rounds);

size_t hpmvs_jpeg_encode_bound(int width, int height);
int hpmvs_jpeg_encode(int device, const uint8_t *rgb, int width, int height, int quality, uint8_t *out, size_t cap, size_t *n,
                      int rgb_on_device);
int hpmvs_scene_get_level_jpeg(const hpmvs_scene *s, int view, int level, int quality, uint8_t *out, size_t cap, size_t *n);
int hpmvs_jpeg_encode_timed(int device, const uint8_t *rgb_device, int width, int height, int quality, uint8_t *out, size_t cap,
                            size_t *n, float *ms);

#define HPMVS_DEPTH_COMBINED (-1)
int hpmvs_depth_colormap(uint8_t lut[768]);
int hpmvs_scene_depth_image(const hpmvs_scene *s, int view, int level, uint8_t *rgb, size_t cap, int rgb_on_device, int *width,
                            int *height, float range[2]);
int hpmvs_scene_depth_jpeg(const hpmvs_scene *s, int view, int level, int quality, uint8_t *out, size_t cap, size_t *n);

int hpmvs_optimize_batch(const hpmvs_scene *s, const hpmvs_options *o, hpmvs_patch_batch *b,
                         int on_device, void *stream);

int hpmvs_init_patches_batch(const hpmvs_scene *s, const hpmvs_options *o, int start_level, int n_points,
                             const double *xyz, const int32_t *meas_off, const int32_t *meas_img,
                             hpmvs_patch_batch *b, int on_device, void *stream);
int hpmvs_init_patches_sphere_batch(const hpmvs_scene *s, const hpmvs_options *o, int start_level, int n_points,
                                    const double *xyz, const int32_t *meas_off, const int32_t *meas_img,
                                    const double sphere[4], hpmvs_patch_batch *b, int on_device, void *stream);

#define HPMVS_EXPAND_EXTEND 0
#define HPMVS_EXPAND_BRANCH 1
int hpmvs_expand_batch(const hpmvs_scene *s, const hpmvs_options *o, int mode, const hpmvs_patch_batch *parents,
                       const float *cell_center, const float *cell_width, const uint8_t *skip,
                       hpmvs_patch_batch *out, int on_device, void *stream);
int hpmvs_expand_directions(int mode, float *dxdy);

int hpmvs_objective_batch(const hpmvs_scene *s, const hpmvs_options *o, const hpmvs_patch_batch *b,
                          const double *x, double *f_out, int32_t *ngrabs_out, int on_device,
                          void *stream);

int hpmvs_inccs_batch(const hpmvs_scene *s, const hpmvs_options *o, const hpmvs_patch_batch *b,
                      int ref_idx, int robust, float *out, int on_device, void *stream);

int hpmvs_scene_depth_reset(hpmvs_scene *s);
int hpmvs_scene_depth_set_level(hpmvs_scene *s, int view, int level, const float *data, int rows, int cols);
int hpmvs_scene_depth_get_level(const hpmvs_scene *s, int view, int level, float *data, size_t capacity, int *rows, int *cols);
int hpmvs_set_depths_batch(hpmvs_scene *s, const hpmvs_patch_batch *b, int on_device, void *stream);
int hpmvs_depth_gates_batch(const hpmvs_scene *s, const hpmvs_patch_batch *b, float margin, int abs_int,
                            int32_t *n_visible, int32_t *n_blocking, int32_t *n_free, int on_device, void *stream);
int hpmvs_depth_ops_batch(hpmvs_scene *s, const hpmvs_patch_batch *b, const uint8_t *subtract, int on_device, void *stream);
int hpmvs_level_support_batch(const hpmvs_scene *s, const hpmvs_patch_batch *b, int min_level, int32_t *support, int on_device, void *stream);
int hpmvs_depth_footprints_batch(const hpmvs_scene *s, const hpmvs_patch_batch *b, int32_t *writes, int32_t *frees,
                                 int32_t *attached, int32_t *view_block, int on_device, void *stream);
int hpmvs_level_conflicts_batch(const hpmvs_scene *s, const hpmvs_patch_batch *b, const uint8_t *is_event, uint32_t *flow_off,
                                uint32_t *flow_adj, size_t cap_flow, uint32_t *anti_off, uint32_t *anti_adj, size_t cap_anti,
                                uint32_t *n_flow, uint32_t *n_anti, int on_device, void *stream);
int hpmvs_conflicts_from_footprints(int device, int n, int max_images, int n_views, int n_levels, const int32_t *n_images,
                                    const int32_t *writes, const int32_t *frees, const int32_t *attached, const int32_t *view_block,
                                    const uint8_t *is_event, uint32_t *flow_off, uint32_t *flow_adj, size_t cap_flow,
                                    uint32_t *anti_off, uint32_t *anti_adj, size_t cap_anti, uint32_t *n_flow, uint32_t *n_anti,
                                    int on_device, void *stream);
#define HPMVS_WALK_EVENT 1
#define HPMVS_WALK_REFINED 2
#define HPMVS_WALK_BORDER 4
#define HPMVS_WALK_HAS_PRE 8
#define HPMVS_WALK_PRE_TAKEN 16
#define HPMVS_WALK_POST_TAKEN 32
int hpmvs_level_walk_batch(hpmvs_scene *s, const hpmvs_options *o, const hpmvs_patch_batch *items, const uint8_t *flags,
                           const int32_t *set, const uint64_t *pre_key, const uint64_t *post_key, float margin, int abs_int,
                           int32_t *stage, int32_t *counts, uint8_t *accepted, int32_t *wave, int32_t *n_waves, int on_device,
                           void *stream);
int hpmvs_last_level_walk(const hpmvs_scene *s, int32_t *rounds, int32_t *most_rounds, int32_t *in_order_passes);

#define HPMVS_MAX_TREE_DEPTH 21
#define HPMVS_REGULARIZE_PROBES 24
typedef struct {
    int32_t n;
    float root_center[3];
    float root_width;
    const float *cell_center;
    const float *cell_width;
    const float *patch_center;
    const int32_t *born;
    const int32_t *died;
} hpmvs_leaf_table;
int hpmvs_regularize_batch(const hpmvs_scene *s, const hpmvs_patch_batch *cells, const float *cell_width, const int32_t *position,
                           const uint8_t *expanded, const hpmvs_leaf_table *leaves, float *flatness, int32_t *n_neighbours,
                           int32_t *neighbour_leaf, int on_device, void *stream);

int hpmvs_filter_batch(const hpmvs_scene *s, const hpmvs_patch_batch *patches, const int32_t *cell_start, int n_cells, float *dist,
                       int32_t *keep, int on_device, void *stream);

typedef struct {
    float root_center[3];
    float root_width;
    float scale_floor;
    int32_t n_rows;
    int32_t n_leaves;
} hpmvs_seed_tree_info;
int hpmvs_seed_tree_batch(hpmvs_scene *s, hpmvs_patch_batch *b, int patch_init_maxlevel, int set_depths,
                          hpmvs_seed_tree_info *info, int32_t *rows , int32_t *cell_start ,
                          float *cell_center , float *cell_width , int32_t *cell_level ,
                          float *patch_center , int on_device, void *stream);

typedef struct {
    float root_center[3];
    float root_width;
    int32_t n_branches;
    int32_t n_leaves;
    const uint64_t *branch_key;
    const uint64_t *leaf_key;
} hpmvs_octree_index;
int hpmvs_octree_locate_batch(const hpmvs_scene *s, const hpmvs_octree_index *t, int n, const float *points ,
                              const float *add_width , uint8_t *inside , uint64_t *leaf_key ,
                              int32_t *leaf_index , float *leaf_width , float *leaf_center ,
                              uint64_t *target_key , int on_device, void *stream);

typedef struct {
    uint8_t  *skip;
    uint8_t  *pre_inside;
    uint64_t *pre_key;
    uint8_t  *border;
    uint64_t *post_key;
} hpmvs_extend_tree_keys;
int hpmvs_extend_tree_batch(const hpmvs_scene *s, const hpmvs_options *o, const hpmvs_octree_index *t,
                            const hpmvs_patch_batch *parents, float width, hpmvs_patch_batch *out,
                            const hpmvs_extend_tree_keys *keys, int on_device, void *stream);

typedef struct {
    int32_t n_trees;
    const float    *root;
    const int32_t  *branch_first;
    const int32_t  *leaf_first;
    const uint64_t *branch_key;
    const uint64_t *leaf_key;
} hpmvs_octree_forest;
int hpmvs_extend_forest_batch(const hpmvs_scene *s, const hpmvs_options *o, const hpmvs_octree_forest *f,
                              const hpmvs_patch_batch *parents, const int32_t *parent_tree ,
                              float width, hpmvs_patch_batch *out, const hpmvs_extend_tree_keys *keys, int on_device, void *stream);

typedef struct {
    int32_t  *support;
    uint8_t  *removed;
    uint8_t  *split;
    uint8_t  *children;
    uint64_t *child_key;
    int32_t  *n_neighbours;
    uint64_t *neighbour_key;
} hpmvs_process_forest_result;
int hpmvs_process_forest_batch(hpmvs_scene *s, const hpmvs_options *o, const hpmvs_octree_forest *f, const float *leaf_patch_center,
                               const hpmvs_patch_batch *cells, const int32_t *cell_tree, const uint64_t *cell_key, float *flatness,
                               const uint8_t *final_level, hpmvs_patch_batch *out, const hpmvs_process_forest_result *res,
                               int on_device, void *stream);

int hpmvs_octree_insert_batch(const hpmvs_scene *s, const hpmvs_octree_index *t, int n, const float *points ,
                              const float *add_width , uint8_t *accepted , uint64_t *leaf_key ,
                              int32_t *blocker , int on_device, void *stream);
int hpmvs_octree_route_batch(const hpmvs_scene *s, int n_trees, const float *roots , int n,
                             const float *points , int32_t *tree , int on_device, void *stream);

typedef struct {
    int32_t  *tree;
    uint8_t  *accepted;
    uint64_t *leaf_key;
    int32_t  *blocker;
} hpmvs_border_forest_result;
int hpmvs_border_forest_batch(hpmvs_scene *s, const hpmvs_octree_forest *f, const hpmvs_patch_batch *border,
                              int set_depths, const hpmvs_border_forest_result *res, int on_device, void *stream);

#define HPMVS_MAX_SUBTREES 4096
typedef struct {
    int32_t n_trees;
    int32_t n_orphans;
    int32_t n_splits;
    int32_t stop;
    int32_t histogram[HPMVS_MAX_TREE_DEPTH + 1];
} hpmvs_octree_partition_info;
int hpmvs_octree_partition(const hpmvs_scene *s, const hpmvs_octree_index *t, int min_trees, int min_split_leaves,
                           hpmvs_octree_partition_info *info,
                           uint64_t *root_key      ,  float *root_cell ,
                           int32_t *tree_first     ,  int32_t *tree_leaves ,
                           int32_t *leaf_order     ,
                           int32_t *leaf_tree      ,   uint64_t *leaf_sub_key   ,
                           int32_t *branch_tree    , uint64_t *branch_sub_key ,
                           int on_device, void *stream);

void *hpmvs_host_alloc(size_t bytes);
void hpmvs_host_free(void *p);
int hpmvs_last_staging(const hpmvs_scene *s, unsigned long long *staged_bytes, unsigned long long *in_place_bytes);

int hpmvs_last_kernel_ms(const hpmvs_scene *s, float *ms);
int hpmvs_last_wide_patches(const hpmvs_scene *s, int32_t *n);

typedef struct hpmvs_record {
    float center[4];
    float normal[4];
    float color[3];
    float scale;
    double fmin;
    uint8_t ok;
    uint8_t pad0;
    uint16_t n_images;
    uint8_t pad1[4];
    uint16_t images[HPMVS_RECORD_IMAGES];
} hpmvs_record;
typedef struct hpmvs_record_tail {
    int32_t patch;
    uint16_t count;
    uint16_t pad;
    uint16_t images[HPMVS_MAX_IMAGES - HPMVS_RECORD_IMAGES];
} hpmvs_record_tail;
int hpmvs_pack_record_tails(const hpmvs_patch_batch *b, hpmvs_record_tail *tails, int32_t cap, int32_t *n_tails, void *stream);
int hpmvs_unpack_record_tails(const hpmvs_record_tail *tails, int32_t n_tails, int32_t patch_offset, hpmvs_patch_batch *b, void *stream);
int hpmvs_pack_records(const hpmvs_patch_batch *b, hpmvs_record *records, void *stream);
int hpmvs_unpack_records(const hpmvs_record *records, int n, hpmvs_patch_batch *b, void *stream);
int hpmvs_allgather_records(void *nccl_comm, const hpmvs_record *send, size_t count, hpmvs_record *recv, void *stream);

#define HPMVS_PLY_BINARY 1
#define HPMVS_PLY_NORMAL 2
#define HPMVS_PLY_SCALE 4
#define HPMVS_PLY_VISIBILITY 8
int hpmvs_ply_ext_batch(int device, const hpmvs_patch_batch *b, const int32_t *order, int n_rows, int flags,
                        uint8_t *out, size_t cap, size_t *n, int on_device, void *stream);
int hpmvs_ply_ext_timed(int device, const hpmvs_patch_batch *b, const int32_t *order, int n_rows, int flags,
                        uint8_t *out, size_t cap, size_t *n, float *ms );

int hpmvs_selftest_bobyqa(int device, int n, const int32_t *kind, const double *params, const double *x0,
                          const double *lb, const double *ub, int maxeval, double *xfinal, double *minf,
                          int32_t *result, int32_t *nevals, int32_t *rescue_calls, double *trace, int trace_cap);

#ifdef __cplusplus
}
#endif
#endif
```

Before: 5.175 million.

## Reuse per-image NCC values to skip reference refinement and final INCC pass

Adds a reference-reuse path, on by default. The per-image INCC values from the filter stage are kept in an extra per-wave results row. Candidate 0's reference sum is then computed from these saved values instead of being re-evaluated, and the best reference's row is snapshotted during the reference search so the closing filter pass can derive its keep mask without another INCC objective call. This removes one photometric evaluation per patch, and usually the final INCC pass too. In exchange it doubles the results-row workspace, adds global-memory row copies on every new best reference, and adds atomic debug counters in the hot loop.

```diff
diff --git a/hpmvs_amd/api.py b/hpmvs_amd/api.py
--- a/hpmvs_amd/api.py
+++ b/hpmvs_amd/api.py
@@ -84,7 +84,7 @@
     "hpmvs_scene_create", "hpmvs_scene_set_view", "hpmvs_scene_set_covis", "hpmvs_scene_commit",
     "hpmvs_scene_destroy", "hpmvs_scene_get_level", "hpmvs_scene_bytes", "hpmvs_build_pyramid",
     "hpmvs_optimize_batch", "hpmvs_init_patches_batch", "hpmvs_objective_batch", "hpmvs_inccs_batch", "hpmvs_last_kernel_ms",
-    "hpmvs_last_wide_patches",
+    "hpmvs_last_wide_patches", "hpmvs_last_ref_reuse",
     "hpmvs_expand_batch", "hpmvs_expand_directions", "hpmvs_selftest_bobyqa",
     "hpmvs_pack_records", "hpmvs_unpack_records", "hpmvs_allgather_records", "hpmvs_pack_record_tails", "hpmvs_unpack_record_tails",
     "hpmvs_scene_depth_reset", "hpmvs_scene_depth_set_level", "hpmvs_scene_depth_get_level",
@@ -164,6 +164,8 @@
     L.hpmvs_inccs_batch.argtypes = [C.c_void_p, C.POINTER(Options), C.POINTER(PatchBatch), C.c_int, C.c_int,
                                     C.c_void_p, C.c_int, C.c_void_p]
     L.hpmvs_last_kernel_ms.argtypes = [C.c_void_p, C.POINTER(C.c_float)]
+    if hasattr(L, "hpmvs_last_ref_reuse"):
+        L.hpmvs_last_ref_reuse.argtypes = [C.c_void_p, C.POINTER(C.c_int32)]
     L.hpmvs_host_alloc.argtypes = [C.c_size_t]
     L.hpmvs_host_alloc.restype = C.c_void_p
     L.hpmvs_host_free.argtypes = [C.c_void_p]
@@ -454,6 +456,13 @@
         _chk(lib().hpmvs_last_wide_patches(self.h, C.byref(n)))
         return n.value
 
+    REF_REUSE_COUNTERS = ("cand0_from_f2", "cand0_posted", "closing_same_ref", "closing_new_ref", "closing_removed")
+
+    def last_ref_reuse(self) -> dict:
+        out = (C.c_int32 * 5)()
+        _chk(lib().hpmvs_last_ref_reuse(self.h, out))
+        return dict(zip(self.REF_REUSE_COUNTERS, (int(v) for v in out)))
+
     def last_kernel_ms(self) -> float:
         ms = C.c_float()
         _chk(lib().hpmvs_last_kernel_ms(self.h, C.byref(ms)))
diff --git a/hpmvs_amd/csrc/capi.hip b/hpmvs_amd/csrc/capi.hip
--- a/hpmvs_amd/csrc/capi.hip
+++ b/hpmvs_amd/csrc/capi.hip
@@ -2815,6 +2815,16 @@
     return HPMVS_OK;
 }
 
+int hpmvs_last_ref_reuse(const hpmvs_scene* s, int32_t* out5) {
+    if (!s || !out5) return fail(HPMVS_ERR_ARG, "last_ref_reuse: null argument");
+    for (int k = 0; k < 5; k++) out5[k] = 0;
+    if (!s->last_ws) return HPMVS_OK;
+    HIPCHK(hipSetDevice(s->device));
+    HIPCHK(hipDeviceSynchronize());
+    HIPCHK(hipMemcpy(out5, s->last_ws + 208, 5 * sizeof(int32_t), hipMemcpyDeviceToHost));
+    return HPMVS_OK;
+}
+
 int hpmvs_debug_counters(const hpmvs_scene* s, unsigned long long* out4) {
     if (!s || !out4) return fail(HPMVS_ERR_ARG, "debug_counters: null argument");
     HIPCHK(hipSetDevice(s->device));
diff --git a/hpmvs_amd/csrc/kernel_optimize.hip b/hpmvs_amd/csrc/kernel_optimize.hip
--- a/hpmvs_amd/csrc/kernel_optimize.hip
+++ b/hpmvs_amd/csrc/kernel_optimize.hip
@@ -73,6 +73,8 @@
 constexpr int kRow = 64;
 constexpr size_t kCounterBytes = 1024;
 constexpr int kPark16 = HPMVS_REGION_16;
+constexpr int kResRows = HPMVS_REF_REUSE ? 2 : 1;
+constexpr int kReuseCounters = 208;
 
 #ifndef HPMVS_PARK_AUX
 #define HPMVS_PARK_AUX 0
@@ -161,7 +163,7 @@
     uint4* park = (uint4*)((char*)queue + kCounterBytes + (size_t)W * n_wgs * kP * kRow * sizeof(uint16_t)) + (size_t)gw * kPark16;
 #if HPMVS_COLD_GLOBAL
     char* cold = (char*)queue + kCounterBytes + (size_t)W * n_wgs * kP * kRow * sizeof(uint16_t) + (size_t)W * n_wgs * kPark16 * 16 +
-                 (size_t)W * n_wgs * kP * kRow * sizeof(float) + (size_t)gw * BQ_NCOLD * kP * sizeof(double);
+                 (size_t)W * n_wgs * kResRows * kP * kRow * sizeof(float) + (size_t)gw * BQ_NCOLD * kP * sizeof(double);
     {
         const unsigned long long a = (unsigned long long)cold;
         const unsigned lo = (unsigned)__builtin_amdgcn_readfirstlane((int)(a & 0xffffffffull)), hi = (unsigned)__builtin_amdgcn_readfirstlane((int)(a >> 32));
@@ -169,10 +171,11 @@
     }
 #endif
     const GlobalRows erows{(float*)((char*)queue + kCounterBytes + (size_t)W * n_wgs * kP * kRow * sizeof(uint16_t) +
-                                    (size_t)W * n_wgs * kPark16 * 16) + (size_t)gw * kP * kRow, kRow};
+                                    (size_t)W * n_wgs * kPark16 * 16) + (size_t)gw * kResRows * kP * kRow, kRow};
     constexpr bool kProxy = HPMVS_PROXY == 2 || (HPMVS_PROXY == 1 && SERVICE);
+    constexpr bool kReuse = HPMVS_REF_REUSE && !kProxy;
     gdouble* const auxw = (gdouble*)(unsigned long long)((char*)queue + kCounterBytes + (size_t)W * n_wgs * kP * kRow * sizeof(uint16_t) +
-                          (size_t)W * n_wgs * kPark16 * 16 + (size_t)W * n_wgs * kP * kRow * sizeof(float) +
+                          (size_t)W * n_wgs * kPark16 * 16 + (size_t)W * n_wgs * kResRows * kP * kRow * sizeof(float) +
                           (size_t)W * n_wgs * (size_t)(HPMVS_COLD_GLOBAL ? (164 - HPMVS_STATE_ND) : 0) * kP * sizeof(double)) +
                           (size_t)gw * kP * kAuxDoubles;
     gdouble* const aux = auxw + (lane < kP ? lane : 0) * kAuxDoubles;
@@ -373,10 +376,20 @@
                 break;
             case S_F2B: {
                 nimg = res_n;
-                if (res_fail) { fail_stage = res_fail; finish_fail = true; break; }
+                if (res_fail > 0) { fail_stage = res_fail; finish_fail = true; break; }
                 ii = 0; refindex = -1; refbest = 3.402823466e+38f;
                 op = OP_REFSUM; req_ref = 0; req_robust = 1;
                 stage = S_RS;
+#if HPMVS_REF_REUSE
+                if (kReuse) {
+                    __hip_atomic_fetch_add(&queue[kReuseCounters + (res_fail < 0 ? 0 : 1)], 1, __ATOMIC_RELAXED, __HIP_MEMORY_SCOPE_AGENT);
+                    if (res_fail < 0) {
+                        refbest = res_sum; refindex = 0; ngrabs += nimg;
+                        ii = 1; req_ref = 1;
+                        if (nimg < 2) { op = OP_NONE; ii = 0; res_sum = 3.402823466e+38f; }
+                    }
+                }
+#endif
                 if (kProxy) {
                     gfloat* ctx = (gfloat*)aux + kAuxCtx;
                     ctx[0] = scale; ctx[1] = __int_as_float(nimg);
@@ -385,7 +398,16 @@
                 break;
             }
             case S_RS: {
-                if (res_sum < refbest) { refbest = res_sum; refindex = ii; }
+                if (res_sum < refbest) {
+                    refbest = res_sum; refindex = ii;
+#if HPMVS_REF_REUSE
+                    if (kReuse) {
+                        const gfloat* cur = (const gfloat*)(unsigned long long)(erows.base + (lane < kP ? lane : 0) * kRow);
+                        gfloat* best = (gfloat*)(unsigned long long)(erows.base + (kP + (lane < kP ? lane : 0)) * kRow);
+                        for (int k = 0; k < nimg; k++) best[k] = cur[k];
+                    }
+#endif
+                }
                 ii++;
                 if (kProxy) {
                     for (int k = 0; k < extra; k++) {
@@ -402,6 +424,13 @@
                     row[0] = row[refindex];
                     row[refindex] = t;
                 }
+#if HPMVS_REF_REUSE
+                if (kReuse && refindex >= 0) {
+                    res_mask = (unsigned long long)refindex;
+                    op = OPL_F3R; stage = S_F3B;
+                    break;
+                }
+#endif
                 op = OP_INCC; req_ref = 0; req_robust = 0; req_thr = o.NCC_ALPHA_2;
                 stage = S_F3;
                 break;
@@ -411,6 +440,13 @@
                 stage = S_F3B;
                 break;
             case S_F3B: {
+#if HPMVS_REF_REUSE
+                if (res_fail < 0) {
+                    op = OP_INCC; req_ref = 0; req_robust = 0; req_thr = o.NCC_ALPHA_2;
+                    stage = S_F3;
+                    break;
+                }
+#endif
                 nimg = res_n;
                 if (res_fail) { fail_stage = res_fail; finish_fail = true; break; }
                 finish_ok = true;
@@ -468,7 +504,7 @@
         }
         {
             wave_lds_sync();
-            const unsigned long long lm = __ballot(op >= OPL_ADD && op <= OPL_F3);
+            const unsigned long long lm = __ballot(op >= OPL_ADD && op <= OPL_LAST);
             if (lm) {
                 BQ_PROF_BEGIN(tls_);
                 for (unsigned long long t = lm; t; t &= t - 1ull) {
@@ -481,14 +517,31 @@
                     const float pscale = bcast_f(scale, p);
                     const unsigned long long pmask = bcast_u64(res_mask, p);
                     ListResult r;
-                    r.nimg = 0; r.fail = 0; r.rgb = U3{0.0f, 0.0f, 0.0f};
+                    r.nimg = 0; HPMVS_LIST_RESULT_INIT(r);
                     const ListEnv le = list_env(sc, o);
                     if (kind == OPL_ADD) r.nimg = coop_add_images(le, prow, pn, pc, pnrm, pscale);
                     else if (kind == OPL_F1) r = coop_list_f1(le, prow, pn, pmask, pc, pnrm, pscale);
+#if HPMVS_REF_REUSE
+                    else if (kind == OPL_F2) r = coop_list_f2(le, prow, pn, pmask, pc, pnrm, erows.base + p * kRow, erows.base + (kP + p) * kRow,
+                                                              kReuse && 1.0f - o.NCC_ALPHA_2 <= 2.0f);
+#else
                     else if (kind == OPL_F2) r = coop_list_f2(le, prow, pn, pmask, pc, pnrm);
-                    else { LevelThr lt; for (int k = 0; k < kMaxLevels; k++) lt.t[k] = sc.lvl_thr[k]; r = coop_list_f3(sc.views, lt, o.MIN_IMAGES_PER_PATCH, prow, pn, pmask, pc, pscale, b.max_images, service || b.color != nullptr); }
+#endif
+                    else { LevelThr lt; for (int k = 0; k < kMaxLevels; k++) lt.t[k] = sc.lvl_thr[k]; r = coop_list_f3(sc.views, lt, o.MIN_IMAGES_PER_PATCH, prow, pn, pmask, pc, pscale, b.max_images, service || b.color != nullptr
+#if HPMVS_REF_REUSE
+                                           , kind == OPL_F3R ? erows.base + (kP + p) * kRow : nullptr, 1.0f - o.NCC_ALPHA_2
+#endif
+                                           ); }
                     if (lane == p) {
                         res_n = r.nimg; res_fail = r.fail;
+#if HPMVS_REF_REUSE
+                        if (kind == OPL_F2 && r.cand0) { res_fail = -1; res_sum = r.cand0_sum; }
+                        if (kind == OPL_F3R && r.cand0) {
+                            ngrabs += r.cand0;
+                            __hip_atomic_fetch_add(&queue[kReuseCounters + (refindex > 0 ? 3 : 2)], 1, __ATOMIC_RELAXED, __HIP_MEMORY_SCOPE_AGENT);
+                            if (r.cand0_sum != 0.0f) __hip_atomic_fetch_add(&queue[kReuseCounters + 4], 1, __ATOMIC_RELAXED, __HIP_MEMORY_SCOPE_AGENT);
+                        }
+#endif
                         res_rgb[0] = r.rgb.x; res_rgb[1] = r.rgb.y; res_rgb[2] = r.rgb.z;
                         op = OP_NONE;
                     }
@@ -618,7 +671,7 @@
                 else if (failed) { op = OP_NONE; stage = S_BQFAIL; }
                 else if (done) { op = OPL_ADD; stage = S_ADD2; }
             }
-            if (__any((op == OP_NONE && stage != S_IDLE) || (op >= OPL_ADD && op <= OPL_F3))) continue;
+            if (__any((op == OP_NONE && stage != S_IDLE) || (op >= OPL_ADD && op <= OPL_LAST))) continue;
         }
         const uint16_t* brow = row;
         if (kProxy) {
@@ -746,7 +799,7 @@
 
 size_t HPMVS_V(optimize_workspace_bytes)(int n_cus) {
     const size_t waves = (size_t)HPMVS_WG_WAVES * max_workgroups(n_cus, HPMVS_WG_WAVES, HPMVS_WG_REGIONS);
-    return kCounterBytes + waves * kP * kRow * sizeof(uint16_t) + waves * (size_t)kPark16 * 16 + waves * kP * kRow * sizeof(float) +
+    return kCounterBytes + waves * kP * kRow * sizeof(uint16_t) + waves * (size_t)kPark16 * 16 + waves * kResRows * kP * kRow * sizeof(float) +
            waves * (size_t)(HPMVS_COLD_GLOBAL ? (164 - HPMVS_STATE_ND) : 0) * kP * sizeof(double) +
            (HPMVS_PROXY == 2 ? waves * kP * kAuxDoubles * sizeof(double) : 0);
 }
@@ -754,7 +807,7 @@
 #ifndef HPMVS_VARIANT_SUFFIX
 size_t optimize_workspace_bytes_for(int wgs) {
     return kCounterBytes + (size_t)2 * wgs * kP * kRow * sizeof(uint16_t) + (size_t)2 * wgs * (size_t)kPark16 * 16 +
-           (size_t)2 * wgs * kP * kRow * sizeof(float) + (size_t)2 * wgs * (size_t)(HPMVS_COLD_GLOBAL ? (164 - HPMVS_STATE_ND) : 0) * kP * sizeof(double) +
+           (size_t)2 * wgs * kResRows * kP * kRow * sizeof(float) + (size_t)2 * wgs * (size_t)(HPMVS_COLD_GLOBAL ? (164 - HPMVS_STATE_ND) : 0) * kP * sizeof(double) +
            (HPMVS_PROXY ? (size_t)2 * wgs * kP * kAuxDoubles * sizeof(double) : 0);
 }
 size_t optimize_stage_bytes_for(int wgs) { return (size_t)2 * wgs * kP * kSvcOutDwords * sizeof(uint32_t); }
diff --git a/hpmvs_amd/csrc/photometric.hpp b/hpmvs_amd/csrc/photometric.hpp
--- a/hpmvs_amd/csrc/photometric.hpp
+++ b/hpmvs_amd/csrc/photometric.hpp
@@ -163,6 +163,10 @@
 
 __device__ __forceinline__ float robustincc(float rhs) { return rhs / (1 + 3 * rhs); }
 
+#ifndef HPMVS_REF_REUSE
+#define HPMVS_REF_REUSE 1
+#endif
+
 struct PackedReq {
     int obj_mode;
     int ref, robust, nimg;
@@ -474,6 +478,9 @@
                 okS[k] = __ballot(PS[k].ok != 0);
                 const unsigned long long pb = (unsigned long long)PS[k].pix;
                 pix_lo[k] = (int)(pb & 0xffffffffull); pix_hi[k] = (int)(pb >> 32);
+#if HPMVS_REF_REUSE
+                if (!WRITE_INCCS && J > 64 * k && jp[k] >= 0 && PS[k].ok == 0) rows.store(jp[k], ji[k], 2.0f);
+#endif
             }
         }
 
@@ -511,7 +518,11 @@
         PH_T(t2);
         PH_ADD(t1, t2, 13);
 
+    #if HPMVS_REF_REUSE
+        int g_req = -1, g_off = 0, g_ref = 0, g_cur = 0;
+#else
         int g_req = -1, g_off = 0, g_ref = 0, g_userob = 0, g_cur = 0;
+#endif
         bool g_isref = false;
         unsigned long long g_ok = 0ull;
         float refn[kRowVals];
@@ -531,10 +542,14 @@
                     todo &= ~(1ull << p);
                     const int gl = __ffsll((long long)idle) - 1;
                     idle &= idle - 1ull;
-                    const int r_off = bcast_i(myoff, p), r_ref = bcast_i(q_refsel, p), r_rob = bcast_i(q_userob, p);
+                    const int r_off = bcast_i(myoff, p), r_ref = bcast_i(q_refsel, p);
                     const unsigned long long r_ok = bcast_u64(myok, p);
+#if !HPMVS_REF_REUSE
+                    const int r_rob = bcast_i(q_userob, p);
+                    if (gl0 == gl) g_userob = r_rob;
+#endif
                     if (gl0 == gl) {
-                        g_req = p; g_off = r_off; g_ref = r_ref; g_userob = r_rob;
+                        g_req = p; g_off = r_off; g_ref = r_ref;
                         g_ok = r_ok & ~(1ull << r_ref);
                         g_cur = r_ref; g_isref = true;
                     }
@@ -545,7 +560,10 @@
                     const int n_other = __popcll(nonref);
                     const int nh = n_other < kGroups - 1 ? n_other : kGroups - 1;
                     if (nh > 0) {
-                        const int r_req = bcast_i(g_req, 0), r_off = bcast_i(g_off, 0), r_ref = bcast_i(g_ref, 0), r_rob = bcast_i(g_userob, 0);
+                        const int r_req = bcast_i(g_req, 0), r_off = bcast_i(g_off, 0), r_ref = bcast_i(g_ref, 0);
+#if !HPMVS_REF_REUSE
+                        const int r_rob = bcast_i(g_userob, 0);
+#endif
                         unsigned long long mine = nonref, rest = nonref;
 #pragma unroll
                         for (int i = 1; i < kGroups; i++) {
@@ -554,7 +572,10 @@
                         }
                         if (grp == 0) g_ok = rest;
                         else if (glane && grp <= nh) {
-                            g_req = r_req; g_off = r_off; g_ref = r_ref; g_userob = r_rob;
+                            g_req = r_req; g_off = r_off; g_ref = r_ref;
+#if !HPMVS_REF_REUSE
+                            g_userob = r_rob;
+#endif
                             g_cur = __ffsll((long long)mine) - 1; g_ok = 0ull; g_isref = false; rsrc = yy;
                         }
                         moved = true;
@@ -579,11 +600,17 @@
                         const int take = (best + 1) / 2;
                         unsigned long long hi = bcast_u64(g_ok, vl);
                         for (int i = 0; i < best - take; i++) hi &= hi - 1ull;
-                        const int r_req = bcast_i(g_req, vl), r_off = bcast_i(g_off, vl), r_ref = bcast_i(g_ref, vl), r_rob = bcast_i(g_userob, vl);
+                        const int r_req = bcast_i(g_req, vl), r_off = bcast_i(g_off, vl), r_ref = bcast_i(g_ref, vl);
+#if !HPMVS_REF_REUSE
+                        const int r_rob = bcast_i(g_userob, vl);
+#endif
                         const int r_src = bcast_i(rsrc, vl);
                         if (gl0 == vl) g_ok &= ~hi;
                         if (gl0 == tl && glane) {
-                            g_req = r_req; g_off = r_off; g_ref = r_ref; g_userob = r_rob;
+                            g_req = r_req; g_off = r_off; g_ref = r_ref;
+#if !HPMVS_REF_REUSE
+                            g_userob = r_rob;
+#endif
                             g_cur = __ffsll((long long)hi) - 1; g_ok = hi & (hi - 1ull); g_isref = false; rsrc = r_src + yy;
                         }
                     }
@@ -689,7 +716,10 @@
                 t[3 * xx + 1] = div_by(t[3 * xx + 1] - a1, iv);
                 t[3 * xx + 2] = div_by(t[3 * xx + 2] - a2, iv);
             }
-            float raw = 0.0f, rob = 0.0f;
+            float raw = 0.0f;
+#if !HPMVS_REF_REUSE
+            float rob = 0.0f;
+#endif
 #pragma unroll
             for (int i = 0; i < kRowVals; i++) refn[i] = g_isref ? t[i] : refn[i];
             if (moved) {
@@ -703,13 +733,19 @@
 #pragma unroll
                 for (int i = 0; i < kRowVals; i++) pr[i] = refn[i] * t[i];
                 raw = 1.0f - div_by(shfl_f(window_sum<kRowVals>(pr), last), 1.0 / 147.0);
+#if !HPMVS_REF_REUSE
                 rob = robustincc(raw);
+#endif
             }
             PH_T(t7);
             PH_ADD(t6, t7, 21);
 
             if (act) {
+#if HPMVS_REF_REUSE
+                if (!g_isref && yy == 0) rows.store(g_req, g_cur, raw);
+#else
                 if (!g_isref && yy == 0) rows.store(g_req, g_cur, g_userob ? rob : raw);
+#endif
                 if (g_ok) { g_cur = __ffsll((long long)g_ok) - 1; g_ok &= g_ok - 1ull; g_isref = false; }
                 else g_req = -1;
             }
@@ -723,6 +759,9 @@
         if (inbatch && !refok) {
             if (q.obj_mode) out.obj = 2.0;
             else {
+#if HPMVS_REF_REUSE
+                if (!WRITE_INCCS && q.nimg > 0) rows.store(lane, q_refsel, __int_as_float(0));
+#endif
                 float s = 0.0f;
                 for (int k = 0; k < q.nimg; k++) s += 2.0f;
                 out.keep = 0ull;
@@ -753,9 +792,15 @@
                     const bool isref = k == q_refsel;
                     const unsigned long long bit = 1ull << (k & 63);
                     const bool add_o = in && okk && !isref;
-                    val += add_o ? (double)e[j] : 0.0;
+#if HPMVS_REF_REUSE
+                    const float ev = q_userob ? robustincc(e[j]) : e[j];
+                    if (WRITE_INCCS) { if (q_userob && add_o) rows.store(lane, k, ev); }
+#else
+                    const float ev = e[j];
+#endif
+                    val += add_o ? (double)ev : 0.0;
                     nok += add_o ? 1 : 0;
-                    const float v = okk ? e[j] : 2.0f;
+                    const float v = okk ? ev : 2.0f;
                     s += (in && !isref) ? v : 0.0f;
                     const bool kp = in && (isref ? (0.0f < thr1) : (v < thr1));
                     keep |= kp ? bit : 0ull;
@@ -768,6 +813,9 @@
                     out.keep = WRITE_INCCS ? myok : keep;
                     out.incc_sum = s;
                     if (WRITE_INCCS) rows.store(lane, q_refsel, 0.0f);
+#if HPMVS_REF_REUSE
+                    else rows.store(lane, q_refsel, __int_as_float(mylen));
+#endif
                 }
             }
         }
diff --git a/hpmvs_amd/csrc/pipeline.hpp b/hpmvs_amd/csrc/pipeline.hpp
--- a/hpmvs_amd/csrc/pipeline.hpp
+++ b/hpmvs_amd/csrc/pipeline.hpp
@@ -10,7 +10,13 @@
 
 enum Op { OP_NONE = 0, OP_OBJ = 1, OP_INCC = 2, OP_REFSUM = 3,
           OPL_ADD = 4, OPL_F1 = 5, OPL_F2 = 6, OPL_F3 = 7,
+#if HPMVS_REF_REUSE
+          OPL_F3R = 8, OPL_LAST = 8,
+          OPQ_START = 9, OPQ_STEP = 10 };
+#else
+          OPL_LAST = 7,
           OPQ_START = 8, OPQ_STEP = 9 };
+#endif
 enum Stage {
     S_FETCH = 0, S_WAIT, S_ADD1, S_F1, S_F1B, S_BQ, S_BQFAIL, S_ADD2, S_F2, S_F2B, S_RS, S_F3, S_F3B, S_IDLE
 };
@@ -226,7 +232,27 @@
     return U3{bcast_f(rgb[0], pick), bcast_f(rgb[1], pick), bcast_f(rgb[2], pick)};
 }
 
+#if HPMVS_REF_REUSE
+struct ListResult { int nimg; int fail; U3 rgb; int cand0; float cand0_sum; };
+#define HPMVS_LIST_RESULT_INIT(r) (r).fail = 0; (r).rgb = U3{0.0f, 0.0f, 0.0f}; (r).cand0 = 0; (r).cand0_sum = 0.0f
+#else
 struct ListResult { int nimg; int fail; U3 rgb; };
+#define HPMVS_LIST_RESULT_INIT(r) (r).fail = 0; (r).rgb = U3{0.0f, 0.0f, 0.0f}
+#endif
+
+__device__ __forceinline__ int compact_list_vals(int& id, float& val, unsigned long long keep) {
+    const int lane = lane_id();
+    int nid = -1, m = 0;
+    float nval = 0.0f;
+    for (unsigned long long t = keep; t; t &= t - 1ull, m++) {
+        const int src = __ffsll((long long)t) - 1;
+        const int v = bcast_i(id, src);
+        const float f = bcast_f(val, src);
+        if (lane == m) { nid = v; nval = f; }
+    }
+    id = nid; val = nval;
+    return m;
+}
 
 __device__ __forceinline__ void store_list(uint16_t* row, int id, int nimg) {
     if (lane_id() < nimg) row[lane_id()] = (uint16_t)id;
@@ -238,7 +264,7 @@
     const int lane = lane_id();
     const float c[3] = {c_.x, c_.y, c_.z}, n[3] = {n_.x, n_.y, n_.z};
     ListResult r;
-    r.fail = 0; r.rgb = U3{0.0f, 0.0f, 0.0f};
+    HPMVS_LIST_RESULT_INIT(r);
     int id = (lane < nimg) ? (int)row[lane] : -1;
     const unsigned long long all = nimg >= 64 ? ~0ull : ((1ull << nimg) - 1ull);
     nimg = compact_list(id, (keep | 1ull) & all);
@@ -252,13 +278,51 @@
     return r;
 }
 
+#if HPMVS_REF_REUSE
+__device__ __noinline__ ListResult coop_list_f2(ListEnv sc, uint16_t* row, int nimg, unsigned long long keep,
+                                               U3 c_, U3 n_, const float* vals, float* best, int reuse_ok) {
+    typedef __attribute__((address_space(1))) float gfloat;
+    const ListEnv& o = sc;
+    const int lane = lane_id();
+    const float c[3] = {c_.x, c_.y, c_.z}, n[3] = {n_.x, n_.y, n_.z};
+    ListResult r;
+    HPMVS_LIST_RESULT_INIT(r);
+    int id = (lane < nimg) ? (int)row[lane] : -1;
+    float v = (lane < nimg) ? ((const gfloat*)(unsigned long long)vals)[lane] : 0.0f;
+    const bool refok = __float_as_int(bcast_f(v, 0)) > 0;
+    const unsigned long long all = nimg >= 64 ? ~0ull : ((1ull << nimg) - 1ull);
+    nimg = compact_list_vals(id, v, (keep | 1ull) & all);
+    r.nimg = nimg;
+    if (nimg < o.MIN_IMAGES_PER_PATCH) { r.fail = 6; return r; }
+    bool kp = false;
+    if (lane < nimg) {
+        float ray[3];
+        ray_to_cam(sc.views[id], c, ray);
+        kp = dot3f(ray, n) > o.cos_max_f;
+    }
+    const unsigned long long ak = __ballot(kp);
+    nimg = compact_list_vals(id, v, ak);
+    r.nimg = nimg;
+    if (nimg < o.MIN_IMAGES_PER_PATCH) { r.fail = 7; return r; }
+    if (!coop_assure_image_angles(sc, o, id, nimg, c)) { r.fail = 8; return r; }
+    store_list(row, id, nimg);
+    if (reuse_ok && refok && (ak & 1ull)) {
+        const float rv = robustincc(v);
+        float s = 0.0f;
+        for (int k = 1; k < nimg; k++) s += bcast_f(rv, k);
+        if (lane < nimg) ((gfloat*)(unsigned long long)best)[lane] = lane == 0 ? __int_as_float(nimg) : v;
+        r.cand0 = 1; r.cand0_sum = s;
+    }
+    return r;
+}
+#else
 __device__ __noinline__ ListResult coop_list_f2(ListEnv sc, uint16_t* row, int nimg, unsigned long long keep,
                                                U3 c_, U3 n_) {
     const ListEnv& o = sc;
     const int lane = lane_id();
     const float c[3] = {c_.x, c_.y, c_.z}, n[3] = {n_.x, n_.y, n_.z};
     ListResult r;
-    r.fail = 0; r.rgb = U3{0.0f, 0.0f, 0.0f};
+    HPMVS_LIST_RESULT_INIT(r);
     int id = (lane < nimg) ? (int)row[lane] : -1;
     const unsigned long long all = nimg >= 64 ? ~0ull : ((1ull << nimg) - 1ull);
     nimg = compact_list(id, (keep | 1ull) & all);
@@ -271,18 +335,36 @@
     store_list(row, id, nimg);
     return r;
 }
+#endif
 
 __device__ __noinline__ ListResult coop_list_f3(const DevView* views, LevelThr lt, int min_images, uint16_t* row, int nimg, unsigned long long keep,
-                                               U3 c_, float scale, int max_images, int want_colour) {
+                                               U3 c_, float scale, int max_images, int want_colour
+#if HPMVS_REF_REUSE
+                                               , const float* best, float thr1
+#endif
+                                               ) {
     DevScene sc;
     sc.views = views; sc.covis_off = nullptr; sc.covis = nullptr; sc.n_views = 0;
     for (int k = 0; k < kMaxLevels; k++) sc.lvl_thr[k] = lt.t[k];
     const int lane = lane_id();
     const float c[3] = {c_.x, c_.y, c_.z};
     ListResult r;
-    r.fail = 0; r.rgb = U3{0.0f, 0.0f, 0.0f};
+    HPMVS_LIST_RESULT_INIT(r);
     int id = (lane < nimg) ? (int)row[lane] : -1;
     const unsigned long long all = nimg >= 64 ? ~0ull : ((1ull << nimg) - 1ull);
+#if HPMVS_REF_REUSE
+    if (best) {
+        typedef __attribute__((address_space(1))) float gfloat;
+        const gfloat* bv = (const gfloat*)(unsigned long long)best;
+        const int refsel = (int)keep;
+        const int cnt = __float_as_int(bv[refsel]);
+        if (cnt <= 0) { r.nimg = nimg; r.fail = -1; return r; }
+        bool kp = false;
+        if (lane < nimg) kp = lane == 0 ? (0.0f < thr1) : (bv[lane == refsel ? 0 : lane] < thr1);
+        keep = __ballot(kp);
+        r.cand0 = cnt; r.cand0_sum = ((keep | 1ull) & all) != all ? 1.0f : 0.0f;
+    }
+#endif
     nimg = compact_list(id, (keep | 1ull) & all);
     r.nimg = nimg;
     if (nimg < min_images) { r.fail = 9; return r; }
diff --git a/include/hpmvs_amd.h b/include/hpmvs_amd.h
--- a/include/hpmvs_amd.h
+++ b/include/hpmvs_amd.h
@@ -291,6 +291,7 @@
 
 int hpmvs_last_kernel_ms(const hpmvs_scene *s, float *ms);
 int hpmvs_last_wide_patches(const hpmvs_scene *s, int32_t *n);
+int hpmvs_last_ref_reuse(const hpmvs_scene *s, int32_t *out5);
 
 typedef struct hpmvs_record {
     float center[4];
```

Measured after the change: 5.152 million. About the same (-0.5%).
